# shichaoy/pop_up_slam

Measured on AMD Instinct MI355X. Metric: graph-solve iters/sec + final chi2, 1k-pose/5k-edge plane graph, higher is better.
Workload: dtype f64; 1 GPU; C2 synthetic corridor: 1000 SE3 poses, 200 planes, 5000 plane edges, 999 odometry edges (BASELINE.json configs[1], seed 42); jacobian_mode=numeric, total_lm_solves=773

## Files before the change

### include/pps.h

```cpp
#ifndef PPS_H
#define PPS_H

#include <stddef.h>
#include <stdint.h>

#ifdef __cplusplus
extern "C" {
#endif

#define PPS_VERSION 305

typedef struct pps_graph pps_graph;

enum pps_status {
  PPS_OK = 0,
  PPS_EINVAL = 1,
  PPS_ENOTPD = 2,
  PPS_EHIP = 3,
  PPS_ENOMEM = 4,
  PPS_ESTATE = 5
};

enum pps_jacobian_mode {
  PPS_JAC_NUMERIC = 0,
  PPS_JAC_ANALYTIC = 1
};

typedef struct pps_props {
  double epsilon2;
  double epsilon_abs;
  double epsilon_rel;
  int    max_iterations;
  double lm_lambda0;
  double lm_lambda_factor;
  int    jacobian_mode;
  int    device;
  int    verbose;
} pps_props;

void pps_default_props(pps_props* p);
int  pps_version(void);
const char* pps_last_error(const pps_graph* g);

int pps_graph_create(const pps_props* props, pps_graph** out);
int pps_graph_destroy(pps_graph* g);
int pps_get_props(const pps_graph* g, pps_props* out);
int pps_set_props(pps_graph* g, const pps_props* p);

int pps_add_pose(pps_graph* g, const double tq[7], int* id);
int pps_add_plane(pps_graph* g, const double abcd[4], int* id);

int pps_add_pose_prior(pps_graph* g, int pose, const double meas6[6], const double sqrtinf_ut[21], int* fid);
int pps_add_odometry(pps_graph* g, int pose1, int pose2, const double meas6[6], const double sqrtinf_ut[21], int* fid);
int pps_add_plane_obs(pps_graph* g, int pose, int plane, const double meas4[4], const double sqrtinf_ut[6], int* fid);
int pps_add_plane_obs2(pps_graph* g, int pose_id, int plane_id, const double meas4[4], const double ray6[6],
                       const double sqrtinf_ut[6], int* fid);
int pps_edge_ray(const float invK[9], const float seg2d[4], double ray6[6]);
int pps_add_plane_prior(pps_graph* g, int plane, const double meas4[4], const double sqrtinf_ut[6], int* fid);

int pps_set_measurement(pps_graph* g, int fid, const double meas4[4]);
int pps_set_measurements(pps_graph* g, int n, const int* fids, const double* meas4 );

int pps_remove_factor(pps_graph* g, int fid);
int pps_remove_node(pps_graph* g, int nid);

int pps_update(pps_graph* g);
int pps_batch_optimize(pps_graph* g, int* iterations);
int pps_chi2(pps_graph* g, double* chi2);

int pps_cov_recover(pps_graph* g);
int pps_cov_marginals(pps_graph* g, int n, const int* ids, double* out, int64_t* offsets);
int pps_cov_access(pps_graph* g, int n, const int* rows, const int* cols, double* out, int64_t* offsets, int* in_pattern);
int pps_cov_joint(pps_graph* g, int n, const int* ids, double* out);
int pps_cov_last_times(const pps_graph* g, double sec[2]);
int pps_cov_factor(pps_graph* g);
int pps_debug_cov_path_form(pps_graph* g, int form);
int pps_cov_select(pps_graph* g);
int pps_debug_cov_select_form(pps_graph* g, int form);
int pps_cov_block(pps_graph* g, int nr, const int* rows, int nc, const int* cols, double* out);
int pps_cov_block_last(const pps_graph* g, double* kernel_sec, int* launches);

int pps_assoc_gate(pps_graph* g, int pose_id, int n_meas, const double* meas4, const double* sqrtinf_ut, int n_planes, const int* plane_ids,
                   double* d2, int* best);
int pps_assoc_gate_last(const pps_graph* g, double* kernel_sec, int* launches);
int pps_debug_assoc_gate_records(pps_graph* g, int64_t cap, double* rec, int64_t* needed);

int pps_merge_gate(pps_graph* g, int n_planes, const int* plane_ids, double floor_var, double threshold, double* d2, int* best, int cap_pairs,
                   int* pairs, int* n_pairs);
int pps_merge_gate_last(const pps_graph* g, double* kernel_sec, int* launches, int* n_not_pd);
int pps_debug_merge_gate_records(pps_graph* g, int64_t cap, double* rec, int64_t* needed);

int pps_loop_gate(pps_graph* g, int n, const int* pose_a, const int* pose_b, const double* meas6 ,
                  const double* sqrtinf_ut , double threshold, double* d2 , double* S ,
                  int cap_accepted, int* accepted, int* n_accepted);
int pps_loop_gate_last(const pps_graph* g, double* kernel_sec, int* launches, int* n_not_pd);
int pps_debug_loop_gate_records(pps_graph* g, int64_t cap, double* rec, int64_t* needed);

int pps_factor_gate(pps_graph* g, int n, const int* fids, double thr3, double thr6, double* d2, double* leverage, int cap_flagged, int* flagged,
                    int* n_flagged);
int pps_factor_gate_last(const pps_graph* g, double* kernel_sec, int* launches, int* n_untestable);
int pps_debug_factor_gate_records(pps_graph* g, int64_t cap, double* rec, int64_t* needed);

enum pps_cost_kind { PPS_COST_NONE = 0, PPS_COST_HUBER = 1, PPS_COST_PSEUDO_HUBER = 2, PPS_COST_CAUCHY = 3 };
int pps_set_cost_function(pps_graph* g, int kind, double b);
int pps_get_cost_function(const pps_graph* g, int* kind, double* b);

typedef struct pps_multi pps_multi;
int pps_multi_create(int n, pps_graph* const* graphs, pps_multi** out);
int pps_multi_destroy(pps_multi* m);
const char* pps_multi_last_error(const pps_multi* m);
int pps_multi_optimize(pps_multi* m, int* iterations, int* status);
int pps_multi_rounds(const pps_multi* m, int* rounds);
int pps_multi_save_state(pps_multi* m);
int pps_multi_restore_state(pps_multi* m);
int pps_multi_set_profiling(pps_multi* m, int level);
int pps_multi_phase_times(const pps_multi* m, double sec[5], long long counts[4]);

int pps_num_nodes(const pps_graph* g, int* n);
int pps_num_factors(const pps_graph* g, int* n);
int pps_get_pose(pps_graph* g, int id, double tq[7]);
int pps_get_plane(pps_graph* g, int id, double abcd[4]);
int pps_set_pose(pps_graph* g, int id, const double tq[7]);
int pps_set_plane(pps_graph* g, int id, const double abcd[4]);
int pps_get_poses(pps_graph* g, int n, const int* ids, double* out);
int pps_get_planes(pps_graph* g, int n, const int* ids, double* out);
int pps_save_state(pps_graph* g);
int pps_restore_state(pps_graph* g);

typedef struct pps_stats {
  int    n_poses, n_planes, n_factors;
  int    dim_nodes, dim_measure;
  int    n_fronts, n_levels, max_front;
  int64_t nnz_L;
  int    lm_iterations;
  int    lm_trials_accepted, lm_trials_rejected;
  double chi2_initial, chi2_final, lambda_final;
  double last_delta_norm;
  double t_total, t_analysis, t_upload;
  double t_linearize, t_assemble, t_factor, t_backsolve, t_retract_chi2;
  int    n_linearize, n_factorize;
  int    lm_trials_notpd;
  int    n_launches;
} pps_stats;
int pps_get_stats(const pps_graph* g, pps_stats* out);
int pps_get_trace(const pps_graph* g, int cap, double* lambda, double* chi2, int* accepted, int* n);
int pps_set_profiling(pps_graph* g, int level);

int pps_factor_shape(const pps_graph* g, int fid, int* dim, int* cols);
int pps_eval_factor(pps_graph* g, int fid, int mode , double* J, double* r);

int pps_analyze(pps_graph* g);
int pps_analysis_reuse(const pps_graph* g, int* fronts_kept, int* fronts_total);
int pps_analysis_kept(const pps_graph* g, int kept[6]);
int pps_analysis_dump(pps_graph* g, int64_t cap, int32_t* out, int64_t* needed);

int pps_time_linearize(pps_graph* g, int mode, int iters, double* sec_per_launch);
int pps_bench_sweep(pps_graph* g, int mode, int replicas, int iters, double sec_per_sweep[3],
                    int64_t* n_plane_edges, int64_t* n_odo_edges);

int pps_debug_front_factor(int tiles, int strip, int p, int b, const double* A, double* L, double* U, double* not_pd);
int pps_debug_front_factor_w(int tiles, int strip, int p, int b, const double* A, double* L, double* U, double* not_pd, int width);

int pps_debug_exmap(int kind, int n, const double* x, const double* delta, double* out);

int pps_debug_solve(pps_graph* g, double lambda, double lambda2, double* delta, double* delta2, int* form, double* not_pd);

int pps_popup_planes(int device, const float* seg2d, int n, const float invK[9], const float T_wc[16],
                     float* planes_out);

typedef struct pps_point { float x, y, z; uint32_t rgba; } pps_point;

typedef struct pps_popup pps_popup;
int pps_popup_create(int device, int width, int height, const float invK[9], pps_popup** out);
int pps_popup_destroy(pps_popup* p);
const char* pps_popup_last_error(const pps_popup* p);
int pps_popup_set_image(pps_popup* p, const unsigned char* bgr);
int pps_popup_run(pps_popup* p, const float* seg2d, int n, const float T_wc[16], const float* polys,
                  const int* poly_off, int nplanes, int step, float depth_thre, float ceiling_thre, int* n_valid);
int pps_popup_run_async(pps_popup* p, const float* seg2d, int n, const float T_wc[16], const float* polys,
                        const int* poly_off, int nplanes, int step, float depth_thre, float ceiling_thre);
int pps_popup_planes_wait(pps_popup* p, float* planes);
int pps_popup_wait(pps_popup* p, int* n_valid);
int pps_popup_download(pps_popup* p, float* planes, pps_point* cloud, float* depth, int32_t* plane_id);
int pps_popup_set_outputs(pps_popup* p, int want_depth, int want_plane_id);
int pps_popup_plane_info(pps_popup* p, float plane_cam_dist_thre, const int* actual_plane_indices, int n_actual,
                         float* dist_to_cam, int32_t* good);
int pps_popup_fill_depth(pps_popup* p);
int pps_popup_download_segments3d(pps_popup* p, float* seg3d_world);
int pps_popup_last_kernel_time(const pps_popup* p, double* sec);
int pps_popup_polygons_simple(const float K[9], const float invK[9], const float T_wc[16], int width, int height, const float* seg2d, int n,
                              float* verts, int cap_verts, int* poly_off, int* n_verts);
int pps_popup_mask_host(const float* polys, const int* poly_off, int nplanes, int width, int height, int step, int32_t* plane_id);

int pps_frames_set_calibration(pps_graph* g, const float invK[9]);
int pps_frames_add(pps_graph* g, int pose_id, int n_seg, const float* seg2d, const int* fids, int* frame_id);
int pps_refresh_measurements(pps_graph* g);
int pps_get_measurement(pps_graph* g, int fid, double meas4[4]);

typedef struct pps_assoc_params {
  double edge_asso_2ddist;
  double edge_asso_planedist;
  double edge_asso_proj;
  double edge_asso_angle;
  int assoc_near_frames;
} pps_assoc_params;
void pps_assoc_default_params(pps_assoc_params* p);
int pps_landmark_update(pps_graph* g, int plane_id, int frame_plane_indice, int frame_seq_id, const float seg2d[4],
                        const float seg3d_xy[4]);
int pps_landmark_set_merged(pps_graph* g, int plane_id);
int pps_find_closest_planes(pps_graph* g, const double est_pose[7], int frame_seq_id, int n, const double* planes_local,
                            const int* frame_plane_indice, const float* seg2d, const float* seg3d_xy,
                            const pps_assoc_params* prm, int* best_plane_id, double* best_err);

int pps_graph_save(pps_graph* g, const char* path, int precision);
int pps_graph_load(const char* path, const pps_props* props, pps_graph** out);

int pps_reproject_points(pps_graph* g, int n, const int* plane_ids, const float* pts_xyz, float* out_xyz);

typedef struct pps_edge_params {
  int downsample_contour;
  int dilation_distance, erosion_distance;
  double pre_vertical_thre, pre_minium_len, pre_contour_close_thre, interval_overlap_thre, post_short_thre,
         post_bind_dist_thre, post_merge_dist_thre, post_merge_angle_thre, post_extend_thre;
  double pre_boundary_thre, pre_merge_angle_thre, pre_merge_dist_thre, pre_proj_angle_thre, pre_proj_cover_thre,
         pre_proj_cover_large_thre, pre_proj_dist_thre;
} pps_edge_params;
void pps_edge_default_params(pps_edge_params* p);

typedef struct pps_edges pps_edges;
int pps_edges_create(int device, int width, int height, pps_edges** out);
int pps_edges_destroy(pps_edges* e);
const char* pps_edges_last_error(const pps_edges* e);
int pps_edges_select(pps_edges* e, const unsigned char* label_map, int label_on_device, const float* lsd_lines,
                     int n_lines, const pps_edge_params* prm, float* open_segs, int* n_open, float* closed_segs,
                     int* n_closed, float* open_in_closed);
int pps_edges_download_label(pps_edges* e, unsigned char* out, int* w, int* h);
int pps_edges_contour(pps_edges* e, float* xy, int cap, int* n, int* n_contours, int* n_points);
int pps_edges_last_kernel_time(const pps_edges* e, double* sec);
int pps_edges_host_contour(const int16_t* cell_segs, int n, float scale, float* xy, int cap, int* n_xy, int* n_contours,
                           int* n_points);
int pps_edges_host_select(const float* contour_xy, int n_contour, int width, int height, const float* lsd_lines, int n_lines,
                          const pps_edge_params* prm, float* open_segs, int* n_open, float* closed_segs, int* n_closed,
                          float* open_in_closed);

typedef struct pps_map pps_map;
typedef struct pps_map_chunk {
  int32_t frame;
  int32_t frame_seq_id;
  int32_t frame_plane;
  int32_t plane_id;
  int64_t offset, count;
} pps_map_chunk;
typedef struct pps_map_totals {
  int64_t capacity, n_points;
  int64_t built_points;
  int32_t n_frames, n_chunks, built_chunks, reserved;
} pps_map_totals;
typedef struct pps_map_select {
  int32_t counter;
  int32_t every_frame;
  int32_t old_age, old_every, new_every;
  int32_t age[3], min_tracked[3];
} pps_map_select;
void pps_map_default_select(pps_map_select* s, int counter);
int pps_map_create(pps_graph* g, int64_t capacity_points, pps_map** out);
int pps_map_destroy(pps_map* m);
const char* pps_map_last_error(const pps_map* m);
int pps_map_add_frame(pps_map* m, pps_popup* p, int frame_seq_id, int nplanes, const int* plane_node_ids, int* counts);
int pps_map_redirect(pps_map* m, int from_plane, int to_plane);
int pps_map_info(const pps_map* m, pps_map_totals* out);
int pps_map_chunks(const pps_map* m, int cap, pps_map_chunk* out, int* n);
int pps_map_built_chunks(const pps_map* m, int cap, pps_map_chunk* out, int* n);
int pps_map_select_host(const pps_map_chunk* chunks, int n, const pps_map_select* sel, int32_t* keep, int* n_keep);
int pps_map_build(pps_map* m, const pps_map_select* sel, int64_t* n_points, int* n_chunks);
int pps_map_download(pps_map* m, int which, int64_t first, int64_t n, pps_point* out);
int pps_map_last_times(const pps_map* m, double sec[2]);

#ifdef __cplusplus
}
#endif
#endif
```

### pop_up_slam_amd/__init__.py

```python
from __future__ import annotations

import ctypes as C
import os

import numpy as np

_HERE = os.path.dirname(os.path.abspath(__file__))
LIB_PATH = os.environ.get("PPS_LIB") or os.path.join(_HERE, "libpps.so")

PPS_OK, PPS_EINVAL, PPS_ENOTPD, PPS_EHIP, PPS_ENOMEM, PPS_ESTATE = range(6)
JAC_NUMERIC, JAC_ANALYTIC = 0, 1
COST_NONE, COST_HUBER, COST_PSEUDO_HUBER, COST_CAUCHY = range(4)

_dp = C.POINTER(C.c_double)
_fp = C.POINTER(C.c_float)
_ip = C.POINTER(C.c_int)


PPS_VERSION = 305


class PpsProps(C.Structure):
    _fields_ = [
        ("epsilon2", C.c_double), ("epsilon_abs", C.c_double), ("epsilon_rel", C.c_double),
        ("max_iterations", C.c_int), ("lm_lambda0", C.c_double), ("lm_lambda_factor", C.c_double),
        ("jacobian_mode", C.c_int), ("device", C.c_int), ("verbose", C.c_int),
    ]


class PpsStats(C.Structure):
    _fields_ = [
        ("n_poses", C.c_int), ("n_planes", C.c_int), ("n_factors", C.c_int),
        ("dim_nodes", C.c_int), ("dim_measure", C.c_int),
        ("n_fronts", C.c_int), ("n_levels", C.c_int), ("max_front", C.c_int),
        ("nnz_L", C.c_int64),
        ("lm_iterations", C.c_int), ("lm_trials_accepted", C.c_int), ("lm_trials_rejected", C.c_int),
        ("chi2_initial", C.c_double), ("chi2_final", C.c_double), ("lambda_final", C.c_double),
        ("last_delta_norm", C.c_double),
        ("t_total", C.c_double), ("t_analysis", C.c_double), ("t_upload", C.c_double),
        ("t_linearize", C.c_double), ("t_assemble", C.c_double), ("t_factor", C.c_double),
        ("t_backsolve", C.c_double), ("t_retract_chi2", C.c_double),
        ("n_linearize", C.c_int), ("n_factorize", C.c_int), ("lm_trials_notpd", C.c_int), ("n_launches", C.c_int),
    ]

    def asdict(self):
        return {k: getattr(self, k) for k, _ in self._fields_}


class PpsError(RuntimeError):
    def __init__(self, code, msg):
        super().__init__(f"pps error {code}: {msg}")
        self.code = code


_LIB = None

def edge_ray(invK, seg2d):
    k = np.ascontiguousarray(invK, dtype=np.float32).reshape(9); sg = np.ascontiguousarray(seg2d, dtype=np.float32).reshape(4)
    out = np.zeros(6)
    rc = lib().pps_edge_ray(k.ctypes.data_as(_fp), sg.ctypes.data_as(_fp), out.ctypes.data_as(_dp))
    if rc != PPS_OK:
        raise PpsError(rc, "pps_edge_ray")
    return out


class PpsEdgeParams(C.Structure):
    _fields_ = [("downsample_contour", C.c_int), ("dilation_distance", C.c_int), ("erosion_distance", C.c_int)] + [
        (k, C.c_double) for k in ("pre_vertical_thre", "pre_minium_len", "pre_contour_close_thre", "interval_overlap_thre",
                                  "post_short_thre", "post_bind_dist_thre", "post_merge_dist_thre", "post_merge_angle_thre",
                                  "post_extend_thre", "pre_boundary_thre", "pre_merge_angle_thre", "pre_merge_dist_thre",
                                  "pre_proj_angle_thre", "pre_proj_cover_thre", "pre_proj_cover_large_thre",
                                  "pre_proj_dist_thre")]


class PpsAssocParams(C.Structure):
    _fields_ = [("edge_asso_2ddist", C.c_double), ("edge_asso_planedist", C.c_double), ("edge_asso_proj", C.c_double),
                ("edge_asso_angle", C.c_double), ("assoc_near_frames", C.c_int)]


class PpsMapChunk(C.Structure):
    _fields_ = [("frame", C.c_int32), ("frame_seq_id", C.c_int32), ("frame_plane", C.c_int32), ("plane_id", C.c_int32),
                ("offset", C.c_int64), ("count", C.c_int64)]


class PpsMapTotals(C.Structure):
    _fields_ = [("capacity", C.c_int64), ("n_points", C.c_int64), ("built_points", C.c_int64),
                ("n_frames", C.c_int32), ("n_chunks", C.c_int32), ("built_chunks", C.c_int32), ("reserved", C.c_int32)]


class PpsMapSelect(C.Structure):
    _fields_ = [("counter", C.c_int32), ("every_frame", C.c_int32), ("old_age", C.c_int32), ("old_every", C.c_int32),
                ("new_every", C.c_int32), ("age", C.c_int32 * 3), ("min_tracked", C.c_int32 * 3)]


CHUNK_DTYPE = np.dtype([("frame", "<i4"), ("frame_seq_id", "<i4"), ("frame_plane", "<i4"), ("plane_id", "<i4"),
                        ("offset", "<i8"), ("count", "<i8")])


SYMBOLS = [
    "pps_default_props", "pps_version", "pps_last_error", "pps_graph_create", "pps_graph_destroy",
    "pps_get_props", "pps_set_props", "pps_add_pose", "pps_add_plane", "pps_add_pose_prior",
    "pps_add_odometry", "pps_add_plane_obs", "pps_add_plane_prior", "pps_set_measurement",
    "pps_set_measurements", "pps_remove_factor", "pps_remove_node", "pps_update", "pps_batch_optimize",
    "pps_chi2", "pps_num_nodes", "pps_num_factors", "pps_get_pose", "pps_get_plane", "pps_set_pose",
    "pps_set_plane", "pps_get_poses", "pps_get_planes", "pps_get_stats", "pps_get_trace",
    "pps_set_profiling", "pps_factor_shape", "pps_eval_factor", "pps_analyze", "pps_analysis_dump",
    "pps_bench_sweep", "pps_save_state", "pps_restore_state",
    "pps_popup_planes", "pps_popup_create", "pps_popup_destroy", "pps_popup_last_error", "pps_popup_set_image",
    "pps_popup_run", "pps_popup_run_async", "pps_popup_planes_wait", "pps_popup_wait", "pps_popup_download", "pps_popup_last_kernel_time",
    "pps_frames_set_calibration", "pps_frames_add", "pps_refresh_measurements", "pps_get_measurement",
    "pps_popup_download_segments3d", "pps_assoc_default_params", "pps_landmark_update", "pps_landmark_set_merged",
    "pps_find_closest_planes", "pps_graph_save", "pps_graph_load", "pps_add_plane_obs2", "pps_edge_ray",
    "pps_time_linearize", "pps_debug_front_factor", "pps_debug_front_factor_w", "pps_debug_exmap", "pps_debug_solve", "pps_reproject_points", "pps_popup_set_outputs",
    "pps_edge_default_params", "pps_edges_create", "pps_edges_destroy", "pps_edges_last_error", "pps_edges_select",
    "pps_edges_download_label", "pps_edges_contour", "pps_edges_last_kernel_time", "pps_edges_host_contour",
    "pps_edges_host_select", "pps_popup_fill_depth", "pps_popup_plane_info", "pps_popup_mask_host",
    "pps_multi_create", "pps_multi_destroy", "pps_multi_last_error", "pps_multi_optimize", "pps_multi_rounds", "pps_multi_save_state", "pps_multi_restore_state", "pps_multi_set_profiling", "pps_multi_phase_times", "pps_popup_polygons_simple", "pps_analysis_reuse", "pps_analysis_kept",
    "pps_cov_recover", "pps_cov_marginals", "pps_cov_access", "pps_cov_joint", "pps_cov_last_times",
    "pps_cov_factor", "pps_debug_cov_path_form", "pps_cov_select", "pps_debug_cov_select_form",
    "pps_cov_block", "pps_cov_block_last", "pps_assoc_gate", "pps_assoc_gate_last", "pps_debug_assoc_gate_records",
    "pps_merge_gate", "pps_merge_gate_last", "pps_debug_merge_gate_records",
    "pps_factor_gate", "pps_factor_gate_last", "pps_debug_factor_gate_records",
    "pps_loop_gate", "pps_loop_gate_last", "pps_debug_loop_gate_records",
    "pps_map_default_select", "pps_map_create", "pps_map_destroy", "pps_map_last_error", "pps_map_add_frame", "pps_map_redirect",
    "pps_map_info", "pps_map_chunks", "pps_map_built_chunks", "pps_map_select_host", "pps_map_build", "pps_map_download",
    "pps_map_last_times",
    "pps_set_cost_function", "pps_get_cost_function",
]


def lib():
    global _LIB
    if _LIB is None:
        if not os.path.exists(LIB_PATH):
            raise ImportError(
                f"{LIB_PATH} not found: build it with `python -c 'import __graft_entry__ as g; g.build()'` "
                "(or make -C pop_up_slam_amd/csrc).  There is no CPU fallback.")
        L = C.CDLL(LIB_PATH)
        L.pps_version.restype = C.c_int
        if L.pps_version() != PPS_VERSION:
            raise ImportError(f"{LIB_PATH} reports PPS_VERSION {L.pps_version()}, this binding mirrors {PPS_VERSION}: rebuild the library")
        L.pps_last_error.restype = C.c_char_p
        L.pps_last_error.argtypes = [C.c_void_p]
        L.pps_default_props.argtypes = [C.POINTER(PpsProps)]
        L.pps_default_props.restype = None
        L.pps_graph_create.argtypes = [C.POINTER(PpsProps), C.POINTER(C.c_void_p)]
        L.pps_graph_destroy.argtypes = [C.c_void_p]
        L.pps_get_props.argtypes = [C.c_void_p, C.POINTER(PpsProps)]
        L.pps_set_props.argtypes = [C.c_void_p, C.POINTER(PpsProps)]
        L.pps_add_pose.argtypes = [C.c_void_p, _dp, _ip]
        L.pps_add_plane.argtypes = [C.c_void_p, _dp, _ip]
        L.pps_add_pose_prior.argtypes = [C.c_void_p, C.c_int, _dp, _dp, _ip]
        L.pps_add_odometry.argtypes = [C.c_void_p, C.c_int, C.c_int, _dp, _dp, _ip]
        L.pps_add_plane_obs.argtypes = [C.c_void_p, C.c_int, C.c_int, _dp, _dp, _ip]
        L.pps_add_plane_prior.argtypes = [C.c_void_p, C.c_int, _dp, _dp, _ip]
        L.pps_set_measurement.argtypes = [C.c_void_p, C.c_int, _dp]
        L.pps_set_measurements.argtypes = [C.c_void_p, C.c_int, _ip, _dp]
        L.pps_remove_factor.argtypes = [C.c_void_p, C.c_int]
        L.pps_remove_node.argtypes = [C.c_void_p, C.c_int]
        L.pps_update.argtypes = [C.c_void_p]
        L.pps_batch_optimize.argtypes = [C.c_void_p, _ip]
        L.pps_chi2.argtypes = [C.c_void_p, _dp]
        L.pps_num_nodes.argtypes = [C.c_void_p, _ip]
        L.pps_num_factors.argtypes = [C.c_void_p, _ip]
        L.pps_get_pose.argtypes = [C.c_void_p, C.c_int, _dp]
        L.pps_get_plane.argtypes = [C.c_void_p, C.c_int, _dp]
        L.pps_set_pose.argtypes = [C.c_void_p, C.c_int, _dp]
        L.pps_set_plane.argtypes = [C.c_void_p, C.c_int, _dp]
        L.pps_get_poses.argtypes = [C.c_void_p, C.c_int, _ip, _dp]
        L.pps_get_planes.argtypes = [C.c_void_p, C.c_int, _ip, _dp]
        L.pps_save_state.argtypes = [C.c_void_p]
        L.pps_restore_state.argtypes = [C.c_void_p]
        L.pps_get_stats.argtypes = [C.c_void_p, C.POINTER(PpsStats)]
        L.pps_get_trace.argtypes = [C.c_void_p, C.c_int, _dp, _dp, _ip, _ip]
        L.pps_set_profiling.argtypes = [C.c_void_p, C.c_int]
        L.pps_factor_shape.argtypes = [C.c_void_p, C.c_int, _ip, _ip]
        L.pps_eval_factor.argtypes = [C.c_void_p, C.c_int, C.c_int, _dp, _dp]
        L.pps_analyze.argtypes = [C.c_void_p]
        L.pps_analysis_dump.argtypes = [C.c_void_p, C.c_int64, C.POINTER(C.c_int32), C.POINTER(C.c_int64)]
        L.pps_bench_sweep.argtypes = [C.c_void_p, C.c_int, C.c_int, C.c_int, _dp, C.POINTER(C.c_int64),
                                      C.POINTER(C.c_int64)]
        _u8 = C.POINTER(C.c_ubyte)
        L.pps_popup_planes.argtypes = [C.c_int, _fp, C.c_int, _fp, _fp, _fp]
        L.pps_popup_create.argtypes = [C.c_int, C.c_int, C.c_int, _fp, C.POINTER(C.c_void_p)]
        L.pps_popup_destroy.argtypes = [C.c_void_p]
        L.pps_popup_last_error.argtypes = [C.c_void_p]
        L.pps_popup_last_error.restype = C.c_char_p
        L.pps_popup_set_image.argtypes = [C.c_void_p, _u8]
        L.pps_popup_run.argtypes = [C.c_void_p, _fp, C.c_int, _fp, _fp, _ip, C.c_int, C.c_int, C.c_float, C.c_float, _ip]
        L.pps_popup_run_async.argtypes = L.pps_popup_run.argtypes[:-1]
        L.pps_popup_planes_wait.argtypes = [C.c_void_p, _fp]
        L.pps_popup_wait.argtypes = [C.c_void_p, C.POINTER(C.c_int)]
        L.pps_popup_download.argtypes = [C.c_void_p, _fp, C.c_void_p, _fp, C.POINTER(C.c_int32)]
        L.pps_popup_last_kernel_time.argtypes = [C.c_void_p, _dp]
        L.pps_popup_mask_host.argtypes = [_fp, _ip, C.c_int, C.c_int, C.c_int, C.c_int, C.POINTER(C.c_int32)]
        L.pps_popup_polygons_simple.argtypes = [_fp, _fp, _fp, C.c_int, C.c_int, _fp, C.c_int, _fp, C.c_int, _ip, _ip]
        L.pps_multi_create.argtypes = [C.c_int, C.POINTER(C.c_void_p), C.POINTER(C.c_void_p)]
        L.pps_multi_destroy.argtypes = [C.c_void_p]
        L.pps_multi_last_error.argtypes = [C.c_void_p]
        L.pps_multi_last_error.restype = C.c_char_p
        L.pps_multi_optimize.argtypes = [C.c_void_p, _ip, _ip]
        L.pps_multi_rounds.argtypes = [C.c_void_p, _ip]
        L.pps_multi_save_state.argtypes = [C.c_void_p]; L.pps_multi_restore_state.argtypes = [C.c_void_p]
        L.pps_multi_set_profiling.argtypes = [C.c_void_p, C.c_int]
        L.pps_multi_phase_times.argtypes = [C.c_void_p, _dp, C.POINTER(C.c_longlong)]
        L.pps_popup_fill_depth.argtypes = [C.c_void_p]
        L.pps_popup_plane_info.argtypes = [C.c_void_p, C.c_float, _ip, C.c_int, _fp, _ip]
        L.pps_frames_set_calibration.argtypes = [C.c_void_p, _fp]
        L.pps_frames_add.argtypes = [C.c_void_p, C.c_int, C.c_int, _fp, _ip, _ip]
        L.pps_refresh_measurements.argtypes = [C.c_void_p]
        L.pps_get_measurement.argtypes = [C.c_void_p, C.c_int, _dp]
        L.pps_popup_download_segments3d.argtypes = [C.c_void_p, _fp]
        L.pps_popup_set_outputs.argtypes = [C.c_void_p, C.c_int, C.c_int]
        L.pps_assoc_default_params.argtypes = [C.POINTER(PpsAssocParams)]
        L.pps_edge_default_params.argtypes = [C.POINTER(PpsEdgeParams)]; L.pps_edge_default_params.restype = None
        L.pps_edges_create.argtypes = [C.c_int, C.c_int, C.c_int, C.POINTER(C.c_void_p)]
        L.pps_edges_destroy.argtypes = [C.c_void_p]
        L.pps_edges_last_error.argtypes = [C.c_void_p]; L.pps_edges_last_error.restype = C.c_char_p
        L.pps_edges_select.argtypes = [C.c_void_p, C.c_void_p, C.c_int, _fp, C.c_int, C.POINTER(PpsEdgeParams), _fp, _ip, _fp, _ip, _fp]
        L.pps_edges_download_label.argtypes = [C.c_void_p, C.POINTER(C.c_ubyte), _ip, _ip]
        L.pps_edges_contour.argtypes = [C.c_void_p, _fp, C.c_int, _ip, _ip, _ip]
        L.pps_edges_last_kernel_time.argtypes = [C.c_void_p, _dp]
        L.pps_edges_host_contour.argtypes = [C.POINTER(C.c_int16), C.c_int, C.c_float, _fp, C.c_int, _ip, _ip, _ip]
        L.pps_edges_host_select.argtypes = [_fp, C.c_int, C.c_int, C.c_int, _fp, C.c_int, C.POINTER(PpsEdgeParams), _fp, _ip, _fp, _ip, _fp]
        L.pps_assoc_default_params.restype = None
        L.pps_landmark_update.argtypes = [C.c_void_p, C.c_int, C.c_int, C.c_int, _fp, _fp]
        L.pps_landmark_set_merged.argtypes = [C.c_void_p, C.c_int]
        L.pps_add_plane_obs2.argtypes = [C.c_void_p, C.c_int, C.c_int, _dp, _dp, _dp, _ip]
        L.pps_edge_ray.argtypes = [_fp, _fp, _dp]
        L.pps_time_linearize.argtypes = [C.c_void_p, C.c_int, C.c_int, C.POINTER(C.c_double)]
        L.pps_debug_front_factor.argtypes = [C.c_int, C.c_int, C.c_int, C.c_int, _dp, _dp, _dp, C.POINTER(C.c_double)]
        if hasattr(L, "pps_debug_front_factor_w"):
            L.pps_debug_front_factor_w.argtypes = L.pps_debug_front_factor.argtypes + [C.c_int]
        L.pps_debug_exmap.argtypes = [C.c_int, C.c_int, _dp, _dp, _dp]
        L.pps_debug_solve.argtypes = [C.c_void_p, C.c_double, C.c_double, _dp, _dp, C.POINTER(C.c_int), C.POINTER(C.c_double)]
        L.pps_reproject_points.argtypes = [C.c_void_p, C.c_int, _ip, _fp, _fp]
        L.pps_graph_save.argtypes = [C.c_void_p, C.c_char_p, C.c_int]
        L.pps_graph_load.argtypes = [C.c_char_p, C.POINTER(PpsProps), C.POINTER(C.c_void_p)]
        L.pps_find_closest_planes.argtypes = [C.c_void_p, _dp, C.c_int, C.c_int, _dp, _ip, _fp, _fp, C.POINTER(PpsAssocParams), _ip, _dp]
        _i64p = C.POINTER(C.c_int64)
        L.pps_cov_recover.argtypes = [C.c_void_p]
        L.pps_cov_marginals.argtypes = [C.c_void_p, C.c_int, _ip, _dp, _i64p]
        L.pps_cov_access.argtypes = [C.c_void_p, C.c_int, _ip, _ip, _dp, _i64p, _ip]
        L.pps_cov_joint.argtypes = [C.c_void_p, C.c_int, _ip, _dp]
        L.pps_cov_last_times.argtypes = [C.c_void_p, _dp]
        L.pps_cov_factor.argtypes = [C.c_void_p]
        L.pps_debug_cov_path_form.argtypes = [C.c_void_p, C.c_int]
        L.pps_cov_select.argtypes = [C.c_void_p]
        L.pps_debug_cov_select_form.argtypes = [C.c_void_p, C.c_int]
        L.pps_cov_block.argtypes = [C.c_void_p, C.c_int, _ip, C.c_int, _ip, _dp]
        L.pps_cov_block_last.argtypes = [C.c_void_p, _dp, _ip]
        L.pps_assoc_gate.argtypes = [C.c_void_p, C.c_int, C.c_int, _dp, _dp, C.c_int, _ip, _dp, _ip]
        L.pps_assoc_gate_last.argtypes = [C.c_void_p, _dp, _ip]
        L.pps_debug_assoc_gate_records.argtypes = [C.c_void_p, C.c_int64, _dp, C.POINTER(C.c_int64)]
        L.pps_merge_gate.argtypes = [C.c_void_p, C.c_int, _ip, C.c_double, C.c_double, _dp, _ip, C.c_int, _ip, _ip]
        L.pps_merge_gate_last.argtypes = [C.c_void_p, _dp, _ip, _ip]
        L.pps_debug_merge_gate_records.argtypes = [C.c_void_p, C.c_int64, _dp, C.POINTER(C.c_int64)]
        L.pps_loop_gate.argtypes = [C.c_void_p, C.c_int, _ip, _ip, _dp, _dp, C.c_double, _dp, _dp, C.c_int, _ip, _ip]
        L.pps_loop_gate_last.argtypes = [C.c_void_p, _dp, _ip, _ip]
        L.pps_debug_loop_gate_records.argtypes = [C.c_void_p, C.c_int64, _dp, C.POINTER(C.c_int64)]
        L.pps_factor_gate.argtypes = [C.c_void_p, C.c_int, _ip, C.c_double, C.c_double, _dp, _dp, C.c_int, _ip, _ip]
        L.pps_factor_gate_last.argtypes = [C.c_void_p, _dp, _ip, _ip]
        L.pps_debug_factor_gate_records.argtypes = [C.c_void_p, C.c_int64, _dp, C.POINTER(C.c_int64)]
        L.pps_set_cost_function.argtypes = [C.c_void_p, C.c_int, C.c_double]
        L.pps_get_cost_function.argtypes = [C.c_void_p, _ip, _dp]
        _i32p = C.POINTER(C.c_int32)
        L.pps_map_default_select.argtypes = [C.POINTER(PpsMapSelect), C.c_int]; L.pps_map_default_select.restype = None
        L.pps_map_create.argtypes = [C.c_void_p, C.c_int64, C.POINTER(C.c_void_p)]
        L.pps_map_destroy.argtypes = [C.c_void_p]
        L.pps_map_last_error.argtypes = [C.c_void_p]; L.pps_map_last_error.restype = C.c_char_p
        L.pps_map_add_frame.argtypes = [C.c_void_p, C.c_void_p, C.c_int, C.c_int, _ip, _ip]
        L.pps_map_redirect.argtypes = [C.c_void_p, C.c_int, C.c_int]
        L.pps_map_info.argtypes = [C.c_void_p, C.POINTER(PpsMapTotals)]
        L.pps_map_chunks.argtypes = [C.c_void_p, C.c_int, C.c_void_p, _ip]
        L.pps_map_built_chunks.argtypes = [C.c_void_p, C.c_int, C.c_void_p, _ip]
        L.pps_map_select_host.argtypes = [C.c_void_p, C.c_int, C.POINTER(PpsMapSelect), _i32p, _ip]
        L.pps_map_build.argtypes = [C.c_void_p, C.POINTER(PpsMapSelect), _i64p, _ip]
        L.pps_map_download.argtypes = [C.c_void_p, C.c_int, C.c_int64, C.c_int64, C.c_void_p]
        L.pps_map_last_times.argtypes = [C.c_void_p, _dp]
        _LIB = L
    return _LIB


def _d(a, n=None):
    a = np.ascontiguousarray(a, dtype=np.float64)
    if n is not None and a.size != n:
        raise ValueError(f"expected {n} doubles, got {a.size}")
    return a, a.ctypes.data_as(_dp)


def default_props(**kw):
    p = PpsProps()
    lib().pps_default_props(C.byref(p))
    for k, v in kw.items():
        setattr(p, k, v)
    return p


class Graph:

    def __init__(self, **props):
        self.L = lib()
        self.props = default_props(**props)
        h = C.c_void_p()
        rc = self.L.pps_graph_create(C.byref(self.props), C.byref(h))
        if rc != PPS_OK:
            raise PpsError(rc, "pps_graph_create failed")
        self.h = h

    @classmethod
    def load(cls, path, **props):
        self = cls.__new__(cls)
        self.L = lib()
        self.props = default_props(**props)
        h = C.c_void_p()
        rc = self.L.pps_graph_load(os.fsencode(path), C.byref(self.props), C.byref(h))
        if rc != PPS_OK:
            raise PpsError(rc, f"pps_graph_load({path}) failed")
        self.h = h
        return self

    def save(self, path, precision=0):
        self._ck(self.L.pps_graph_save(self.h, os.fsencode(path), int(precision)))

    def close(self):
        if getattr(self, "h", None):
            self.L.pps_graph_destroy(self.h)
            self.h = None

    def __del__(self):
        try:
            self.close()
        except Exception:
            pass

    def _ck(self, rc):
        if rc != PPS_OK:
            raise PpsError(rc, self.L.pps_last_error(self.h).decode())

    def set_props(self, **kw):
        for k, v in kw.items():
            setattr(self.props, k, v)
        self._ck(self.L.pps_set_props(self.h, C.byref(self.props)))

    def get_props(self):
        p = PpsProps(); self._ck(self.L.pps_get_props(self.h, C.byref(p))); return p

    def add_pose(self, tq):
        a, p = _d(tq, 7); i = C.c_int(); self._ck(self.L.pps_add_pose(self.h, p, C.byref(i))); return i.value

    def add_plane(self, abcd):
        a, p = _d(abcd, 4); i = C.c_int(); self._ck(self.L.pps_add_plane(self.h, p, C.byref(i))); return i.value

    def add_pose_prior(self, pose, meas6, ut21):
        a, p = _d(meas6, 6); b, q = _d(ut21, 21); i = C.c_int()
        self._ck(self.L.pps_add_pose_prior(self.h, pose, p, q, C.byref(i))); return i.value

    def add_odometry(self, p1, p2, meas6, ut21):
        a, p = _d(meas6, 6); b, q = _d(ut21, 21); i = C.c_int()
        self._ck(self.L.pps_add_odometry(self.h, p1, p2, p, q, C.byref(i))); return i.value

    def add_plane_obs(self, pose, plane, meas4, ut6):
        a, p = _d(meas4, 4); b, q = _d(ut6, 6); i = C.c_int()
        self._ck(self.L.pps_add_plane_obs(self.h, pose, plane, p, q, C.byref(i))); return i.value

    def add_plane_obs2(self, pose, plane, meas4, ray6, ut6):
        a, p = _d(meas4, 4); r, pr = _d(ray6, 6); b, q = _d(ut6, 6); i = C.c_int()
        self._ck(self.L.pps_add_plane_obs2(self.h, pose, plane, p, pr, q, C.byref(i))); return i.value

    def add_plane_prior(self, plane, meas4, ut6):
        a, p = _d(meas4, 4); b, q = _d(ut6, 6); i = C.c_int()
        self._ck(self.L.pps_add_plane_prior(self.h, plane, p, q, C.byref(i))); return i.value

    def set_measurement(self, fid, meas4):
        a, p = _d(meas4, 4); self._ck(self.L.pps_set_measurement(self.h, fid, p))

    def set_measurements(self, fids, meas):
        f = np.ascontiguousarray(fids, dtype=np.int32); a, p = _d(meas, 4 * len(f))
        self._ck(self.L.pps_set_measurements(self.h, len(f), f.ctypes.data_as(_ip), p))

    def remove_factor(self, fid):
        self._ck(self.L.pps_remove_factor(self.h, fid))

    def remove_node(self, nid):
        self._ck(self.L.pps_remove_node(self.h, nid))

    def update(self):
        self._ck(self.L.pps_update(self.h))

    def batch_optimize(self):
        it = C.c_int(); self._ck(self.L.pps_batch_optimize(self.h, C.byref(it))); return it.value

    def chi2(self):
        v = C.c_double(); self._ck(self.L.pps_chi2(self.h, C.byref(v))); return v.value

    def set_cost_function(self, kind, b=1.0):
        self._ck(self.L.pps_set_cost_function(self.h, int(kind), float(b)))

    def cost_function(self):
        k = C.c_int(); b = C.c_double()
        self._ck(self.L.pps_get_cost_function(self.h, C.byref(k), C.byref(b)))
        return k.value, b.value

    def _node_dims(self, ids):
        dims = []
        for i in ids:
            try:
                self.get_pose(int(i)); dims.append(6)
            except PpsError:
                self.get_plane(int(i)); dims.append(3)
        return dims

    def cov_recover(self):
        self._ck(self.L.pps_cov_recover(self.h))

    def cov_factor(self):
        self._ck(self.L.pps_cov_factor(self.h))

    def cov_select(self):
        self._ck(self.L.pps_cov_select(self.h))

    def debug_cov_select_form(self, form):
        self._ck(self.L.pps_debug_cov_select_form(self.h, int(form)))

    def debug_cov_path_form(self, form):
        self._ck(self.L.pps_debug_cov_path_form(self.h, int(form)))

    def cov_marginals(self, ids=None):
        if ids is None:
            n = self.num_nodes(); ptr = None
        else:
            i = np.ascontiguousarray(ids, dtype=np.int32); n = len(i); ptr = i.ctypes.data_as(_ip)
        out = np.zeros(36 * max(n, 1)); off = np.zeros(n + 1, dtype=np.int64)
        self._ck(self.L.pps_cov_marginals(self.h, n, ptr, out.ctypes.data_as(_dp), off.ctypes.data_as(C.POINTER(C.c_int64))))
        blocks = []
        for k in range(n):
            d = int(round(np.sqrt(off[k + 1] - off[k])))
            blocks.append(out[off[k]:off[k + 1]].reshape(d, d).copy())
        return blocks

    def cov_access(self, pairs):
        pr = np.ascontiguousarray(pairs, dtype=np.int32).reshape(-1, 2); n = len(pr)
        rows = np.ascontiguousarray(pr[:, 0]); cols = np.ascontiguousarray(pr[:, 1])
        out = np.full(36 * max(n, 1), np.nan); off = np.zeros(n + 1, dtype=np.int64); inp = np.zeros(max(n, 1), dtype=np.int32)
        self._ck(self.L.pps_cov_access(self.h, n, rows.ctypes.data_as(_ip), cols.ctypes.data_as(_ip), out.ctypes.data_as(_dp),
                                       off.ctypes.data_as(C.POINTER(C.c_int64)), inp.ctypes.data_as(_ip)))
        res = []
        for k in range(n):
            if not inp[k]:
                res.append(None); continue
            size = int(off[k + 1] - off[k])
            dr = 6 if size == 36 else 3 if size == 9 else self._node_dims([pr[k, 0]])[0]
            res.append(out[off[k]:off[k + 1]].reshape(dr, size // dr).copy())
        return res

    def cov_joint(self, ids):
        i = np.ascontiguousarray(ids, dtype=np.int32); n = len(i)
        N = sum(self._node_dims(i))
        out = np.zeros((N, N))
        self._ck(self.L.pps_cov_joint(self.h, n, i.ctypes.data_as(_ip), out.ctypes.data_as(_dp)))
        return out

    def _records(self, fn):
        n = C.c_int64(0)
        self._ck(fn(self.h, 0, None, C.byref(n)))
        rec = np.zeros(n.value)
        self._ck(fn(self.h, n.value, rec.ctypes.data_as(_dp), C.byref(n)))
        return rec

    def _last(self, fn, n_ints):
        s = C.c_double(); k = [C.c_int() for _ in range(n_ints)]
        self._ck(fn(self.h, C.byref(s), *[C.byref(i) for i in k]))
        return (s.value,) + tuple(i.value for i in k)

    def cov_block(self, rows, cols=None):
        r = np.ascontiguousarray(rows, dtype=np.int32).reshape(-1)
        c = r if cols is None else np.ascontiguousarray(cols, dtype=np.int32).reshape(-1)
        out = np.full(36 * max(len(r), 1) * max(len(c), 1), np.nan)
        self._ck(self.L.pps_cov_block(self.h, len(r), r.ctypes.data_as(_ip), len(c), None if cols is None else c.ctypes.data_as(_ip),
                                      out.ctypes.data_as(_dp)))
        nr, nc = sum(self._node_dims(r)), sum(self._node_dims(c))
        return out[:nr * nc].reshape(nr, nc).copy()

    def cov_block_last(self):
        return self._last(self.L.pps_cov_block_last, 1)

    def assoc_gate(self, pose_id, meas4, sqrtinf_ut, plane_ids=None):
        m = np.ascontiguousarray(meas4, dtype=np.float64).reshape(-1, 4)
        w = np.ascontiguousarray(sqrtinf_ut, dtype=np.float64).reshape(-1, 6)
        if len(m) != len(w):
            raise ValueError("assoc_gate: one sqrtinf row per measurement")
        ids = None if plane_ids is None else np.ascontiguousarray(plane_ids, dtype=np.int32).reshape(-1)
        n_pl = self.stats()["n_planes"] if ids is None else len(ids)
        d2 = np.full((len(m), n_pl), np.nan); best = np.full(len(m), -1, dtype=np.int32)
        self._ck(self.L.pps_assoc_gate(self.h, int(pose_id), len(m), m.ctypes.data_as(_dp), w.ctypes.data_as(_dp), n_pl,
                                       None if ids is None else ids.ctypes.data_as(_ip), d2.ctypes.data_as(_dp), best.ctypes.data_as(_ip)))
        return d2, best

    def assoc_gate_records(self):
        rec = self._records(self.L.pps_debug_assoc_gate_records).reshape(-1, 30)
        return np.concatenate([rec[:, :18].reshape(-1, 3, 6), rec[:, 18:27].reshape(-1, 3, 3)], axis=2), rec[:, 27:].copy()

    def assoc_gate_last(self):
        return self._last(self.L.pps_assoc_gate_last, 1)

    def merge_gate(self, plane_ids=None, floor_var=0.0, threshold=7.815, want_d2=True):
        ids = None if plane_ids is None else np.ascontiguousarray(plane_ids, dtype=np.int32).reshape(-1)
        n = self.stats()["n_planes"] if ids is None else len(ids)
        d2 = np.zeros((n, n)) if want_d2 else None
        best = np.full(max(n, 1), -1, dtype=np.int32)
        cap = min(max(n * (n - 1) // 2, 1), 4096)
        while True:
            pairs = np.zeros((cap, 2), dtype=np.int32); cnt = C.c_int(0)
            self._ck(self.L.pps_merge_gate(self.h, n, None if ids is None else ids.ctypes.data_as(_ip), float(floor_var), float(threshold),
                                           None if d2 is None else d2.ctypes.data_as(_dp), best.ctypes.data_as(_ip), cap, pairs.ctypes.data_as(_ip),
                                           C.byref(cnt)))
            if cnt.value <= cap:
                return d2, best[:n].copy(), pairs[:cnt.value].copy()
            cap = cnt.value

    def merge_gate_records(self):
        rec = self._records(self.L.pps_debug_merge_gate_records).reshape(-1, 21)
        return rec[:, :9].reshape(-1, 3, 3).copy(), rec[:, 9:18].reshape(-1, 3, 3).copy(), rec[:, 18:].copy()

    def merge_gate_last(self):
        return self._last(self.L.pps_merge_gate_last, 2)

    def loop_gate(self, pose_a, pose_b, meas6, sqrtinf_ut, threshold=12.592, want_S=False):
        ia = np.ascontiguousarray(pose_a, dtype=np.int32).reshape(-1); ib = np.ascontiguousarray(pose_b, dtype=np.int32).reshape(-1)
        n = len(ia)
        m = np.ascontiguousarray(meas6, dtype=np.float64).reshape(-1, 6); w = np.ascontiguousarray(sqrtinf_ut, dtype=np.float64).reshape(-1, 21)
        if len(ib) != n or len(m) != n or len(w) != n:
            raise ValueError("loop_gate: pose_a, pose_b, meas6 and sqrtinf_ut must have one entry per candidate")
        d2 = np.full(n, np.nan); S = np.zeros((n, 6, 6)) if want_S else None
        acc = np.zeros(max(n, 1), dtype=np.int32); cnt = C.c_int(0)
        self._ck(self.L.pps_loop_gate(self.h, n, ia.ctypes.data_as(_ip), ib.ctypes.data_as(_ip), m.ctypes.data_as(_dp), w.ctypes.data_as(_dp), float(threshold),
                                      d2.ctypes.data_as(_dp), None if S is None else S.ctypes.data_as(_dp), n, acc.ctypes.data_as(_ip), C.byref(cnt)))
        return d2, S, acc[:cnt.value].copy()

    def loop_gate_records(self):
        rec = self._records(self.L.pps_debug_loop_gate_records).reshape(-1, 78)
        return rec[:, :72].reshape(-1, 6, 12).copy(), rec[:, 72:].copy()

    def loop_gate_last(self):
        return self._last(self.L.pps_loop_gate_last, 2)

    def factor_gate(self, fids=None, thr3=7.815, thr6=12.592):
        ids = None if fids is None else np.ascontiguousarray(fids, dtype=np.int32).reshape(-1)
        n = self.num_factors() if ids is None else len(ids)
        d2 = np.full(n, np.nan); lev = np.full(n, np.nan)
        flagged = np.zeros(max(n, 1), dtype=np.int32); cnt = C.c_int(0)
        self._ck(self.L.pps_factor_gate(self.h, n, None if ids is None else ids.ctypes.data_as(_ip), float(thr3), float(thr6), d2.ctypes.data_as(_dp),
                                        lev.ctypes.data_as(_dp), n, flagged.ctypes.data_as(_ip), C.byref(cnt)))
        return d2, lev, flagged[:cnt.value].copy()

    def factor_gate_records(self):
        return self._records(self.L.pps_debug_factor_gate_records).reshape(-1, 78)

    def factor_gate_last(self):
        return self._last(self.L.pps_factor_gate_last, 2)

    def cov_last_times(self):
        s = (C.c_double * 2)(); self._ck(self.L.pps_cov_last_times(self.h, s)); return float(s[0]), float(s[1])

    def num_nodes(self):
        n = C.c_int(); self._ck(self.L.pps_num_nodes(self.h, C.byref(n))); return n.value

    def num_factors(self):
        n = C.c_int(); self._ck(self.L.pps_num_factors(self.h, C.byref(n))); return n.value

    def get_pose(self, nid):
        out = np.zeros(7); self._ck(self.L.pps_get_pose(self.h, nid, out.ctypes.data_as(_dp))); return out

    def get_plane(self, nid):
        out = np.zeros(4); self._ck(self.L.pps_get_plane(self.h, nid, out.ctypes.data_as(_dp))); return out

    def set_pose(self, nid, tq):
# ... 583 lines not shown
```

### pop_up_slam_amd/csrc/pps_api.cpp

```cpp
#include "pps_graph.h"

using namespace pps;
using namespace pps_impl;

namespace pps {
Switches read_switches() {
  auto on = [](const char* k) { return getenv(k) != nullptr; };
  auto num = [](const char* k, long long dflt) { const char* e = getenv(k); return e && *e ? atoll(e) : dflt; };
  Switches s;
  s.k1_thread_form = on("PPS_K1_THREAD_FORM");
  {
    long long plain = num("PPS_PLAIN_SCHEDULE", 0);
    if (on("PPS_PLAIN_SCHEDULE") && plain <= 0) plain = 15;
    s.no_preassemble = (plain & 1) != 0; s.no_solve_flow = (plain & 2) != 0; s.no_root_fuse = (plain & 4) != 0; s.split_expand = (plain & 8) != 0;
  }
  s.no_spec_lin = on("PPS_NO_SPEC_LIN");
  s.no_dual = on("PPS_NO_DUAL");
  s.lm_plain_host = on("PPS_LM_PLAIN_HOST");
  s.no_early_record = on("PPS_NO_EARLY_RECORD");
  s.no_strip = on("PPS_NO_STRIP");
  s.no_incremental = on("PPS_NO_INCREMENTAL");
  s.no_incr_compact = on("PPS_NO_INCR_COMPACT");
  s.verify_upload = on("PPS_DEBUG_VERIFY_UPLOAD");
  s.multi_levels = on("PPS_MULTI_LEVELS");
  s.multi_thread_form = on("PPS_MULTI_THREAD_FORM");
  s.debug_drop_flag = (int)num("PPS_DEBUG_DROP_FLAG", 0);
  if (on("PPS_DEBUG_DROP_FLAG") && s.debug_drop_flag < 1) s.debug_drop_flag = 1;
  s.trace = (int)num("PPS_TRACE", 0);
  if (on("PPS_TRACE") && s.trace < 1) s.trace = 1;
  {
    long long tm = num("PPS_TIMING", 0);
    if (on("PPS_TIMING") && tm <= 0) tm = 7;
    s.analysis_timing = (tm & 1) != 0; s.upload_timing = (tm & 2) != 0; s.multi_timing = (tm & 8) ? 2 : ((tm & 4) ? 1 : 0);
    s.lm_timing = (tm & 16) != 0;
  }
  s.multi_split = (int)num("PPS_MULTI_SPLIT", 0);
  s.multi_thread_factors = num("PPS_MULTI_THREAD_FACTORS", 120000);
  return s;
}
}

namespace pps_impl {
void report_front_trace(pps_graph* g) {
  const Analysis& A = g->an;
  std::vector<long long> tr((size_t)A.n_fronts * 8);
  (void)hipMemcpy(tr.data(), g->dev.trace, tr.size() * 8, hipMemcpyDeviceToHost);
  if (g->dev.trace_solve) {
    for (int l = A.n_levels - 1; l >= 0; l--) {
      double ph[5] = {0, 0, 0, 0, 0}, gap = 0; int n = 0, ng = 0;
      for (int s2 = 0; s2 < A.n_fronts; s2++) {
        if (A.f_level[s2] != l) continue;
        n++;
        for (int k = 0; k < 5; k++) ph[k] += (double)(tr[(size_t)s2 * 8 + k + 1] - tr[(size_t)s2 * 8 + k]);
        const int par = A.f_parent[s2];
        if (par >= 0) { gap += (double)(tr[(size_t)s2 * 8] - tr[(size_t)par * 8 + 5]); ng++; }
      }
      if (!n) continue;
      fprintf(stderr, "  solve level %d (%d fronts): panel load %.0f boundary values %.0f y - L_B^T x_b %.0f back-substitution %.0f store %.0f | start after parent's end %.0f\n",
              l, n, ph[0] / n, ph[1] / n, ph[2] / n, ph[3] / n, ph[4] / n, ng ? gap / ng : 0.0);
    }
  } else {
    double acc[5] = {0, 0, 0, 0, 0};
    std::vector<double> lvl_tot(A.n_levels, 0.0); std::vector<int> lvl_n(A.n_levels, 0);
    for (int s2 = 0; s2 < A.n_fronts; s2++) {
      for (int k = 0; k < 5; k++) acc[k] += (double)(tr[(size_t)s2 * 8 + k + 1] - tr[(size_t)s2 * 8 + k]);
      lvl_tot[A.f_level[s2]] += (double)(tr[(size_t)s2 * 8 + 5] - tr[(size_t)s2 * 8]); lvl_n[A.f_level[s2]]++;
    }
    { double pn = 0, tr2 = 0; for (int s2 = 0; s2 < A.n_fronts; s2++) { pn += (double)tr[(size_t)s2 * 8 + 6]; tr2 += (double)tr[(size_t)s2 * 8 + 7]; }
      fprintf(stderr, "PPS_TRACE elimination split: panel %.0f trailing %.0f cycles per front\n", pn / A.n_fronts, tr2 / A.n_fronts); }
    fprintf(stderr, "PPS_TRACE mean cycles per front: zero %.0f gather %.0f extend-add %.0f eliminate %.0f store %.0f\n",
            acc[0] / A.n_fronts, acc[1] / A.n_fronts, acc[2] / A.n_fronts, acc[3] / A.n_fronts, acc[4] / A.n_fronts);
    for (int l = 0; l < A.n_levels; l++) fprintf(stderr, "  level %d: %d fronts, mean total %.0f cycles\n", l, lvl_n[l], lvl_tot[l] / std::max(1, lvl_n[l]));
    {
      std::vector<long long> last_child_end(A.n_fronts, 0);
      for (int s2 = 0; s2 < A.n_fronts; s2++) if (A.f_parent[s2] >= 0) last_child_end[A.f_parent[s2]] = std::max(last_child_end[A.f_parent[s2]], tr[(size_t)s2 * 8 + 5]);
      for (int l = 0; l < A.n_levels; l++) {
        double ph[7] = {0, 0, 0, 0, 0, 0, 0}, gap = 0; int n = 0, ng = 0;
        for (int s2 = 0; s2 < A.n_fronts; s2++) {
          if (A.f_level[s2] != l) continue;
          n++;
          for (int k = 0; k < 5; k++) ph[k] += (double)(tr[(size_t)s2 * 8 + k + 1] - tr[(size_t)s2 * 8 + k]);
          ph[5] += (double)tr[(size_t)s2 * 8 + 6]; ph[6] += (double)tr[(size_t)s2 * 8 + 7];
          if (last_child_end[s2] > 0) { gap += (double)(tr[(size_t)s2 * 8] - last_child_end[s2]); ng++; }
        }
        if (!n) continue;
        fprintf(stderr, "  level %d: zero %.0f gather %.0f extend-add %.0f eliminate %.0f (panel %.0f trailing %.0f) store %.0f | start after last child's end %.0f\n", l,
                ph[0] / n, ph[1] / n, ph[2] / n, ph[3] / n, ph[5] / n, ph[6] / n, ph[4] / n, ng ? gap / ng : 0.0);
      }
    }
    {
      double w[8] = {0, 0, 0, 0, 0, 0, 0, 0}; int nw2 = 0;
      for (int s2 = 0; s2 < A.n_fronts; s2++) {
        if (A.f_p[s2] + A.f_b[s2] + 1 <= 64) continue;
        nw2++;
        for (int k = 0; k < 5; k++) w[k] += (double)(tr[(size_t)s2 * 8 + k + 1] - tr[(size_t)s2 * 8 + k]);
        w[5] += (double)tr[(size_t)s2 * 8 + 6]; w[6] += (double)tr[(size_t)s2 * 8 + 7];
      }
      if (nw2) fprintf(stderr, "  fronts beyond 64 rows (%d): zero %.0f gather %.0f extend-add %.0f eliminate %.0f (panel %.0f trailing %.0f) store %.0f cycles\n", nw2,
                       w[0] / nw2, w[1] / nw2, w[2] / nw2, w[3] / nw2, w[5] / nw2, w[6] / nw2, w[4] / nw2);
    }
    long long tmin = tr[0], tmax = tr[5];
    for (int s2 = 0; s2 < A.n_fronts; s2++) { tmin = std::min(tmin, tr[(size_t)s2 * 8]); tmax = std::max(tmax, tr[(size_t)s2 * 8 + 5]); }
    fprintf(stderr, "  first start -> last end: %lld cycles\n", tmax - tmin);
  }
}
}

extern "C" {

void pps_default_props(pps_props* p) {
  if (!p) return;
  p->epsilon2 = 1e-2 * 0.1;
  p->epsilon_abs = 1e-3 * 0.1;
  p->epsilon_rel = 1e-5 * 0.1;
  p->max_iterations = 500;
  p->lm_lambda0 = 1e-6;
  p->lm_lambda_factor = 10.;
  p->jacobian_mode = PPS_JAC_NUMERIC;
  p->device = 0;
  p->verbose = 0;
}

int pps_version(void) { return PPS_VERSION; }

const char* pps_last_error(const pps_graph* g) { return g ? g->err.c_str() : "null handle"; }

int pps_graph_create(const pps_props* props, pps_graph** out) {
  if (!out) return PPS_EINVAL;
  pps_graph* g = new (std::nothrow) pps_graph();
  if (!g) return PPS_ENOMEM;
  if (props) g->props = *props; else pps_default_props(&g->props);
  g->sw = read_switches();
  g->aprm.timing = g->sw.analysis_timing ? 1 : 0;
  *out = g;
  return PPS_OK;
}

int pps_graph_destroy(pps_graph* g) {
  if (!g) return PPS_EINVAL;
  if (!g->up_laps.empty()) {
    std::vector<std::pair<std::string, double>> v(g->up_laps.begin(), g->up_laps.end());
    std::sort(v.begin(), v.end());
    for (auto& kv : v) fprintf(stderr, "[upload] %-34s %9.3f ms total\n", kv.first.c_str(), 1e3 * kv.second);
  }
  if (g->acache) analysis_cache_free(g->acache);
  if (g->dev_ready) {
    (void)hipSetDevice(g->props.device);
    (void)hipStreamSynchronize(g->stream);
    free_device(g);
    release_arenas(g);
    if (g->host_result) (void)hipHostFree(g->host_result);
    if (g->ev[0]) (void)hipEventDestroy(g->ev[0]);
    if (g->ev[1]) (void)hipEventDestroy(g->ev[1]);
    for (hipEvent_t e : g->k1_events) (void)hipEventDestroy(e);
    for (hipEvent_t e : g->fk_events) (void)hipEventDestroy(e);
    if (g->d_lms) (void)hipFree(g->d_lms);
    if (g->h_lms) (void)hipHostFree(g->h_lms);
    if (g->d_queries) (void)hipHostFree(g->d_queries);
    if (g->d_results) (void)hipHostFree(g->d_results);
    if (g->d_lm_planes) (void)hipFree(g->d_lm_planes);
    if (g->rp_pin) (void)hipHostFree(g->rp_pin);
    cov_release(g);
    (void)hipStreamDestroy(g->stream);
  }
  delete g;
  return PPS_OK;
}

int pps_get_props(const pps_graph* g, pps_props* out) {
  if (!g || !out) return PPS_EINVAL;
  *out = g->props;
  return PPS_OK;
}
int pps_set_props(pps_graph* g, const pps_props* p) {
  if (!g || !p) return PPS_EINVAL;
  if (g->dev_ready && p->device != g->props.device) return fail(g, PPS_ESTATE, "device cannot change after the first solve");
  if (p->jacobian_mode != g->props.jacobian_mode) cov_invalidate(g);
  g->props = *p;
  return PPS_OK;
}

int pps_set_cost_function(pps_graph* g, int kind, double b) {
  if (!g) return PPS_EINVAL;
  if (kind != PPS_COST_NONE && kind != PPS_COST_HUBER && kind != PPS_COST_PSEUDO_HUBER && kind != PPS_COST_CAUCHY)
    return fail(g, PPS_EINVAL, "set_cost_function: unknown kind " + std::to_string(kind));
  if (kind != PPS_COST_NONE) {
    if (!std::isfinite(b) || !(b > 0.0)) return fail(g, PPS_EINVAL, "set_cost_function: b must be a finite number > 0");
    if (kind == PPS_COST_CAUCHY && b >= kPi) return fail(g, PPS_EINVAL, "set_cost_function: the Cauchy cost log(pi / b) log(1 + d^2 / b^2) is positive only for b < pi");
  }
  cov_invalidate(g);
  g->cost = kind == PPS_COST_NONE ? CostFn{} : make_cost(kind, b);
  return PPS_OK;
}
int pps_get_cost_function(const pps_graph* g, int* kind, double* b) {
  if (!g || !kind || !b) return PPS_EINVAL;
  *kind = g->cost.kind; *b = g->cost.b;
  return PPS_OK;
}

static int add_node(pps_graph* g, int type, const double* v, int nv, int* id) {
  if (!g || !v) return PPS_EINVAL;
  for (int k = 0; k < nv; k++) if (!std::isfinite(v[k])) return fail(g, PPS_EINVAL, "non-finite node value");
  if (g->dev_values_newer) { int rc = download_state(g); if (rc != PPS_OK) return rc; }
  cov_invalidate(g);
  HostNode n{};
  n.type = type;
  for (int k = 0; k < nv; k++) n.v[k] = v[k];
  if (type == NODE_PLANE) normalize4(n.v);
  n.deleted = false; n.compact = n.slot = -1;
  g->nodes.push_back(n);
  g->n_live_nodes++;
  g->dim_nodes += type == NODE_POSE ? 6 : 3;
  g->topo_dirty = true; g->analysis_stale = true; g->host_values_newer = true;
  if (id) *id = (int)g->nodes.size() - 1;
  return PPS_OK;
}

int pps_add_pose(pps_graph* g, const double tq[7], int* id) { return add_node(g, NODE_POSE, tq, 7, id); }
int pps_add_plane(pps_graph* g, const double abcd[4], int* id) { return add_node(g, NODE_PLANE, abcd, 4, id); }

static int add_factor(pps_graph* g, int type, int a, int b, const double* meas, int nm, const double* ut, int nw, int* fid) {
  if (!g || !meas || !ut) return PPS_EINVAL;
  for (int k = 0; k < nm; k++) if (!std::isfinite(meas[k])) return fail(g, PPS_EINVAL, "non-finite measurement");
  for (int k = 0; k < nw; k++) if (!std::isfinite(ut[k])) return fail(g, PPS_EINVAL, "non-finite sqrtinf");
  cov_invalidate(g);
  HostFactor f{};
  f.type = type; f.a = a; f.b = b; f.deleted = false; f.slot = -1;
  for (int k = 0; k < nm; k++) f.meas[k] = meas[k];
  if (nm == 4) normalize4(f.meas);
  for (int k = 0; k < nw; k++) f.w[k] = ut[k];
  g->factors.push_back(f);
  g->n_live_factors++;
  g->n_live_type[type]++;
  g->dim_measure += kFDim[type];
  g->topo_dirty = true; g->analysis_stale = true;
  if (fid) *fid = (int)g->factors.size() - 1;
  return PPS_OK;
}

int pps_add_pose_prior(pps_graph* g, int pose, const double meas6[6], const double ut[21], int* fid) {
  if (!g) return PPS_EINVAL;
  if (!live_node(g, pose, NODE_POSE)) return fail(g, PPS_EINVAL, "pose prior: unknown pose id");
  return add_factor(g, F_POSE_PRIOR, pose, -1, meas6, 6, ut, 21, fid);
}
int pps_add_odometry(pps_graph* g, int p1, int p2, const double meas6[6], const double ut[21], int* fid) {
  if (!g) return PPS_EINVAL;
  if (!live_node(g, p1, NODE_POSE) || !live_node(g, p2, NODE_POSE) || p1 == p2) return fail(g, PPS_EINVAL, "odometry: bad pose ids");
  return add_factor(g, F_ODOMETRY, p1, p2, meas6, 6, ut, 21, fid);
}
int pps_add_plane_obs(pps_graph* g, int pose, int plane, const double meas4[4], const double ut[6], int* fid) {
  if (!g) return PPS_EINVAL;
  if (!live_node(g, pose, NODE_POSE) || !live_node(g, plane, NODE_PLANE)) return fail(g, PPS_EINVAL, "plane obs: bad node ids");
  return add_factor(g, F_PLANE_OBS, pose, plane, meas4, 4, ut, 6, fid);
}
int pps_add_plane_obs2(pps_graph* g, int pose, int plane, const double meas4[4], const double ray6[6], const double ut[6],
                       int* fid) {
  if (!g || !ray6) return PPS_EINVAL;
  for (int k = 0; k < 6; k++) if (!std::isfinite(ray6[k])) return fail(g, PPS_EINVAL, "non-finite edge ray");
  int id = -1;
  int rc = pps_add_plane_obs(g, pose, plane, meas4, ut, &id);
  if (rc != PPS_OK) return rc;
  g->factors[id].repop = 1;
  g->n_live_repop++;
  memcpy(g->factors[id].ray, ray6, sizeof g->factors[id].ray);
  if (fid) *fid = id;
  return PPS_OK;
}

int pps_edge_ray(const float invK[9], const float seg2d[4], double ray6[6]) {
  if (!invK || !seg2d || !ray6) return PPS_EINVAL;
  for (int e = 0; e < 2; e++) {
    const float u = seg2d[2 * e], v = seg2d[2 * e + 1];
    for (int i = 0; i < 3; i++) ray6[3 * e + i] = (double)(invK[i * 3 + 0] * u + invK[i * 3 + 1] * v + invK[i * 3 + 2] * 1.f);
  }
  return PPS_OK;
}

int pps_add_plane_prior(pps_graph* g, int plane, const double meas4[4], const double ut[6], int* fid) {
  if (!g) return PPS_EINVAL;
  if (!live_node(g, plane, NODE_PLANE)) return fail(g, PPS_EINVAL, "plane prior: unknown plane id");
  return add_factor(g, F_PLANE_PRIOR, plane, -1, meas4, 4, ut, 6, fid);
}

int pps_set_measurement(pps_graph* g, int fid, const double meas4[4]) { return pps_set_measurements(g, 1, &fid, meas4); }

int pps_set_measurements(pps_graph* g, int n, const int* fids, const double* meas4) {
  if (!g || !fids || !meas4 || n < 0) return PPS_EINVAL;
  cov_invalidate(g);
  if (g->dev_meas_newer) { int rc = download_measurements(g); if (rc != PPS_OK) return rc; }
  for (int i = 0; i < n; i++) {
    const int fid = fids[i];
    if (fid < 0 || fid >= (int)g->factors.size() || g->factors[fid].deleted) return fail(g, PPS_EINVAL, "set_measurement: unknown factor id");
    HostFactor& f = g->factors[fid];
    if (f.type != F_PLANE_OBS && f.type != F_PLANE_PRIOR) return fail(g, PPS_EINVAL, "set_measurement: not a plane factor");
    for (int k = 0; k < 4; k++) {
      if (!std::isfinite(meas4[4 * i + k])) return fail(g, PPS_EINVAL, "non-finite measurement");
      f.meas[k] = meas4[4 * i + k];
    }
    normalize4(f.meas);
  }
  g->meas_dirty = true; g->pk_meas_ok = false;
  return PPS_OK;
}

// ... 314 lines not shown
```

### pop_up_slam_amd/csrc/pps_device.h

```cpp
#pragma once

#include <hip/hip_runtime.h>

#include <cstdint>

#include "pps_cost.h"
#include "pps_k3_plan.h"

namespace pps {

struct DevGraph {
  int n_pose = 0, n_plane = 0, pose_ld = 0, plane_ld = 0;
  double *pose_est = nullptr, *pose_lin = nullptr;
  double *plane_est = nullptr, *plane_lin = nullptr;
  int *pose_voff = nullptr, *plane_voff = nullptr;
  int n_obs = 0, n_odo = 0, n_pp = 0, n_lp = 0;
  int obs_ld = 0, odo_ld = 0, pp_ld = 0, lp_ld = 0;
  int *obs_pose = nullptr, *obs_plane = nullptr; double *obs_meas = nullptr, *obs_w = nullptr;
  int n_obs_fixed = 0; double* obs_ray = nullptr;
  int *odo_a = nullptr, *odo_b = nullptr;         double *odo_meas = nullptr, *odo_w = nullptr;
  int *pp_pose = nullptr;                          double *pp_meas = nullptr, *pp_w = nullptr;
  int *lp_plane = nullptr;                         double *lp_meas = nullptr, *lp_w = nullptr;
  double* J = nullptr;
  int64_t joff_obs = 0, joff_odo = 0, joff_pp = 0, joff_lp = 0;
  double* P = nullptr;
  int64_t poff_obs = 0;
  double* H = nullptr;
  double* L = nullptr;
  double* U = nullptr;
  double* delta = nullptr;
  int n_scalars = 0;
  int n_fronts = 0, n_levels = 0, max_front = 0, n_segs = 0, n_blocks = 0;
  int *f_p = nullptr, *f_b = nullptr, *f_poff = nullptr;
  int* pidx = nullptr;
  int64_t *f_Loff = nullptr, *f_Uoff = nullptr;
  int *f_bidx_off = nullptr, *bidx = nullptr;
  int *f_child_off = nullptr, *child = nullptr;
  int *f_cmap_off = nullptr, *cmap = nullptr;
  int *level_fronts = nullptr;
  int *f_asm_off = nullptr, *asm_blk = nullptr, *asm_lrow = nullptr, *asm_lcol = nullptr;
  int *asm_el0 = nullptr, *asm_fsz = nullptr;
  int *blk_rows = nullptr, *blk_cols = nullptr, *blk_size = nullptr, *blk_nseg = nullptr;
  int64_t* blk_hoff = nullptr;
  int *seg_blk = nullptr, *seg_c0 = nullptr, *seg_cnt = nullptr;
  int64_t* seg_hoff = nullptr;
  int* contrib = nullptr;
  int n_mseg = 0; int* mseg_blk = nullptr;
  int *f_el_off = nullptr, *el_src = nullptr, *el_tgt = nullptr;
  int *blk_doff = nullptr, *blk_dst = nullptr;
  double* Hf = nullptr;
  int64_t* f_ea_off = nullptr; int* ea_tgt = nullptr;
  int *grp_lvl_off = nullptr, *glvl_front_off = nullptr, *glvl_fronts = nullptr;
  int* grp_span = nullptr;
  int *frec = nullptr, *crec = nullptr, *srec = nullptr;
  int* obs_dir = nullptr;
  int* k3_flag = nullptr;
  double* k3_xhand = nullptr;
  int* nd_segs = nullptr; int n_nd_segs = 0;
  int* k2_single = nullptr; int n_k2_single = 0;
  int* k2_multi = nullptr; int n_k2_multi = 0;
  int* k2_finish = nullptr; int n_k2_finish = 0;
  int* k2t = nullptr; int n_k2t_big = 0, n_k2t_small = 0, n_k2t_spec = 0;
  int *cls_off = nullptr, *cls_fronts = nullptr;
  double* chi2_partials = nullptr;
  int chi2_blocks = 0;
  double* dn_partials = nullptr;
  unsigned int* ticket = nullptr;
  double* result_dev = nullptr;
  long long* trace = nullptr;
  int trace_solve = 0;
  int no_strip = 0;
  unsigned sw = 0;
  double step_ac[4] = {0, 0, 0, 0};
  double* gwork = nullptr;
  int64_t gwork_stride = 0;
};

constexpr double kStatusInternal = 64.0;
enum : unsigned { SW_K1_THREAD_FORM = 1u, SW_NO_SOLVE_FLOW = 2u, SW_NO_ROOT_FUSE = 4u, SW_DEBUG_DROP_FLAG = 8u, SW_DEBUG_DROP_XFLAG = 16u, SW_NO_EARLY_RECORD = 32u };
struct Switches {
  bool k1_thread_form = false;
  bool no_preassemble = false;
  bool no_solve_flow = false;
  bool no_root_fuse = false;
  bool split_expand = false;
  bool no_spec_lin = false;
  bool no_dual = false;
  bool no_early_record = false;
  bool lm_plain_host = false;
  bool no_strip = false;
  bool no_incremental = false;
  bool no_incr_compact = false;
  bool verify_upload = false;
  bool multi_levels = false, multi_thread_form = false;
  int debug_drop_flag = 0;
  int trace = 0;
  bool analysis_timing = false, upload_timing = false, lm_timing = false;
  int multi_timing = 0;
  int multi_split = 0;
  long long multi_thread_factors = 120000;
  unsigned dev_bits() const {
    return (k1_thread_form ? SW_K1_THREAD_FORM : 0u) | (no_solve_flow ? SW_NO_SOLVE_FLOW : 0u) | (no_root_fuse ? SW_NO_ROOT_FUSE : 0u) |
           (debug_drop_flag == 1 ? SW_DEBUG_DROP_FLAG : 0u) | (debug_drop_flag == 2 ? SW_DEBUG_DROP_XFLAG : 0u) |
           (no_early_record ? SW_NO_EARLY_RECORD : 0u);
  }
};
Switches read_switches();

struct LinGuard {
  const double* chi[2];
  const double* pose[2];
  const double* plane[2];
  double error;
  int on, single;
  int want = -1;
};

struct SpecLin {
  double *J, *P, *H, *Hf;
  int which;
};

unsigned long long launch_count();
void count_launch();
#define PPS_LAUNCH(...) do { ::pps::count_launch(); hipLaunchKernelGGL(__VA_ARGS__); } while (0)
#define PPS_LAUNCH_EV(ev0, ev1, kernel, grid, block, lds, st, ...)                                                     \
  do {                                                                                                                 \
    ::pps::count_launch();                                                                                             \
    if (ev0) hipExtLaunchKernelGGL(kernel, grid, block, lds, st, ev0, ev1, 0, __VA_ARGS__);                            \
    else hipLaunchKernelGGL(kernel, grid, block, lds, st, __VA_ARGS__);                                                \
  } while (0)

hipError_t step_constants(double ac[4]);
hipError_t launch_linearize(const DevGraph& d, int mode, bool at_estimate, hipStream_t st, const LinGuard* guard = nullptr, hipEvent_t ev0 = nullptr,
                            hipEvent_t ev1 = nullptr);
hipError_t launch_hblocks(const DevGraph& d, hipStream_t st, const LinGuard* guard = nullptr, bool products = true);
bool k1_lane_form(const DevGraph& d, int mode);
bool k1_products(const DevGraph& d, int mode);
hipError_t launch_factor_level(const DevGraph& d, int level_begin, int level_count, int level_max_front, double lambda,
                               hipStream_t st);
hipError_t launch_backsolve_level(const DevGraph& d, int level_begin, int level_count, hipStream_t st);
struct DualAlt {
  double *L, *U, *delta, *result_dev, *chi2_partials, *dn_partials;
  unsigned int* ticket;
  double lambda;
};
hipError_t ensure_k3_attrs();
hipError_t launch_band_factor(const DevGraph& d, const DualAlt* alt, const K3StagePlan& sp, double lambda, hipStream_t st, hipEvent_t ev0 = nullptr,
                              hipEvent_t ev1 = nullptr, bool pre_ok = true);
hipError_t launch_band_solve(const DevGraph& d, const DualAlt* alt, const K3StagePlan& sp, hipStream_t st);
hipError_t launch_band_root(const DevGraph& d, const DualAlt* alt, const K3Plan& p, double lambda, hipStream_t st, hipEvent_t ev0 = nullptr,
                            hipEvent_t ev1 = nullptr);
hipError_t launch_band_all_factor(const DevGraph& d, const DualAlt* alt, const K3Plan& p, double lambda, int epoch, hipStream_t st,
                                  hipEvent_t ev0 = nullptr, hipEvent_t ev1 = nullptr);
hipError_t launch_band_all_solve(const DevGraph& d, const DualAlt* alt, const K3Plan& p, int epoch, hipStream_t st);
hipError_t launch_trial_dual(const DevGraph& d, const DualAlt& alt, const double* base_pose, const double* base_plane, double* out_pose0,
                             double* out_plane0, double* out_pose1, double* out_plane1, double* host_result0, double seq0, double* host_result1,
                             double seq1, hipStream_t st, int n_trials = 2);
hipError_t launch_trial_lin(const DevGraph& d, const DualAlt& alt, const SpecLin& sl, const double* base_pose, const double* base_plane, double* out_pose0,
                            double* out_plane0, double* out_pose1, double* out_plane1, double* host_result0, double seq0, double* host_result1,
                            double seq1, hipStream_t st, hipEvent_t ev0 = nullptr, hipEvent_t ev1 = nullptr);
int trial_lin_waves(const DevGraph& d);
bool trial_lin_ok(const DevGraph& d, int mode);
hipError_t launch_hblocks_spec(const DevGraph& d, const SpecLin& sl, hipStream_t st, const LinGuard* guard = nullptr);
hipError_t launch_expand_ea(const DevGraph& d, int n_fronts, double* zero, size_t n_zero, int* ones, size_t n_ones, hipStream_t st);
hipError_t launch_expand_el(const DevGraph& d, int n_asm, hipStream_t st);
hipError_t launch_expand_lists(const DevGraph& d, int n_fronts, int n_asm, double* zero, size_t n_zero, hipStream_t st);
bool band_level_solve_direct_ok(int p, int b);
int debug_front_factor(int tiles, int strip, int p, int b, const double* A_host, double* L_host, double* U_host, double* not_pd);
int debug_front_factor_w(int tiles, int strip, int p, int b, const double* A_host, double* L_host, double* U_host, double* not_pd, int width);
int debug_exmap(int kind, int n, const double* x_host, const double* delta_host, double* out_host);
hipError_t launch_retract_trial(const DevGraph& d, hipStream_t st);
hipError_t launch_retract_apply(const DevGraph& d, hipStream_t st);
hipError_t launch_chi2(const DevGraph& d, bool at_estimate, double* host_result, double seq, hipStream_t st);
hipError_t launch_clear_status(const DevGraph& d, hipStream_t st);
hipError_t launch_chi2_trial(const DevGraph& d, double* host_result, double seq, hipStream_t st);
hipError_t launch_linearize_robust(const DevGraph& d, const CostFn& cost, int mode, bool at_estimate, hipStream_t st, hipEvent_t ev0 = nullptr,
                                   hipEvent_t ev1 = nullptr);
hipError_t launch_chi2_robust(const DevGraph& d, const CostFn& cost, bool at_estimate, double* host_result, double seq, hipStream_t st);
hipError_t launch_chi2_trial_robust(const DevGraph& d, const CostFn& cost, double* host_result, double seq, hipStream_t st);

int dense_front_max_pivots();
hipError_t launch_dense_hpush(const DevGraph& d, int max_el_per_front, double lambda, hipStream_t st);
hipError_t launch_dense_factor_level(const DevGraph& d, int level_begin, int level_count, const int* off_asm, int n_asm,
                                     const int* off_pan, int n_pan, const int* off_trl, int n_trl, hipStream_t st);
hipError_t launch_dense_solve_level(const DevGraph& d, int level_begin, int level_count, int level_max_b, hipStream_t st);

constexpr int kBatchMax = 128;
enum { BF_ACTIVE = 1,
       BF_RELIN = 2 };
struct BatchStage { int grp_begin, grp_count; };
struct BatchAlt {
  double *L, *U, *delta, *result_dev, *chi2_partials, *dn_partials;
  unsigned int* ticket;
  double* pose[3];
  double* plane[3];
};
struct BatchArgs {
  const DevGraph* gs;
  const BatchStage* stage_tab;
  double* results;
  int n_total, b0, n;
  int no_products;
  double seq;
  double lambda[kBatchMax];
  unsigned char flags[kBatchMax];
  const BatchAlt* alt;
  int rstride, lin_apply;
  double lambda2[kBatchMax];
  unsigned char xsel[kBatchMax];
};
struct BatchGeom {
  int lin_blocks = 0, lin_obs_blocks = 0, lin_rest_blocks = 0, repop_blocks = 0;
  int hblocks = 0, k2t_blocks = 0, k2tg_blocks = 0, hreduce = 0, retract = 0, chi2 = 0;
  int k2_blocks = 0, k2_finish = 0;
  long long n_factors_total = 0;
  bool lin_thread_form = false;
  int n_stages = 0;
  int stage_groups[32] = {0}, stage_nw_factor[32] = {0}, stage_nw_solve[32] = {0};
  int stage_per_wave_factor[32] = {0}, stage_per_wave_solve[32] = {0}, stage_grp_fronts[32] = {0};
  bool stage_reg_only[32] = {false};
  bool stage_pre[32] = {false};
  int stage_nw_flow[32] = {0};
  bool level_form = false;
  int n_levels = 0;
  int lvl_cls_blocks[64][3] = {{0}};
  int lvl_blocks[64] = {0};
  int lvl_direct_pp[64] = {0};
  int lvl_max_panel[64] = {0};
  int solve_per_wave_all = 0;
  int stage_max_front[32] = {0};
};
hipError_t launch_batch_linearize(const BatchArgs& a, const BatchGeom& g, int mode, hipStream_t st);
hipError_t launch_batch_hblocks(const BatchArgs& a, const BatchGeom& g, hipStream_t st, bool products);
hipError_t launch_batch_chi2(const BatchArgs& a, const BatchGeom& g, int slot, hipStream_t st);
hipError_t launch_batch_solve(const BatchArgs& a, const BatchGeom& g, hipStream_t st, hipEvent_t after_factor = nullptr);
struct RestoreRec { double* dst; const double* src; long long n; };
hipError_t launch_batch_restore(const RestoreRec* tab, int n, hipStream_t st);
hipError_t launch_batch_begin_dual(const BatchArgs& a, const BatchGeom& g, hipStream_t st);
hipError_t launch_batch_trial_dual(const BatchArgs& a, const BatchGeom& g, hipStream_t st);

hipError_t launch_scatter_patches(const char* table, const char* src_base, int n_patches, char* arena, hipStream_t st);

int lds_front_limit();

hipError_t launch_sweep_bench(const DevGraph& d, int mode, int replicas, double* Jbig, int part, hipStream_t st);

}
```

### pop_up_slam_amd/csrc/pps_graph.h

```cpp
#pragma once
#include <hip/hip_runtime.h>

#include <algorithm>
#include <charconv>
#include <chrono>
#include <cmath>
#include <cstdio>
#include <cstdlib>
#include <cstring>
#include <mutex>
#include <new>
#include <string>
#include <unordered_map>
#include <vector>

#include "../../include/pps.h"
#include "pps_cov.h"
#include "pps_device.h"
#include "pps_geom.h"
#include "pps_lm.h"
#include "pps_popup_dev.h"
#include "pps_symbolic.h"

namespace pps_impl {

struct HostNode {
  int type;
  double v[7];
  bool deleted;
  int compact;
  int slot;
};
struct HostFactor {
  int type;
  int a, b;
  double meas[6];
  double w[21];
  bool deleted;
  int slot;
  int repop;
  double ray[6];
};

inline pps::BandTreeView k3_tree_view(const pps::Analysis& A) {
  pps::BandTreeView v;
  v.n_stages = A.n_stages; v.n_groups = A.n_groups; v.n_levels = A.n_levels; v.n_fronts = A.n_fronts; v.band_levels = A.band_levels;
  v.stage_grp_off = A.stage_grp_off.data(); v.grp_lvl_off = A.grp_lvl_off.data(); v.glvl_front_off = A.glvl_front_off.data(); v.glvl_fronts = A.glvl_fronts.data();
  v.stage_max_front = A.stage_max_front.data(); v.stage_max_width = A.stage_max_width.data(); v.f_p = A.f_p.data(); v.f_b = A.f_b.data(); v.f_level = A.f_level.data();
  v.level_off = A.level_off.data(); v.level_fronts = A.level_fronts.data(); v.f_el_off = A.f_el_off.data();
  return v;
}

inline double now_s() {
  using namespace std::chrono;
  return duration_cast<duration<double>>(steady_clock::now().time_since_epoch()).count();
}

template <class T>
struct DevBuf {
  T* p = nullptr; size_t cap = 0;
  int reserve(pps_graph* g, size_t count, const char* who = nullptr, const std::string& what = std::string(), const char* advice = "");
  void release() { if (p) (void)hipFree(p); p = nullptr; cap = 0; }
};

struct QueryState {
  DevBuf<char> out;
  DevBuf<unsigned int> ticket;
  DevBuf<double> rec;
  size_t rec_n = 0;
  bool clean = false;
  bool done = false;
  double sec = 0; int launches = 0;
  int count = 0;
  void release() { out.release(); ticket.release(); rec.release(); rec_n = 0; clean = done = false; }
};

}

struct pps_graph {
  pps_props props;
  std::string err;
  std::vector<pps_impl::HostNode> nodes;
  std::vector<pps_impl::HostFactor> factors;
  int n_live_nodes = 0, n_live_factors = 0, dim_nodes = 0, dim_measure = 0;
  int n_live_type[4] = {0, 0, 0, 0}, n_live_repop = 0;
  bool topo_dirty = true;
  bool analysis_stale = true;
  bool host_values_newer = true;
  bool dev_values_newer = false;
  bool meas_dirty = false;
  bool analyzed = false;
  int n_analyses = 0;
  std::vector<pps::SymNode> sym_nodes; std::vector<pps::SymFactor> sym_factors;
  size_t cmp_nodes = 0, cmp_factors = 0; int64_t cmp_base[4] = {0, 0, 0, 0}; bool cmp_valid = false, cmp_has_repop = false;
  bool grown_only = true;
  bool grown_only_upload = false;
  pps::Analysis an;
  pps::AnalysisParams aprm;
  pps::Switches sw;
  pps::CostFn cost;
  pps::AnalysisCache* acache = nullptr;
  std::vector<int> pose_ids, plane_ids;
  std::vector<int> fslot_ids[4];
  pps::K3Plan plan;
  bool use_band() const { return plan.band(); }
  bool use_dense() const { return plan.form == pps::K3Form::Dense; }
  int *d_dw_asm = nullptr, *d_dw_pan = nullptr, *d_dw_trl = nullptr;
  bool dev_ready = false;
  hipStream_t stream = nullptr;
  pps::DevGraph dev;
  std::vector<void*> allocs;
  struct Arena { char* base = nullptr; size_t cap = 0, off = 0, spill = 0; };
  Arena up, scr;
  char* stage = nullptr;
  size_t stage_cap = 0;
  size_t stage_lo = 0, stage_hi = 0;
  struct UpSlot { size_t off, cap; };
  std::vector<UpSlot> up_slots;
  size_t up_cursor = 0, up_high = 0;
  bool up_unknown = true;
  long an_seq = 0, an_base_seq = -1, up_an_seq = -1;
  bool hint_violation = false;
  bool verify_hints = false;
  bool up_unknown_meas = false;
  size_t slot_obs_meas = (size_t)-1;
  size_t slot_lp_meas = (size_t)-1;
  std::vector<int> pk_obs_a, pk_obs_b, pk_odo_a, pk_odo_b, pk_obs_ids, pk_odo_ids;
  std::vector<double> pk_obs_m, pk_obs_w, pk_odo_m, pk_odo_w;
  size_t pk_n_obs = 0, pk_n_odo = 0, pk_ld_obs = 0, pk_ld_odo = 0;
  bool pk_meas_ok = false;
  bool status_clean = false;
  bool up_inflight = false;
  double* state_pin = nullptr; size_t state_pin_cap = 0;
  bool pin_holds_est = false;
  std::unordered_map<std::string, double> up_laps;
  struct UpPatch { size_t off, len; bool exact8 = false; };
  std::vector<UpPatch> up_patches;
  char* patch_host = nullptr; size_t patch_cap = 0;
  size_t up_bytes_sent = 0, up_bytes_total = 0;
  double* host_result = nullptr;
  double seq = 0.0;
  double *spec_pose = nullptr, *spec_plane = nullptr, *spec_chi2_partials = nullptr, *spec_dn_partials = nullptr;
  unsigned int* spec_ticket = nullptr;
  double seq2 = 0.0;
  double *spec_L = nullptr, *spec_U = nullptr, *spec_delta = nullptr;
  double* spec_result = nullptr;
  double *spec_J = nullptr, *spec_P = nullptr, *spec_H = nullptr, *spec_Hf = nullptr;
  int k3_epoch = 0;
  double *snap_pose = nullptr, *snap_plane = nullptr;
  int snap_version = -1, upload_version = 0;
  int k2t_version = -1;
  int profiling = 0;
  hipEvent_t ev[2] = {nullptr, nullptr};
  unsigned long long launches0 = 0;
  std::vector<char> k1_skip;
  std::vector<hipEvent_t> k1_events;
  std::vector<hipEvent_t> fk_events;
  int fk_used = 0;
  int k1_used = 0;
  float frames_invK[9] = {1, 0, 0, 0, 1, 0, 0, 0, 1};
  std::vector<int> fr_pose;
  std::vector<int> fr_seg_off{0};
  std::vector<float> fr_seg;
  std::vector<int> fr_item_frame, fr_item_plane, fr_item_fid;
  bool frames_dirty = true;
  std::vector<int> fr_slot, fr_pslot;
  long n_removals = 0, fr_cache_removals = -1;
  int fr_hint_version = -2; size_t fr_hint_cursor = 0, fr_hint_items = 0, fr_hint_frames = 0;
  int frames_version = -1;
  int *d_item_frame = nullptr, *d_item_plane = nullptr, *d_item_slot = nullptr, *d_frame_pose_slot = nullptr, *d_frame_seg_off = nullptr;
  float* d_fr_seg = nullptr;
  bool dev_meas_newer = false;
  int n_obs_fixed = 0;
  struct Landmark { int plane_id, fpi, seq, deleted; float seg2d[4], seg3d[4]; };
  std::vector<Landmark> lms;
  std::unordered_map<int, int> lm_of_plane;
  bool lms_dirty = true;
  int lms_upload_version = -1;
  pps::AssocLandmark* d_lms = nullptr; size_t d_lms_cap = 0;
  pps::AssocLandmark* h_lms = nullptr;
  pps::AssocQuery* d_queries = nullptr; pps::AssocResult* d_results = nullptr; size_t d_q_cap = 0;
  double* d_lm_planes = nullptr; size_t d_lm_planes_cap = 0;
  char* rp_pin = nullptr; size_t rp_cap = 0;
  bool cov_valid = false;
  bool cov_factor_valid = false;
  int cov_version = -1;
  enum : unsigned { kCovTables = 1,
                    kCovLevelShapes = 2,
                    kCovParent = 4,
                    kCovDense = 8 };
  struct CovCache { int version = -1; unsigned have = 0; } cov_cache;
  pps_impl::DevBuf<double> cov_S;
  pps_impl::DevBuf<int> cov_parent;
  pps_impl::DevBuf<char> cov_req;
  pps_impl::DevBuf<double> cov_out;
  std::vector<int> cov_epos, cov_front_of;
  hipEvent_t cov_ev[3] = {nullptr, nullptr, nullptr};
  double cov_sec[2] = {0, 0};
  std::vector<int> cov_rootlen; int cov_max_p = 0, cov_max_rows = 0;
  pps_impl::DevBuf<char> cov_breq;
  pps_impl::DevBuf<double> cov_strip;
  hipEvent_t cov_qev[2] = {nullptr, nullptr};
  pps_impl::DevBuf<double> cov_zscr;
  int cov_path_form = 0;
  pps_impl::DevBuf<double> cov_G;
  pps_impl::DevBuf<int> cov_dtab;
  int cov_dpre_items = 0;
  std::vector<int> cov_dlevel;
  int cov_select_form = 0;
  pps_impl::QueryState q_block, q_assoc, q_merge, q_loop, q_factor;
  pps_impl::DevBuf<char> fgate_tab; int fgate_tab_version = -1, fgate_tab_n = 0;
  pps_impl::DevBuf<int> fgate_list;
  pps_stats stats{};
  std::vector<double> tr_lambda, tr_chi2;
  std::vector<int> tr_acc;
};

namespace pps_impl {
using namespace pps;

inline int fail(pps_graph* g, int code, const std::string& msg) {
  if (g) g->err = msg;
  return code;
}
inline int hip_fail(pps_graph* g, hipError_t e, const char* what) {
  return fail(g, PPS_EHIP, std::string(what) + ": " + hipGetErrorString(e));
}
#define HIP_TRY(g, expr)                                   \
  do {                                                     \
    hipError_t _e = (expr);                                \
    if (_e != hipSuccess) return hip_fail(g, _e, #expr);   \
  } while (0)

inline bool live_node(const pps_graph* g, int id, int type) {
  return id >= 0 && id < (int)g->nodes.size() && !g->nodes[id].deleted && g->nodes[id].type == type;
}

void free_device(pps_graph* g);
void release_arenas(pps_graph* g);
void up_diff(pps_graph* g, size_t o, const char* src, size_t n, bool force, size_t same_prefix = 0);
int flush_uploads(pps_graph* g);
int verify_uploads(pps_graph* g, const char* where);
int ensure_device(pps_graph* g);
int64_t j_capacity(int64_t n);
void j_bases(const pps_graph* g, int64_t base[4], int64_t* total);
void p_bases(const pps_graph* g, int64_t base[4], int64_t* total);
int run_analysis(pps_graph* g);
int state_pin_reserve(pps_graph* g, size_t doubles);
int linpoint_from_estimate(pps_graph* g);
int download_state(pps_graph* g);
int enqueue_state_download(pps_graph* g);
void state_download_arrived(pps_graph* g);
int upload_state(pps_graph* g, bool sync = true);
int download_measurements(pps_graph* g);
int upload_measurements(pps_graph* g);
int upload_all(pps_graph* g);
int prepare_solve(pps_graph* g);
int read_result(pps_graph* g, bool at_estimate, double* chi2, double* dnorm, bool* notpd);
void begin_solve(pps_graph* g);
void abandon_device_copy(pps_graph* g);
int clear_stale_status(pps_graph* g);
int enqueue_plain_factor(pps_graph* g, double lambda);
struct NoSolveScope {
  pps_graph* g; pps_stats saved; int profiling; unsigned long long launches0;
  explicit NoSolveScope(pps_graph* g_) : g(g_), saved(g_->stats), profiling(g_->profiling), launches0(g_->launches0) { g->profiling = 0; }
  ~NoSolveScope() {
    g->profiling = profiling;
    g->launches0 = launches0;
    pps_stats s = saved;
    s.n_fronts = g->stats.n_fronts; s.n_levels = g->stats.n_levels; s.max_front = g->stats.max_front; s.nnz_L = g->stats.nnz_L;
    g->stats = s;
  }
};
inline LmSink lm_sink(pps_graph* g, bool verbose) { return LmSink{&g->props, &g->tr_lambda, &g->tr_chi2, &g->tr_acc, &g->stats, verbose}; }
inline void place_state_copies(pps_graph* g, double* const pose[3], double* const plane[3], int fin) {
  g->dev.pose_est = pose[fin]; g->dev.plane_est = plane[fin];
  g->dev.pose_lin = pose[(fin + 1) % 3]; g->dev.plane_lin = plane[(fin + 1) % 3];
  g->spec_pose = pose[(fin + 2) % 3]; g->spec_plane = plane[(fin + 2) % 3];
}
constexpr const char* kHandoverMessage = "internal error: a hand-over flag between the waves or workgroups of a K3 launch never arrived (the step was discarded)";
inline bool handover_timed_out(const double* rec) { return rec[2] >= pps::kStatusInternal; }
inline bool robust(const pps_graph* g) { return g->cost.kind != COST_NONE; }
inline hipError_t lin_launch(pps_graph* g, int mode, bool at_estimate, const LinGuard* guard = nullptr, hipEvent_t ev0 = nullptr, hipEvent_t ev1 = nullptr) {
  if (robust(g)) return launch_linearize_robust(g->dev, g->cost, mode, at_estimate, g->stream, ev0, ev1);
  return launch_linearize(g->dev, mode, at_estimate, g->stream, guard, ev0, ev1);
}
inline hipError_t chi2_launch(pps_graph* g, bool at_estimate, double* host_result, double seq) {
  if (robust(g)) return launch_chi2_robust(g->dev, g->cost, at_estimate, host_result, seq, g->stream);
  return launch_chi2(g->dev, at_estimate, host_result, seq, g->stream);
}
inline hipError_t chi2_trial_launch(pps_graph* g, double* host_result, double seq) {
  if (robust(g)) return launch_chi2_trial_robust(g->dev, g->cost, host_result, seq, g->stream);
  return launch_chi2_trial(g->dev, host_result, seq, g->stream);
}
// ... 120 lines not shown
```

### pop_up_slam_amd/csrc/pps_k4.hip

```cpp
#include <algorithm>
#include <cstdlib>

#include <hip/hip_ext.h>

#include "pps_geom.h"
#include "pps_kcommon.h"
#include "pps_k1_body.h"
#include "pps_k4_body.h"

namespace pps {

template <bool TRIAL>
__device__ __forceinline__ void body_retract(const DevGraph& d, double* __restrict__ pose_lin, double* __restrict__ pose_est,
                                             double* __restrict__ plane_lin, double* __restrict__ plane_est, int bx, double* red) {
  const int i = bx * blockDim.x + threadIdx.x;
  double dn = 0.0;
  if (i < d.n_pose) {
    double p[7], o[7], dl[6];
    load_pose(pose_lin, d.pose_ld, i, p);
    const int off = d.pose_voff[i];
#pragma unroll
    for (int k = 0; k < 6; k++) { dl[k] = d.delta[off + k]; dn += dl[k] * dl[k]; }
    pose_exmap(p, dl, o);
    if (TRIAL) {
#pragma unroll
      for (int k = 0; k < 7; k++) { pose_est[(size_t)k * d.pose_ld + i] = p[k]; pose_lin[(size_t)k * d.pose_ld + i] = o[k]; }
    } else {
#pragma unroll
      for (int k = 0; k < 7; k++) pose_est[(size_t)k * d.pose_ld + i] = o[k];
    }
  } else if (i < d.n_pose + d.n_plane) {
    const int l = i - d.n_pose;
    double p[4], o[4], dl[3];
    load_plane(plane_lin, d.plane_ld, l, p);
    const int off = d.plane_voff[l];
#pragma unroll
    for (int k = 0; k < 3; k++) { dl[k] = d.delta[off + k]; dn += dl[k] * dl[k]; }
    plane_exmap(p, dl, o);
    if (TRIAL) {
#pragma unroll
      for (int k = 0; k < 4; k++) { plane_est[(size_t)k * d.plane_ld + l] = p[k]; plane_lin[(size_t)k * d.plane_ld + l] = o[k]; }
    } else {
#pragma unroll
      for (int k = 0; k < 4; k++) plane_est[(size_t)k * d.plane_ld + l] = o[k];
    }
  }
#pragma unroll
  for (int o2 = 32; o2 > 0; o2 >>= 1) dn += __shfl_down(dn, o2, 64);
  if ((threadIdx.x & 63) == 0) red[threadIdx.x >> 6] = dn;
  __syncthreads();
  if (threadIdx.x == 0) d.dn_partials[bx] = red[0] + red[1] + red[2] + red[3];
}

template <bool TRIAL>
__global__ __launch_bounds__(256) void k_retract(DevGraph d) {
  __shared__ double red[4];
  body_retract<TRIAL>(d, d.pose_lin, d.pose_est, d.plane_lin, d.plane_est, blockIdx.x, red);
}

hipError_t launch_retract_trial(const DevGraph& d, hipStream_t st) {
  const int n = d.n_pose + d.n_plane;
  if (n == 0) return hipSuccess;
  PPS_LAUNCH(k_retract<true>, dim3(cdiv(n, 256)), dim3(256), 0, st, d);
  return hipGetLastError();
}
hipError_t launch_retract_apply(const DevGraph& d, hipStream_t st) {
  const int n = d.n_pose + d.n_plane;
  if (n == 0) return hipSuccess;
  PPS_LAUNCH(k_retract<false>, dim3(cdiv(n, 256)), dim3(256), 0, st, d);
  return hipGetLastError();
}

__global__ __launch_bounds__(kChiBlock) void k_chi2(DevGraph d, const double* __restrict__ pose,
                                                    const double* __restrict__ plane, int nb_obs, int nb_odo, int nb_pp,
                                                    int n_dn, double* __restrict__ out, double seq) {
  body_chi2(d, pose, plane, nb_obs, nb_odo, nb_pp, n_dn, out, seq, blockIdx.x, gridDim.x);
}

__device__ __forceinline__ void body_retract_to(const DevGraph& d, const double* __restrict__ base_pose, const double* __restrict__ base_plane,
                                                double* __restrict__ out_pose, double* __restrict__ out_plane, int bx, double* red, bool light = false) {
  const int i = bx * blockDim.x + threadIdx.x;
  double dn = 0.0;
  if (i < d.n_pose) {
    double p[7], o[7], dl[6];
    load_pose(base_pose, d.pose_ld, i, p);
    const int off = d.pose_voff[i];
#pragma unroll
    for (int k = 0; k < 6; k++) { dl[k] = d.delta[off + k]; dn += dl[k] * dl[k]; }
    pose_exmap(p, dl, o);
#pragma unroll
    for (int k = 0; k < 7; k++) out_pose[(size_t)k * d.pose_ld + i] = o[k];
  } else if (i < d.n_pose + d.n_plane) {
    const int l = i - d.n_pose;
    double p[4], o[4], dl[3];
    load_plane(base_plane, d.plane_ld, l, p);
    const int off = d.plane_voff[l];
#pragma unroll
    for (int k = 0; k < 3; k++) { dl[k] = d.delta[off + k]; dn += dl[k] * dl[k]; }
    plane_exmap(p, dl, o);
#pragma unroll
    for (int k = 0; k < 4; k++) out_plane[(size_t)k * d.plane_ld + l] = o[k];
  }
#pragma unroll
  for (int o2 = 32; o2 > 0; o2 >>= 1) dn += __shfl_down(dn, o2, 64);
  if ((threadIdx.x & 63) == 0) red[threadIdx.x >> 6] = dn;
  __syncthreads();
  if (threadIdx.x == 0) {
    const double t = red[0] + red[1] + red[2] + red[3];
    if (light) publish_partial(&d.dn_partials[bx], t); else d.dn_partials[bx] = t;
  }
}

__global__ __launch_bounds__(kChiBlock) void k_trial_dual(DevGraph d, DualAlt alt, const double* __restrict__ base_pose, const double* __restrict__ base_plane,
                                                          double* __restrict__ out_pose, double* __restrict__ out_plane, double* __restrict__ out_pose1,
                                                          double* __restrict__ out_plane1, int nb_ret, int nb_obs, int nb_odo, int nb_pp, int nb_chi,
                                                          double* __restrict__ out, double seq, double* __restrict__ out1, double seq1) {
  if (blockIdx.y) {
    d.delta = alt.delta; d.chi2_partials = alt.chi2_partials; d.dn_partials = alt.dn_partials; d.ticket = alt.ticket; d.result_dev = alt.result_dev;
    out_pose = out_pose1; out_plane = out_plane1; out = out1; seq = seq1;
  }
  const int total = nb_ret + nb_chi;
  if ((int)blockIdx.x >= nb_ret) {
    body_chi2<true, true>(d, base_pose, base_plane, nb_obs, nb_odo, nb_pp, nb_ret, out, seq, (int)blockIdx.x - nb_ret, nb_chi, total);
    return;
  }
  __shared__ double red[4];
  body_retract_to(d, base_pose, base_plane, out_pose, out_plane, blockIdx.x, red);
  __shared__ bool last;
  if (threadIdx.x == 0) {
    __builtin_amdgcn_fence(__ATOMIC_RELEASE, "agent");
    asm volatile("s_waitcnt vmcnt(0)" ::: "memory");
    last = atomicAdd(d.ticket, 1u) == (unsigned int)(total - 1);
  }
  __syncthreads();
  if (!last) return;
  if (threadIdx.x == 0) __builtin_amdgcn_fence(__ATOMIC_ACQUIRE, "agent");
  __syncthreads();
  chi2_finish(d, nb_chi, nb_ret, out, seq);
  if (threadIdx.x == 0) *d.ticket = 0u;
}

hipError_t launch_trial_dual(const DevGraph& d, const DualAlt& alt, const double* base_pose, const double* base_plane, double* out_pose0,
                             double* out_plane0, double* out_pose1, double* out_plane1, double* host_result0, double seq0, double* host_result1,
                             double seq1, hipStream_t st, int n_trials) {
  const int n = d.n_pose + d.n_plane;
  const int nb_obs = cdiv(d.n_obs, kChiBlock), nb_odo = cdiv(d.n_odo, kChiBlock), nb_pp = cdiv(d.n_pp, kChiBlock), nb_lp = cdiv(d.n_lp, kChiBlock);
  const int nb = nb_obs + nb_odo + nb_pp + nb_lp;
  if (nb == 0 || n == 0) return hipErrorInvalidValue;
  const int nb_ret = cdiv(n, 256);
  PPS_LAUNCH(k_trial_dual, dim3(nb_ret + nb, n_trials), dim3(kChiBlock), 0, st, d, alt, base_pose, base_plane, out_pose0, out_plane0, out_pose1, out_plane1, nb_ret,
             nb_obs, nb_odo, nb_pp, nb, host_result0, seq0, host_result1, seq1);
  return hipGetLastError();
}

__global__ __launch_bounds__(kChiBlock) void k_trial_lin(DevGraph d, DualAlt alt, SpecLin sl, const double* __restrict__ base_pose, const double* __restrict__ base_plane,
                                                         double* __restrict__ out_pose, double* __restrict__ out_plane, double* __restrict__ out_pose1,
                                                         double* __restrict__ out_plane1, int nb_ret, int nb_obs, int nb_odo, int nb_pp, int nb_chi,
                                                         double* __restrict__ out, double seq, double* __restrict__ out1, double seq1, int lb_obs, int lb_odo, int lb_pp, int apply) {
  static_assert(kChiBlock == kLanesPerBlock, "one block size for the trial blocks and the lane-form sweep");
  const int total = nb_ret + nb_chi;
  const bool sweep = (int)blockIdx.x >= 2 * total;
  const int y = sweep ? sl.which : ((int)blockIdx.x >= total ? 1 : 0);
  const int bx0 = sweep ? (int)blockIdx.x - 2 * total : (int)blockIdx.x - y * total;
  if (y) {
    d.delta = alt.delta; d.chi2_partials = alt.chi2_partials; d.dn_partials = alt.dn_partials; d.ticket = alt.ticket; d.result_dev = alt.result_dev;
    out_pose = out_pose1; out_plane = out_plane1; out = out1; seq = seq1;
  }
  if (sweep) {
    d.J = sl.J; d.P = sl.P; d.H = sl.H; d.Hf = sl.Hf;
    body_linearize_lanes(d, base_pose, base_plane, lb_obs, lb_odo, lb_pp, bx0, apply != 0);
    return;
  }
  const bool light = (d.sw & SW_NO_EARLY_RECORD) == 0;
  if (light) __builtin_amdgcn_s_setprio(3);
  if (bx0 >= nb_ret) {
    body_chi2<true, true>(d, base_pose, base_plane, nb_obs, nb_odo, nb_pp, nb_ret, out, seq, bx0 - nb_ret, nb_chi, total, CostFn{}, light);
    return;
  }
  __shared__ double red[4];
  body_retract_to(d, base_pose, base_plane, out_pose, out_plane, bx0, red, light);
  __shared__ bool last;
  if (threadIdx.x == 0) {
    if (!light) __builtin_amdgcn_fence(__ATOMIC_RELEASE, "agent");
    asm volatile("s_waitcnt vmcnt(0)" ::: "memory");
    last = atomicAdd(d.ticket, 1u) == (unsigned int)(total - 1);
  }
  __syncthreads();
  if (!last) return;
  if (threadIdx.x == 0) __builtin_amdgcn_fence(__ATOMIC_ACQUIRE, "agent");
  __syncthreads();
  chi2_finish(d, nb_chi, nb_ret, out, seq, light);
  if (threadIdx.x == 0) *d.ticket = 0u;
}

int trial_lin_waves(const DevGraph& d) {
  const int nb = cdiv(d.n_obs, kChiBlock) + cdiv(d.n_odo, kChiBlock) + cdiv(d.n_pp, kChiBlock) + cdiv(d.n_lp, kChiBlock) + cdiv(d.n_pose + d.n_plane, 256);
  const int lb = cdiv(d.n_obs_fixed, kObsPerBlock) + cdiv(d.n_odo, kFactorsPerBlock) + cdiv(d.n_pp, kFactorsPerBlock) + cdiv(d.n_lp, kFactorsPerBlock);
  return (2 * nb + lb) * (kChiBlock / 64);
}
bool trial_lin_ok(const DevGraph& d, int mode) { return k1_lane_form(d, mode) && d.n_obs == d.n_obs_fixed && d.P != nullptr; }

hipError_t launch_trial_lin(const DevGraph& d, const DualAlt& alt, const SpecLin& sl, const double* base_pose, const double* base_plane, double* out_pose0,
                            double* out_plane0, double* out_pose1, double* out_plane1, double* host_result0, double seq0, double* host_result1,
                            double seq1, hipStream_t st, hipEvent_t ev0, hipEvent_t ev1) {
  const int n = d.n_pose + d.n_plane;
  const int nb_obs = cdiv(d.n_obs, kChiBlock), nb_odo = cdiv(d.n_odo, kChiBlock), nb_pp = cdiv(d.n_pp, kChiBlock), nb_lp = cdiv(d.n_lp, kChiBlock);
  const int nb = nb_obs + nb_odo + nb_pp + nb_lp;
  if (nb == 0 || n == 0) return hipErrorInvalidValue;
  const int nb_ret = cdiv(n, 256);
  const int lb_obs = cdiv(d.n_obs_fixed, kObsPerBlock), lb_odo = cdiv(d.n_odo, kFactorsPerBlock), lb_pp = cdiv(d.n_pp, kFactorsPerBlock),
            lb_lp = cdiv(d.n_lp, kFactorsPerBlock);
  const int lb_all = lb_obs + lb_odo + lb_pp + lb_lp;
  PPS_LAUNCH_EV(ev0, ev1, k_trial_lin, dim3(2 * (nb_ret + nb) + lb_all), dim3(kChiBlock), 0, st, d, alt, sl, base_pose, base_plane, out_pose0,
                out_plane0, out_pose1, out_plane1, nb_ret, nb_obs, nb_odo, nb_pp, nb, host_result0, seq0, host_result1, seq1, lb_obs, lb_odo, lb_pp, 1);
  return hipGetLastError();
}

hipError_t launch_chi2(const DevGraph& d, bool at_estimate, double* host_result, double seq, hipStream_t st) {
  const int nb_obs = cdiv(d.n_obs, kChiBlock), nb_odo = cdiv(d.n_odo, kChiBlock), nb_pp = cdiv(d.n_pp, kChiBlock),
            nb_lp = cdiv(d.n_lp, kChiBlock);
  const int nb = nb_obs + nb_odo + nb_pp + nb_lp;
  const double* pose = at_estimate ? d.pose_est : d.pose_lin;
  const double* plane = at_estimate ? d.plane_est : d.plane_lin;
  if (nb == 0) return hipErrorInvalidValue;
  const int n_dn = cdiv(d.n_pose + d.n_plane, 256);
  PPS_LAUNCH(k_chi2, dim3(nb), dim3(kChiBlock), 0, st, d, pose, plane, nb_obs, nb_odo, nb_pp, n_dn, host_result, seq);
  return hipGetLastError();
}

__global__ __launch_bounds__(kChiBlock) void k_chi2_trial(DevGraph d, int nb_obs, int nb_odo, int nb_pp, int n_dn, double* __restrict__ out, double seq) {
  body_chi2<true, true>(d, d.pose_est, d.plane_est, nb_obs, nb_odo, nb_pp, n_dn, out, seq, blockIdx.x, gridDim.x);
}

hipError_t launch_chi2_trial(const DevGraph& d, double* host_result, double seq, hipStream_t st) {
  const int nb_obs = cdiv(d.n_obs, kChiBlock), nb_odo = cdiv(d.n_odo, kChiBlock), nb_pp = cdiv(d.n_pp, kChiBlock),
            nb_lp = cdiv(d.n_lp, kChiBlock);
  const int nb = nb_obs + nb_odo + nb_pp + nb_lp;
  if (nb == 0) return hipErrorInvalidValue;
  PPS_LAUNCH(k_chi2_trial, dim3(nb), dim3(kChiBlock), 0, st, d, nb_obs, nb_odo, nb_pp, cdiv(d.n_pose + d.n_plane, 256), host_result, seq);
  return hipGetLastError();
}

__global__ __launch_bounds__(kChiBlock) void kb_chi2(BatchArgs a, int slot) {
  PPS_BATCH_PROLOGUE(BF_ACTIVE)
  const int nb_obs = dcdiv(d.n_obs, kChiBlock), nb_odo = dcdiv(d.n_odo, kChiBlock), nb_pp = dcdiv(d.n_pp, kChiBlock),
            nb_lp = dcdiv(d.n_lp, kChiBlock);
  const int nb = nb_obs + nb_odo + nb_pp + nb_lp;
  if ((int)blockIdx.x >= nb) return;
  body_chi2<false>(d, pose_lin, plane_lin, nb_obs, nb_odo, nb_pp, dcdiv(d.n_pose + d.n_plane, 256),
                   a.results + (size_t)(a.alt ? 12 : 8) * (size_t)(a.b0 + b) + 4 * slot, a.seq, blockIdx.x, nb);
}

__global__ __launch_bounds__(kChiBlock) void kb_chi2_finish(BatchArgs a, int slot, int dual) {
  PPS_BATCH_PROLOGUE(BF_ACTIVE)
  const int nb = dcdiv(d.n_obs, kChiBlock) + dcdiv(d.n_odo, kChiBlock) + dcdiv(d.n_pp, kChiBlock) + dcdiv(d.n_lp, kChiBlock);
  const int n_dn = dcdiv(d.n_pose + d.n_plane, 256);
  if (!dual) { chi2_finish(d, nb, n_dn, a.results + (size_t)(a.alt ? 12 : 8) * (size_t)(a.b0 + b) + 4 * slot, a.seq); return; }
  DevGraph d2 = d;
  if (blockIdx.z) {
    const BatchAlt al = load_alt(a.alt + a.b0 + b);
    d2.chi2_partials = al.chi2_partials; d2.dn_partials = al.dn_partials; d2.result_dev = al.result_dev;
  }
  chi2_finish(d2, nb, n_dn, a.results + 12 * (size_t)(a.b0 + b) + 4 * (1 + blockIdx.z), a.seq);
}

hipError_t launch_batch_chi2(const BatchArgs& a, const BatchGeom& g, int slot, hipStream_t st) {
  if (g.chi2 <= 0) return hipErrorInvalidValue;
  PPS_LAUNCH(kb_chi2, dim3(g.chi2, a.n), dim3(kChiBlock), 0, st, a, slot);
  PPS_LAUNCH(kb_chi2_finish, dim3(1, a.n), dim3(kChiBlock), 0, st, a, slot, 0);
  return hipGetLastError();
}

__global__ __launch_bounds__(64) void kb_begin_dual(BatchArgs a) {
  PPS_BATCH_PROLOGUE(BF_ACTIVE)
  const BatchAlt al = load_alt(a.alt + a.b0 + b);
  if (threadIdx.x < 4) { d.result_dev[threadIdx.x] = 0.0; al.result_dev[threadIdx.x] = 0.0; }
}

__global__ __launch_bounds__(kChiBlock) void kb_trial_dual(BatchArgs a, int nb_ret) {
  __shared__ double red[4];
  PPS_BATCH_PROLOGUE(BF_ACTIVE)
  const BatchAlt al = load_alt(a.alt + a.b0 + b);
  const int xs = a.xsel[b], z = blockIdx.z;
  const int ts = (xs + 1 + z) % 3;
  DevGraph d2 = d;
  if (z) { d2.delta = al.delta; d2.chi2_partials = al.chi2_partials; d2.dn_partials = al.dn_partials; d2.ticket = al.ticket; d2.result_dev = al.result_dev; }
  if ((int)blockIdx.x < nb_ret) {
    if ((int)blockIdx.x * 256 >= d.n_pose + d.n_plane) return;
    body_retract_to(d2, pose_lin, plane_lin, sel3(al.pose, ts), sel3(al.plane, ts), blockIdx.x, red);
    return;
  }
  const int nb_obs = dcdiv(d.n_obs, kChiBlock), nb_odo = dcdiv(d.n_odo, kChiBlock), nb_pp = dcdiv(d.n_pp, kChiBlock),
            nb_lp = dcdiv(d.n_lp, kChiBlock);
  const int nb = nb_obs + nb_odo + nb_pp + nb_lp;
  const int bx = (int)blockIdx.x - nb_ret;
  if (bx >= nb) return;
  body_chi2<false, true>(d2, pose_lin, plane_lin, nb_obs, nb_odo, nb_pp, dcdiv(d.n_pose + d.n_plane, 256),
                         a.results + 12 * (size_t)(a.b0 + b) + 4 * (1 + z), a.seq, bx, nb);
}

__global__ __launch_bounds__(256) void kb_restore(const RestoreRec* __restrict__ tab) {
  const RestoreRec r = tab[blockIdx.y];
  for (long long i = (long long)blockIdx.x * 256 + threadIdx.x; i < r.n; i += 256LL * gridDim.x) r.dst[i] = r.src[i];
}

hipError_t launch_batch_restore(const RestoreRec* tab, int n, hipStream_t st) {
  PPS_LAUNCH(kb_restore, dim3(8, n), dim3(256), 0, st, tab);
  return hipGetLastError();
}

hipError_t launch_batch_begin_dual(const BatchArgs& a, const BatchGeom& g, hipStream_t st) {
  (void)g;
  PPS_LAUNCH(kb_begin_dual, dim3(1, a.n), dim3(64), 0, st, a);
  return hipGetLastError();
}

hipError_t launch_batch_trial_dual(const BatchArgs& a, const BatchGeom& g, hipStream_t st) {
  if (g.chi2 <= 0) return hipErrorInvalidValue;
  static_assert(kChiBlock == 256, "the retraction blocks of kb_trial_dual are 256 nodes wide");
  PPS_LAUNCH(kb_trial_dual, dim3(g.retract + g.chi2, a.n, 2), dim3(kChiBlock), 0, st, a, g.retract);
  PPS_LAUNCH(kb_chi2_finish, dim3(1, a.n, 2), dim3(kChiBlock), 0, st, a, 0, 1);
  return hipGetLastError();
}

__global__ __launch_bounds__(256) void k_scatter_patches(const char* __restrict__ table, const char* __restrict__ src_base, char* __restrict__ arena) {
  const long long* tab = reinterpret_cast<const long long*>(table) + 4 * (size_t)blockIdx.x;
  const long long dst = tab[0], src = tab[1], len = tab[2];
  if (tab[3]) {
    const long long* s8 = reinterpret_cast<const long long*>(src_base + src);
    long long* d8 = reinterpret_cast<long long*>(arena + dst);
    for (long long i = (long long)blockIdx.y * 256 + threadIdx.x; i < len / 8; i += (long long)gridDim.y * 256) d8[i] = s8[i];
    return;
  }
  const int4* s4 = reinterpret_cast<const int4*>(src_base + src);
  int4* d4 = reinterpret_cast<int4*>(arena + dst);
  for (long long i = (long long)blockIdx.y * 256 + threadIdx.x; i < len / 16; i += (long long)gridDim.y * 256) d4[i] = s4[i];
}

hipError_t launch_scatter_patches(const char* table, const char* src_base, int n_patches, char* arena, hipStream_t st) {
  if (n_patches <= 0) return hipSuccess;
  PPS_LAUNCH(k_scatter_patches, dim3(n_patches, 8), dim3(256), 0, st, table, src_base, arena);
  return hipGetLastError();
}

hipError_t launch_clear_status(const DevGraph& d, hipStream_t st) {
  return hipMemsetAsync(d.result_dev, 0, 4 * sizeof(double), st);
}

__global__ void k_debug_exmap(int kind, int n, const double* __restrict__ x, const double* __restrict__ dl, double* __restrict__ out) {
  const int i = blockIdx.x * blockDim.x + threadIdx.x;
  if (i >= n) return;
  if (kind == 0) {
    double p[7], d[6], o[7];
    for (int k = 0; k < 7; k++) p[k] = x[i * 7 + k];
    for (int k = 0; k < 6; k++) d[k] = dl[i * 6 + k];
    pose_exmap(p, d, o);
    for (int k = 0; k < 7; k++) out[i * 7 + k] = o[k];
  } else {
    double p[4], d[3], o[4];
    for (int k = 0; k < 4; k++) p[k] = x[i * 4 + k];
    for (int k = 0; k < 3; k++) d[k] = dl[i * 3 + k];
    plane_exmap(p, d, o);
    for (int k = 0; k < 4; k++) out[i * 4 + k] = o[k];
  }
}

int debug_exmap(int kind, int n, const double* x_host, const double* delta_host, double* out_host) {
// ... 19 lines not shown
```

### pop_up_slam_amd/csrc/pps_k4_body.h

```cpp
#pragma once
#include "pps_cost.h"
#include "pps_geom.h"
#include "pps_kcommon.h"

namespace pps {

constexpr int kChiBlock = 256;

__device__ __forceinline__ void publish_partial(double* p, double v) {
  const unsigned long long old = __hip_atomic_exchange(reinterpret_cast<unsigned long long*>(p), (unsigned long long)__double_as_longlong(v),
                                                       __ATOMIC_RELAXED, __HIP_MEMORY_SCOPE_AGENT);
  asm volatile("" ::"v"(old));
}

__device__ __forceinline__ void chi2_finish(const DevGraph& d, int nb, int n_dn, double* __restrict__ out, double seq, bool light = false) {
  const double npd = threadIdx.x == 0 ? __hip_atomic_load(&d.result_dev[2], __ATOMIC_RELAXED, __HIP_MEMORY_SCOPE_AGENT) : 0.0;
  double cs = 0.0, dn = 0.0;
  for (int i = threadIdx.x; i < nb; i += kChiBlock) cs += __hip_atomic_load(&d.chi2_partials[i], __ATOMIC_RELAXED, __HIP_MEMORY_SCOPE_AGENT);
  for (int i = threadIdx.x; i < n_dn; i += kChiBlock) dn += __hip_atomic_load(&d.dn_partials[i], __ATOMIC_RELAXED, __HIP_MEMORY_SCOPE_AGENT);
#pragma unroll
  for (int o = 32; o > 0; o >>= 1) { cs += __shfl_down(cs, o, 64); dn += __shfl_down(dn, o, 64); }
  __shared__ double red2[2][kChiBlock / 64];
  if ((threadIdx.x & 63) == 0) { red2[0][threadIdx.x >> 6] = cs; red2[1][threadIdx.x >> 6] = dn; }
  __syncthreads();
  if (threadIdx.x == 0) {
    double a = 0.0, b2 = 0.0;
    for (int k = 0; k < kChiBlock / 64; k++) { a += red2[0][k]; b2 += red2[1][k]; }
    d.result_dev[0] = a; d.result_dev[1] = b2; d.result_dev[2] = 0.0;
    if (light) {
      __hip_atomic_store(&out[0], a, __ATOMIC_RELAXED, __HIP_MEMORY_SCOPE_SYSTEM);
      __hip_atomic_store(&out[1], b2, __ATOMIC_RELAXED, __HIP_MEMORY_SCOPE_SYSTEM);
      __hip_atomic_store(&out[2], npd, __ATOMIC_RELAXED, __HIP_MEMORY_SCOPE_SYSTEM);
      asm volatile("s_waitcnt vmcnt(0)" ::: "memory");
      __hip_atomic_store(&out[3], seq, __ATOMIC_RELAXED, __HIP_MEMORY_SCOPE_SYSTEM);
      return;
    }
    out[0] = a; out[1] = b2; out[2] = npd;
    __hip_atomic_store(&out[3], seq, __ATOMIC_RELEASE, __HIP_MEMORY_SCOPE_SYSTEM);
  }
}

template <bool TICKET = true, bool APPLY = false, bool ROBUST = false>
__device__ __forceinline__ void body_chi2(const DevGraph& d, const double* __restrict__ pose,
                                          const double* __restrict__ plane, int nb_obs, int nb_odo, int nb_pp,
                                          int n_dn, double* __restrict__ out, double seq, int bx, int nb, int total_blocks = 0, const CostFn& cost = CostFn{}, bool light = false) {
  __shared__ double red[kChiBlock / 64];
  int b = bx;
  double s = 0.0;
  if (b < nb_obs) {
    const int i = b * kChiBlock + threadIdx.x;
    if (i < d.n_obs) {
      double pz[7], pl[4], ms[4], w[6], e[3], r[3];
      fetch_pose<APPLY>(d, pose, d.obs_pose[i], pz);
      fetch_plane<APPLY>(d, plane, d.obs_plane[i], pl);
      if (i < d.n_obs_fixed) load_soa<4>(d.obs_meas, d.obs_ld, i, ms);
      else {
        double ray[6];
        load_soa<6>(d.obs_ray, d.n_obs - d.n_obs_fixed, i - d.n_obs_fixed, ray);
        repop_wall_plane(pz, ray, ms);
      }
      load_soa<6>(d.obs_w, d.obs_ld, i, w);
      res_plane_obs(pz, pl, ms, e);
      whiten<3>(w, e, r);
      if (ROBUST) robustify<3>(cost, r);
      s = r[0] * r[0] + r[1] * r[1] + r[2] * r[2];
    }
  } else if ((b -= nb_obs) < nb_odo) {
    const int i = b * kChiBlock + threadIdx.x;
    if (i < d.n_odo) {
      double p1[7], p2[7], ms[6], w[21], e[6], r[6];
      fetch_pose<APPLY>(d, pose, d.odo_a[i], p1);
      fetch_pose<APPLY>(d, pose, d.odo_b[i], p2);
      load_soa<6>(d.odo_meas, d.odo_ld, i, ms);
      load_soa<21>(d.odo_w, d.odo_ld, i, w);
      res_odometry(p1, p2, ms, e);
      whiten<6>(w, e, r);
      if (ROBUST) robustify<6>(cost, r);
#pragma unroll
      for (int k = 0; k < 6; k++) s += r[k] * r[k];
    }
  } else if ((b -= nb_odo) < nb_pp) {
    const int i = b * kChiBlock + threadIdx.x;
    if (i < d.n_pp) {
      double pz[7], ms[6], w[21], e[6], r[6];
      fetch_pose<APPLY>(d, pose, d.pp_pose[i], pz);
      load_soa<6>(d.pp_meas, d.pp_ld, i, ms);
      load_soa<21>(d.pp_w, d.pp_ld, i, w);
      res_pose_prior(pz, ms, e);
      whiten<6>(w, e, r);
      if (ROBUST) robustify<6>(cost, r);
#pragma unroll
      for (int k = 0; k < 6; k++) s += r[k] * r[k];
    }
  } else {
    b -= nb_pp;
    const int i = b * kChiBlock + threadIdx.x;
    if (i < d.n_lp) {
      double pl[4], ms[4], w[6], e[3], r[3];
      fetch_plane<APPLY>(d, plane, d.lp_plane[i], pl);
      load_soa<4>(d.lp_meas, d.lp_ld, i, ms);
      load_soa<6>(d.lp_w, d.lp_ld, i, w);
      res_plane_prior(pl, ms, e);
      whiten<3>(w, e, r);
      if (ROBUST) robustify<3>(cost, r);
      s = r[0] * r[0] + r[1] * r[1] + r[2] * r[2];
    }
  }
#pragma unroll
  for (int o = 32; o > 0; o >>= 1) s += __shfl_down(s, o, 64);
  if ((threadIdx.x & 63) == 0) red[threadIdx.x >> 6] = s;
  __syncthreads();
  if (!TICKET) {
    if (threadIdx.x == 0) { double t = 0.0; for (int k = 0; k < kChiBlock / 64; k++) t += red[k]; d.chi2_partials[bx] = t; }
    return;
  }
  __shared__ bool last;
  if (threadIdx.x == 0) {
    double t = 0.0;
    for (int k = 0; k < kChiBlock / 64; k++) t += red[k];
    if (light) publish_partial(&d.chi2_partials[bx], t);
    else { d.chi2_partials[bx] = t; __builtin_amdgcn_fence(__ATOMIC_RELEASE, "agent"); }
    asm volatile("s_waitcnt vmcnt(0)" ::: "memory");
    last = atomicAdd(d.ticket, 1u) == (unsigned int)((total_blocks > 0 ? total_blocks : nb) - 1);
  }
  __syncthreads();
  if (!last) return;
  if (threadIdx.x == 0) __builtin_amdgcn_fence(__ATOMIC_ACQUIRE, "agent");
  __syncthreads();
  chi2_finish(d, nb, n_dn, out, seq, light);
  if (threadIdx.x == 0) *d.ticket = 0u;
}

}
```

### pop_up_slam_amd/csrc/pps_lm.h

```cpp
#pragma once
#include <cmath>
#include <cstdio>
#include <vector>

#include "../../include/pps.h"

namespace pps_impl {

struct LmSink {
  const pps_props* prop;
  std::vector<double>*tr_lambda, *tr_chi2;
  std::vector<int>* tr_acc;
  pps_stats* stats;
  bool verbose;
};

enum class LmVerdict { Rejected, Accepted, Converged };

constexpr const char* kLmNotPdMessage = "normal equations not positive definite at the last LM trial";

struct LmControl {
  double lambda, error = 0.0, dnorm = 0.0;
  int num_iter = 0;
  bool last_notpd = false;
  int n_notpd = 0;

  explicit LmControl(const pps_props& p) : lambda(p.lm_lambda0) {}

  bool running(const pps_props& p) const { return (p.max_iterations <= 0 || num_iter < p.max_iterations) && dnorm > p.epsilon2 && error > p.epsilon_abs; }

  void take_step(const double* rec) {
    dnorm = std::sqrt(rec[1]);
    last_notpd = rec[2] != 0.0;
    n_notpd += last_notpd ? 1 : 0;
  }

  struct Trial { double lambda, chi2; int iter; bool accepted; };
  __attribute__((always_inline)) LmVerdict decide(const pps_props& p, double error_new, Trial* t) {
    num_iter++;
    const double error_diff = error - error_new;
    const bool accepted = error_diff > 0.;
    *t = Trial{lambda, error_new, num_iter, accepted};
    if (!accepted) {
      lambda *= p.lm_lambda_factor;
      return LmVerdict::Rejected;
    }
    const bool converged = error_diff < p.epsilon_rel * error;
    error = error_new;
    if (converged) return LmVerdict::Converged;
    lambda /= p.lm_lambda_factor;
    return LmVerdict::Accepted;
  }
  static void note(const LmSink& s, const Trial& t) {
    s.tr_lambda->push_back(t.lambda); s.tr_chi2->push_back(t.chi2); s.tr_acc->push_back(t.accepted ? 1 : 0);
    if (s.verbose) fprintf(stderr, "LM Iteration %d: (lambda=%g) %s %.12g\n", t.iter, t.lambda, t.accepted ? "residual:" : "rejected", t.chi2);
    if (t.accepted) s.stats->lm_trials_accepted++; else s.stats->lm_trials_rejected++;
  }
  __attribute__((always_inline)) LmVerdict judge(const LmSink& s, double error_new) {
    Trial t;
    const LmVerdict v = decide(*s.prop, error_new, &t);
    note(s, t);
    return v;
  }

  int finish(const LmSink& s, int* iterations) const {
    pps_stats& st = *s.stats;
    st.lm_iterations = num_iter;
    st.chi2_final = error; st.lambda_final = lambda; st.last_delta_norm = dnorm;
    st.lm_trials_notpd = n_notpd;
    if (iterations) *iterations = num_iter;
    return last_notpd ? PPS_ENOTPD : PPS_OK;
  }
};

enum class LmNext {
  Done,
  Second,
  Relaunch,
  Relinearise
};

struct LmDualWalk {
  LmControl lm;
  int cur = 0, x = 0;
  bool have_next = false;
  bool trial_taken = false;

  explicit LmDualWalk(const pps_props& p) : lm(p) {}

  int trial(int k) const { const int c = x + 1 + k; return c < 3 ? c : c - 3; }
  int final_copy() const { return trial_taken ? trial(cur) : x; }
  void begin_set(bool two_trials) { cur = 0; have_next = two_trials; }
  __attribute__((always_inline)) LmNext judge(const pps_props& p, double error_new, LmControl::Trial* t) {
    const LmVerdict v = lm.decide(p, error_new, t);
    if (v == LmVerdict::Converged) { trial_taken = true; return LmNext::Done; }
    if (v == LmVerdict::Accepted) { x = trial(cur); return LmNext::Relinearise; }
    if (!have_next) return LmNext::Relaunch;
    cur = 1; have_next = false;
    return LmNext::Second;
  }
};

}
```

### pop_up_slam_amd/csrc/pps_solve.cpp

```cpp
#include "pps_graph.h"

using namespace pps;
using namespace pps_impl;

namespace pps_impl {

struct PhaseTimer {
  pps_graph* g; double* acc; bool on;
  PhaseTimer(pps_graph* g_, double* a) : g(g_), acc(a), on(g_->profiling >= 2) { if (on) (void)hipEventRecord(g->ev[0], g->stream); }
  ~PhaseTimer() {
    if (!on) return;
    (void)hipEventRecord(g->ev[1], g->stream);
    (void)hipEventSynchronize(g->ev[1]);
    float ms = 0;
    (void)hipEventElapsedTime(&ms, g->ev[0], g->ev[1]);
    *acc += 1e-3 * ms;
  }
};

static int take_event_pair(pps_graph* g, bool events, std::vector<hipEvent_t>& evs, int& used, hipEvent_t* e0, hipEvent_t* e1) {
  *e0 = *e1 = nullptr;
  if (!events) return PPS_OK;
  if (used + 2 > (int)evs.size()) for (int k = 0; k < 2; k++) { hipEvent_t e; HIP_TRY(g, hipEventCreate(&e)); evs.push_back(e); }
  *e0 = evs[used]; *e1 = evs[used + 1]; used += 2;
  return PPS_OK;
}
static int take_k1_events(pps_graph* g, char skip, hipEvent_t* e0, hipEvent_t* e1, int* pair = nullptr) {
  const bool events = g->profiling == 1;
  const int rc = take_event_pair(g, events, g->k1_events, g->k1_used, e0, e1); if (rc != PPS_OK) return rc;
  if (pair) *pair = events ? g->k1_used / 2 - 1 : -1;
  if (!events) return PPS_OK;
  g->k1_skip.resize(g->k1_events.size() / 2, 0);
  g->k1_skip[g->k1_used / 2 - 1] = skip;
  return PPS_OK;
}

int do_linearize(pps_graph* g, const LinGuard* guard = nullptr) {
  if (g->profiling == 1) {
    hipEvent_t e0, e1;
    { const int rc = take_k1_events(g, 0, &e0, &e1); if (rc != PPS_OK) return rc; }
    HIP_TRY(g, lin_launch(g, g->props.jacobian_mode, false, guard, e0, e1));
  } else
  { PhaseTimer t(g, &g->stats.t_linearize); HIP_TRY(g, lin_launch(g, g->props.jacobian_mode, false, guard)); }
  { PhaseTimer t(g, &g->stats.t_assemble); HIP_TRY(g, launch_hblocks(g->dev, g->stream, guard, k1_products(g->dev, g->props.jacobian_mode))); }
  if (!guard) g->stats.n_linearize++;
  return PPS_OK;
}

struct NoHook { void operator()() const {} };
template <class Hook = NoHook>
static int enqueue_factor_solve(pps_graph* g, const DevGraph& dv, const DualAlt* alt, double lambda, hipStream_t st_, bool events, Hook first_launched = Hook()) {
  const K3Plan& P = g->plan;
  hipEvent_t e0, e1;
  if (P.form == K3Form::BandAll) {
    { const int rc = take_event_pair(g, events, g->fk_events, g->fk_used, &e0, &e1); if (rc != PPS_OK) return rc; }
    g->k3_epoch = g->k3_epoch >= (1 << 30) ? 1 : g->k3_epoch + 1;
    HIP_TRY(g, launch_band_all_factor(dv, alt, P, lambda, g->k3_epoch, st_, e0, e1));
    first_launched();
    HIP_TRY(g, launch_band_all_solve(dv, alt, P, g->k3_epoch, st_));
    return PPS_OK;
  }
  const int top = (int)P.stages.size() - 1;
  const bool fuse = P.root.fusable;
  for (int st = 0; st <= top; st++) {
    { const int rc = take_event_pair(g, events, g->fk_events, g->fk_used, &e0, &e1); if (rc != PPS_OK) return rc; }
    if (fuse && st == top) HIP_TRY(g, launch_band_root(dv, alt, P, lambda, st_, e0, e1));
    else HIP_TRY(g, launch_band_factor(dv, alt, P.stages[st], lambda, st_, e0, e1));
    if (st == 0) first_launched();
  }
  for (int st = fuse ? top - 1 : top; st >= 0; st--) HIP_TRY(g, launch_band_solve(dv, alt, P.stages[st], st_));
  return PPS_OK;
}

static DualAlt dual_alt(const pps_graph* g, double lambda2) {
  return DualAlt{g->spec_L, g->spec_U, g->spec_delta, g->spec_result, g->spec_chi2_partials, g->spec_dn_partials, g->spec_ticket, lambda2};
}

int do_solve_on(pps_graph* g, const DevGraph& dv, double lambda, hipStream_t st_) { return enqueue_factor_solve(g, dv, nullptr, lambda, st_, false); }

int enqueue_plain_factor(pps_graph* g, double lambda) {
  const Analysis& A = g->an;
  const DevGraph& d = g->dev;
  if (g->use_band()) {
    for (const K3StagePlan& sp : g->plan.stages) HIP_TRY(g, launch_band_factor(d, nullptr, sp, lambda, g->stream, nullptr, nullptr, false));
    return PPS_OK;
  }
  if (g->use_dense()) {
    HIP_TRY(g, hipMemsetAsync(d.L, 0, (size_t)A.L_size * 8, g->stream));
    HIP_TRY(g, launch_dense_hpush(d, g->plan.max_el_per_front, lambda, g->stream));
  }
  for (int l = 0; l < A.n_levels; l++) {
    const int base = A.level_off[l] + l, cnt = A.level_off[l + 1] - A.level_off[l];
    if (g->use_dense()) HIP_TRY(g, launch_dense_factor_level(d, A.level_off[l], cnt, g->d_dw_asm + base, g->plan.dw_asm[base + cnt], g->d_dw_pan + base, g->plan.dw_pan[base + cnt],
                                                             g->d_dw_trl + base, g->plan.dw_trl[base + cnt], g->stream));
    else HIP_TRY(g, launch_factor_level(d, A.level_off[l], cnt, g->plan.level_max_front[l], lambda, g->stream));
  }
  return PPS_OK;
}

static int enqueue_plain_backsolve(pps_graph* g) {
  const Analysis& A = g->an;
  const DevGraph& d = g->dev;
  if (g->use_band()) {
    for (int st = A.n_stages - 1; st >= 0; st--) HIP_TRY(g, launch_band_solve(d, nullptr, g->plan.stages[st], g->stream));
    return PPS_OK;
  }
  for (int l = A.n_levels - 1; l >= 0; l--) {
    const int cnt = A.level_off[l + 1] - A.level_off[l];
    if (g->use_dense()) HIP_TRY(g, launch_dense_solve_level(d, A.level_off[l], cnt, g->plan.level_max_b[l], g->stream));
    else HIP_TRY(g, launch_backsolve_level(d, A.level_off[l], cnt, g->stream));
  }
  return PPS_OK;
}

int do_solve(pps_graph* g, double lambda) {
  if (g->use_band() && g->profiling < 2) {
    const int rc = do_solve_on(g, g->dev, lambda, g->stream); if (rc != PPS_OK) return rc;
  } else {
    { PhaseTimer t(g, &g->stats.t_factor); const int rc = enqueue_plain_factor(g, lambda); if (rc != PPS_OK) return rc; }
    { PhaseTimer t(g, &g->stats.t_backsolve); const int rc = enqueue_plain_backsolve(g); if (rc != PPS_OK) return rc; }
  }
  g->stats.n_factorize++;
  return PPS_OK;
}

static int check_handover(pps_graph* g, const double* rec) { return handover_timed_out(rec) ? fail(g, PPS_EHIP, kHandoverMessage) : PPS_OK; }

int wait_result(pps_graph* g, volatile double* slot, double seq, hipStream_t producer = nullptr) {
  const double t0 = now_s();
  unsigned spins = 0;
  while (slot[3] != seq) {
    if ((++spins & 0x3ff) == 0 && now_s() - t0 > 0.5) {
      HIP_TRY(g, hipStreamSynchronize(producer ? producer : g->stream));
      if (slot[3] != seq) return fail(g, PPS_EHIP, "result record did not arrive");
      break;
    }
  }
  __atomic_thread_fence(__ATOMIC_ACQUIRE);
  return check_handover(g, const_cast<const double*>(slot));
}

void swap_state(pps_graph* g) {
  std::swap(g->dev.pose_est, g->dev.pose_lin);
  std::swap(g->dev.plane_est, g->dev.plane_lin);
}

int copy_state(pps_graph* g, bool est_to_lin) {
  const DevGraph& d = g->dev;
  if (est_to_lin) { swap_state(g); return PPS_OK; }
  HIP_TRY(g, hipMemcpyAsync(d.pose_est, d.pose_lin, ((size_t)7 * d.pose_ld + (size_t)4 * d.plane_ld) * 8, hipMemcpyDeviceToDevice, g->stream));
  return PPS_OK;
}

int linpoint_from_estimate(pps_graph* g) {
  const DevGraph& d = g->dev;
  HIP_TRY(g, hipMemcpyAsync(d.pose_lin, d.pose_est, ((size_t)7 * d.pose_ld + (size_t)4 * d.plane_ld) * 8, hipMemcpyDeviceToDevice, g->stream));
  return PPS_OK;
}

int read_result(pps_graph* g, bool at_estimate, double* chi2, double* dnorm, bool* notpd) {
  if (g->n_live_factors == 0) { *chi2 = 0.0; if (dnorm) *dnorm = 0.0; if (notpd) *notpd = false; return PPS_OK; }
  {
    PhaseTimer t(g, &g->stats.t_retract_chi2);
    HIP_TRY(g, chi2_launch(g, at_estimate, g->host_result, 0.0));
  }
  HIP_TRY(g, hipStreamSynchronize(g->stream));
  *chi2 = g->host_result[0];
  if (dnorm) *dnorm = std::sqrt(g->host_result[1]);
  if (notpd) *notpd = g->host_result[2] != 0.0;
  return check_handover(g, g->host_result);
}

void resolve_k1_events(pps_graph* g) {
  for (int k = 0; k + 1 < g->k1_used; k += 2) {
    float ms = 0;
    if ((size_t)(k / 2) < g->k1_skip.size() && g->k1_skip[k / 2]) continue;
    if (hipEventElapsedTime(&ms, g->k1_events[k], g->k1_events[k + 1]) == hipSuccess) g->stats.t_linearize += 1e-3 * ms;
  }
  g->k1_used = 0;
  for (int k = 0; k + 1 < g->fk_used; k += 2) {
    float ms = 0;
    if (hipEventElapsedTime(&ms, g->fk_events[k], g->fk_events[k + 1]) == hipSuccess) g->stats.t_factor += 1e-3 * ms;
  }
  g->fk_used = 0;
}

static void reset_solve_stats(pps_graph* g) {
  pps_stats& s = g->stats;
  s.t_linearize = s.t_assemble = s.t_factor = s.t_backsolve = s.t_retract_chi2 = 0;
  s.n_linearize = s.n_factorize = 0;
  s.lm_iterations = s.lm_trials_accepted = s.lm_trials_rejected = s.lm_trials_notpd = 0;
  s.t_analysis = s.t_upload = 0;
  s.n_launches = 0;
  g->launches0 = launch_count();
}

static void end_solve_stats(pps_graph* g, double t0) { g->stats.t_total = now_s() - t0; g->stats.n_launches = (int)(launch_count() - g->launches0); }

void begin_solve(pps_graph* g) {
  reset_solve_stats(g);
  g->tr_lambda.clear(); g->tr_chi2.clear(); g->tr_acc.clear();
}

int clear_stale_status(pps_graph* g) {
  if (!g->status_clean) {
    HIP_TRY(g, launch_clear_status(g->dev, g->stream));
    if (g->spec_result) HIP_TRY(g, hipMemsetAsync(g->spec_result, 0, 4 * sizeof(double), g->stream));
  }
  g->status_clean = false;
  return PPS_OK;
}

void abandon_device_copy(pps_graph* g) {
  if (!g->dev_ready) return;
  (void)hipStreamSynchronize(g->stream);
  g->topo_dirty = true; g->dev_values_newer = false; g->dev_meas_newer = false;
  g->up_unknown = true; g->up_unknown_meas = true; g->pk_meas_ok = false; g->status_clean = false;
}

}

extern "C" {

static int update_impl(pps_graph* g);
int pps_update(pps_graph* g) {
  if (!g) return PPS_EINVAL;
  cov_invalidate(g);
  const int rc = update_impl(g);
  if (rc != PPS_OK && rc != PPS_ENOTPD) abandon_device_copy(g);
  return rc;
}
static int update_impl(pps_graph* g) {
  const double t0 = now_s();
  reset_solve_stats(g);
  if (g->n_live_nodes > 0 && g->n_live_factors == 0) return PPS_OK;
  int rc = prepare_solve(g);
  if (rc != PPS_OK) return rc;
  rc = clear_stale_status(g); if (rc != PPS_OK) return rc;
  rc = copy_state(g, true); if (rc != PPS_OK) return rc;
  rc = do_linearize(g); if (rc != PPS_OK) return rc;
  rc = do_solve(g, 0.0); if (rc != PPS_OK) return rc;
  double chi2 = 0.0, dn = 0.0; bool notpd = false;
  if (g->n_live_factors > 0 && g->dev.n_pose + g->dev.n_plane > 0 && !robust(g)) {
    const DevGraph& d = g->dev;
    { PhaseTimer t(g, &g->stats.t_retract_chi2);
      HIP_TRY(g, launch_trial_dual(d, DualAlt{}, d.pose_lin, d.plane_lin, d.pose_est, d.plane_est, nullptr, nullptr, g->host_result, 0.0, nullptr, 0.0, g->stream, 1)); }
    rc = enqueue_state_download(g); if (rc != PPS_OK) return rc;
    HIP_TRY(g, hipStreamSynchronize(g->stream));
    chi2 = g->host_result[0]; dn = std::sqrt(g->host_result[1]); notpd = g->host_result[2] != 0.0;
    rc = check_handover(g, g->host_result); if (rc != PPS_OK) return rc;
  } else {
    { PhaseTimer t(g, &g->stats.t_retract_chi2); HIP_TRY(g, launch_retract_apply(g->dev, g->stream)); }
    rc = enqueue_state_download(g); if (rc != PPS_OK) return rc;
    rc = read_result(g, true, &chi2, &dn, &notpd); if (rc != PPS_OK) return rc;
  }
  resolve_k1_events(g);
  if (notpd) {
    rc = copy_state(g, false); if (rc != PPS_OK) return rc;
    HIP_TRY(g, hipStreamSynchronize(g->stream));
    end_solve_stats(g, t0);
    return fail(g, PPS_ENOTPD, "normal equations not positive definite");
  }
  g->dev_values_newer = true;
  state_download_arrived(g);
  g->status_clean = true;
  g->stats.chi2_final = chi2; g->stats.last_delta_norm = dn; g->stats.lambda_final = 0;
  end_solve_stats(g, t0);
  return PPS_OK;
}

static int lm_solve(pps_graph* g, int* iterations);

int pps_batch_optimize(pps_graph* g, int* iterations) {
  if (!g) return PPS_EINVAL;
  cov_invalidate(g);
  if (g->n_live_nodes > 0 && g->n_live_factors == 0) {
    begin_solve(g);
    if (iterations) *iterations = 0;
    return PPS_OK;
  }
  const int rc = lm_solve(g, iterations);
  if (rc != PPS_OK && rc != PPS_ENOTPD) abandon_device_copy(g);
  return rc;
}

static int end_lm_solve(pps_graph* g, const LmControl& lm, const LmSink& sink, int* iterations, double t0) {
  { const int rc2 = enqueue_state_download(g); if (rc2 != PPS_OK) return rc2; }
  HIP_TRY(g, hipStreamSynchronize(g->stream));
  g->dev_values_newer = true;
  state_download_arrived(g);
  g->status_clean = true;
  resolve_k1_events(g);
  end_solve_stats(g, t0);
  if (g->dev.trace) report_front_trace(g);
  if (lm.finish(sink, iterations) != PPS_OK) return fail(g, PPS_ENOTPD, kLmNotPdMessage);
  return PPS_OK;
}

static int lm_solve_dual(pps_graph* g, int* iterations, double t0) {
  const pps_props& prop = g->props;
  const Analysis& A = g->an;
  int rc = clear_stale_status(g); if (rc != PPS_OK) return rc;
  LmDualWalk walk(prop);
  LmControl& lm = walk.lm;
  const LmSink sink = lm_sink(g, prop.verbose != 0);
  double* slot0 = g->host_result;
  double* slot[2] = {g->host_result + 4, g->host_result + 8};
  DevGraph& d = g->dev;
  rc = copy_state(g, true); if (rc != PPS_OK) return rc;
  double* const c_pose[3] = {d.pose_lin, d.pose_est, g->spec_pose};
  double* const c_plane[3] = {d.plane_lin, d.plane_est, g->spec_plane};
  auto t_pose = [&](int k) { return c_pose[walk.trial(k)]; };
  auto t_plane = [&](int k) { return c_plane[walk.trial(k)]; };
  double seqs[2] = {0, 0};
  const bool adaptive = A.n_fronts >= 2048;
  bool use_alt = !adaptive;
  const bool fuse_lin = !g->sw.no_spec_lin && g->spec_J != nullptr && trial_lin_ok(d, prop.jacobian_mode) && trial_lin_waves(d) <= 3072;
  int fused_pair = -1;
  int pred = 0, pred_launched = 0;
  bool error_known = false;
  auto enqueue_trial_lin = [&](const DualAlt& alt, double s0, double s1) -> int {
    pred_launched = use_alt ? pred : 0;
    const SpecLin sl{g->spec_J, g->spec_P, g->spec_H, g->spec_Hf, pred_launched};
    hipEvent_t e0, e1;
    { const int rc2 = take_k1_events(g, 1, &e0, &e1, &fused_pair); if (rc2 != PPS_OK) return rc2; }
    HIP_TRY(g, launch_trial_lin(d, alt, sl, d.pose_lin, d.plane_lin, t_pose(0), t_plane(0), t_pose(1), t_plane(1), slot[0], s0, slot[1], s1, g->stream, e0, e1));
    const LinGuard gd{{d.result_dev, g->spec_result}, {nullptr, nullptr}, {nullptr, nullptr}, lm.error, error_known ? 1 : 0, use_alt ? 0 : 1, pred_launched};
    HIP_TRY(g, launch_hblocks_spec(d, sl, g->stream, &gd));
    return PPS_OK;
  };
  const bool plain_host = g->sw.lm_plain_host;
  struct PendingNote {
    const LmSink& s; LmControl::Trial t{}; bool owed = false;
    void flush() { if (owed) { LmControl::note(s, t); owed = false; } }
    ~PendingNote() { flush(); }
  } pending{sink};
  const bool lm_timing = g->sw.lm_timing;
  double t_rec = 0.0, rt_pre = 0.0, rt_call = 0.0, rt_relin = 0.0; int rt_n = 0, rt_n_relin = 0; bool relin = false;
  auto rt_note = [&](double t_pre) {
    if (!lm_timing || t_rec <= 0.0) return;
    const double t = now_s();
    if (relin) { rt_relin += t - t_rec; rt_n_relin++; } else { rt_pre += t_pre - t_rec; rt_call += t - t_pre; rt_n++; }
    t_rec = 0.0; relin = false;
  };
  auto enqueue_dual = [&](double lam) -> int {
    const DualAlt alt = dual_alt(g, lam * prop.lm_lambda_factor);
    walk.begin_set(use_alt);
    const int n_trials = use_alt ? 2 : 1;
    const double t_pre = lm_timing ? now_s() : 0.0;
    {
      const int rc2 = enqueue_factor_solve(g, d, use_alt ? &alt : nullptr, lam, g->stream, g->profiling == 1, [&] { rt_note(t_pre); pending.flush(); });
      if (rc2 != PPS_OK) return rc2;
    }
    g->stats.n_factorize += n_trials;
    g->seq += 1.0; seqs[0] = g->seq;
    g->seq2 += 1.0; seqs[1] = g->seq2;
    if (fuse_lin) return enqueue_trial_lin(alt, seqs[0], seqs[1]);
    HIP_TRY(g, launch_trial_dual(d, alt, d.pose_lin, d.plane_lin, t_pose(0), t_plane(0), t_pose(1), t_plane(1), slot[0], seqs[0], slot[1], seqs[1],
                                 g->stream, n_trials));
    return PPS_OK;
  };
  rc = do_linearize(g); if (rc != PPS_OK) return rc;
  g->seq += 1.0;
  const double seq0 = g->seq;
  HIP_TRY(g, launch_chi2(d, false, slot0, seq0, g->stream));
  const bool spec_lin = !g->sw.no_spec_lin && !fuse_lin && !adaptive;
  int spec_pair = -1;
  auto enqueue_spec_lin = [&](double err) -> int {
    if (!spec_lin) return PPS_OK;
    LinGuard gd{{d.result_dev, g->spec_result}, {t_pose(0), t_pose(1)}, {t_plane(0), t_plane(1)}, err, 1, walk.have_next ? 0 : 1};
    spec_pair = g->profiling == 1 ? g->k1_used / 2 : -1;
    return do_linearize(g, &gd);
  };
  auto drop_spec_lin = [&]() { if (spec_pair >= 0 && (size_t)spec_pair < g->k1_skip.size()) g->k1_skip[spec_pair] = 1; spec_pair = -1; };
  rc = enqueue_dual(lm.lambda); if (rc != PPS_OK) return rc;
  rc = wait_result(g, slot0, seq0); if (rc != PPS_OK) return rc;
  lm.error = slot0[0]; error_known = true;
  g->stats.chi2_initial = lm.error;
  rc = enqueue_spec_lin(lm.error); if (rc != PPS_OK) return rc;
  rc = wait_result(g, slot[0], seqs[0]); if (rc != PPS_OK) return rc;
  lm.take_step(slot[0]);
  while (lm.running(prop)) {
    if (lm_timing) t_rec = now_s();
    const LmNext next = walk.judge(prop, slot[walk.cur][0], &pending.t);
    if (plain_host) LmControl::note(sink, pending.t); else pending.owed = true;
    if (next == LmNext::Done) break;
    if (next == LmNext::Second) {
      t_rec = 0.0;
      pending.flush();
    } else {
      if (next == LmNext::Relinearise) {
        const int acc = walk.cur;
        if (adaptive) use_alt = acc != 0;
        pred = acc;
        d.pose_lin = c_pose[walk.x]; d.plane_lin = c_plane[walk.x];
        if (fuse_lin && acc == pred_launched) {
          std::swap(d.J, g->spec_J); std::swap(d.P, g->spec_P); std::swap(d.H, g->spec_H); std::swap(d.Hf, g->spec_Hf);
          g->stats.n_linearize++;
          if (fused_pair >= 0 && (size_t)fused_pair < g->k1_skip.size()) g->k1_skip[fused_pair] = 0;
        }
        else if (fuse_lin) { relin = true; rc = do_linearize(g); if (rc != PPS_OK) return rc; }
        else if (spec_lin) { g->stats.n_linearize++; spec_pair = -1; }
        else { rc = do_linearize(g); if (rc != PPS_OK) return rc; }
      } else {
        drop_spec_lin();
        if (adaptive) use_alt = true;
      }
      rc = enqueue_dual(lm.lambda); if (rc != PPS_OK) return rc;
      rc = enqueue_spec_lin(lm.error); if (rc != PPS_OK) return rc;
    }
    rc = wait_result(g, slot[walk.cur], seqs[walk.cur]); if (rc != PPS_OK) return rc;
    lm.take_step(slot[walk.cur]);
  }
  drop_spec_lin();
  pending.flush();
  if (lm_timing && rt_n > 0)
    fprintf(stderr, "[lm] record -> factor launch: %d launch sets, mean %.2f us before the launch call + %.2f us inside it; %d sets that relinearised first, mean %.2f us\n",
            rt_n, 1e6 * rt_pre / rt_n, 1e6 * rt_call / rt_n, rt_n_relin, rt_n_relin ? 1e6 * rt_relin / rt_n_relin : 0.0);
  place_state_copies(g, c_pose, c_plane, walk.final_copy());
  return end_lm_solve(g, lm, sink, iterations, t0);
}

static int lm_solve(pps_graph* g, int* iterations) {
  const double t0 = now_s();
  begin_solve(g);
  int rc = prepare_solve(g);
  if (rc != PPS_OK) return rc;
  if (g->use_band() && g->profiling < 2 && !g->dev.trace && !g->sw.no_dual && !robust(g)) return lm_solve_dual(g, iterations, t0);
  const pps_props& prop = g->props;
  rc = clear_stale_status(g); if (rc != PPS_OK) return rc;
  LmControl lm(prop);
  const LmSink sink = lm_sink(g, prop.verbose != 0);
  double* slot0 = g->host_result;
  double* slot1 = g->host_result + 4;
  auto enqueue_trial = [&](double lam) -> int {
    int r = do_solve(g, lam); if (r != PPS_OK) return r;
    PhaseTimer t(g, &g->stats.t_retract_chi2);
    HIP_TRY(g, launch_retract_trial(g->dev, g->stream));
    g->seq += 1.0;
    HIP_TRY(g, chi2_trial_launch(g, slot1, g->seq));
    return PPS_OK;
  };
  rc = copy_state(g, true); if (rc != PPS_OK) return rc;
  rc = do_linearize(g); if (rc != PPS_OK) return rc;
  g->seq += 1.0;
  const double seq0 = g->seq;
  HIP_TRY(g, chi2_launch(g, false, slot0, seq0));
  rc = enqueue_trial(lm.lambda); if (rc != PPS_OK) return rc;
  rc = wait_result(g, slot0, seq0); if (rc != PPS_OK) return rc;
  rc = wait_result(g, slot1, g->seq); if (rc != PPS_OK) return rc;
  lm.error = slot0[0];
  g->stats.chi2_initial = lm.error;
  lm.take_step(slot1);
  bool trial_pending = true;
  while (lm.running(prop)) {
    const LmVerdict v = lm.judge(sink, slot1[0]);
    if (v == LmVerdict::Converged) { trial_pending = false; break; }
    if (v == LmVerdict::Accepted) { rc = do_linearize(g); if (rc != PPS_OK) return rc; }
    else swap_state(g);
    rc = enqueue_trial(lm.lambda); if (rc != PPS_OK) return rc;
    rc = wait_result(g, slot1, g->seq); if (rc != PPS_OK) return rc;
    lm.take_step(slot1);
  }
  if (trial_pending) swap_state(g);
  swap_state(g);
  return end_lm_solve(g, lm, sink, iterations, t0);
}

int pps_chi2(pps_graph* g, double* chi2) {
  if (!g || !chi2) return PPS_EINVAL;
  int rc = prepare_solve(g);
  if (rc != PPS_OK) return rc;
  double dn; bool np;
  return read_result(g, true, chi2, &dn, &np);
}

static int debug_solve_impl(pps_graph* g, double lambda, double lambda2, double* delta, double* delta2, int* form, double* not_pd) {
  int rc = prepare_solve(g);
  if (rc != PPS_OK) return rc;
  const bool dual = lambda2 >= 0.0;
  if (dual && !(g->use_band() && g->spec_L && g->spec_U && g->spec_delta && g->spec_result))
    return fail(g, PPS_ESTATE, "debug_solve: two damping values in one launch need the band kernels and their second L / U / delta set (this graph runs in another K3 form)");
  if (form) *form = g->use_band() ? (g->plan.form == K3Form::BandAll ? 1 : 0) : (g->use_dense() ? 2 : 3);
  const DevGraph& d = g->dev;
  rc = clear_stale_status(g); if (rc != PPS_OK) return rc;
  rc = linpoint_from_estimate(g); if (rc != PPS_OK) return rc;
  rc = do_linearize(g); if (rc != PPS_OK) return rc;
  if (dual) {
    const DualAlt alt = dual_alt(g, lambda2);
    rc = enqueue_factor_solve(g, d, &alt, lambda, g->stream, false); if (rc != PPS_OK) return rc;
  } else {
    rc = do_solve(g, lambda); if (rc != PPS_OK) return rc;
  }
  double status[8] = {0, 0, 0, 0, 0, 0, 0, 0};
  const size_t n = (size_t)std::max(0, d.n_scalars);
  if (n) HIP_TRY(g, hipMemcpyAsync(delta, d.delta, n * 8, hipMemcpyDeviceToHost, g->stream));
  if (n && dual) HIP_TRY(g, hipMemcpyAsync(delta2, g->spec_delta, n * 8, hipMemcpyDeviceToHost, g->stream));
  HIP_TRY(g, hipMemcpyAsync(status, d.result_dev, 4 * sizeof(double), hipMemcpyDeviceToHost, g->stream));
  if (dual) HIP_TRY(g, hipMemcpyAsync(status + 4, g->spec_result, 4 * sizeof(double), hipMemcpyDeviceToHost, g->stream));
  HIP_TRY(g, hipStreamSynchronize(g->stream));
  if (status[2] != 0.0 || status[6] != 0.0) {
    rc = clear_stale_status(g); if (rc != PPS_OK) return rc;
    HIP_TRY(g, hipStreamSynchronize(g->stream));
  }
  g->status_clean = true;
  if (not_pd) *not_pd = std::max(status[2], status[6]);
  return PPS_OK;
}

int pps_debug_solve(pps_graph* g, double lambda, double lambda2, double* delta, double* delta2, int* form, double* not_pd) {
  if (!g) return PPS_EINVAL;
  if (!delta) return fail(g, PPS_EINVAL, "debug_solve: null delta");
  if (!(lambda >= 0.0) || !std::isfinite(lambda)) return fail(g, PPS_EINVAL, "debug_solve: lambda must be a finite number >= 0");
  if (std::isnan(lambda2) || std::isinf(lambda2)) return fail(g, PPS_EINVAL, "debug_solve: lambda2 must be a finite number (negative: one damping value)");
  if (lambda2 >= 0.0 && !delta2) return fail(g, PPS_EINVAL, "debug_solve: lambda2 >= 0 needs delta2");
  if (g->n_live_nodes == 0) return fail(g, PPS_ESTATE, "empty graph");
  if (g->n_live_factors == 0) return fail(g, PPS_ESTATE, "debug_solve: the graph has no factor");
  cov_invalidate(g);
  int rc;
  { NoSolveScope scope(g); rc = debug_solve_impl(g, lambda, lambda2, delta, delta2, form, not_pd); }
  if (rc != PPS_OK && rc != PPS_EINVAL && rc != PPS_ESTATE) abandon_device_copy(g);
  return rc;
}

}
```

### pop_up_slam_amd/csrc/pps_upload.cpp

```cpp
#include "pps_graph.h"

using namespace pps;
using namespace pps_impl;

namespace pps_impl {

void free_device(pps_graph* g) {
  for (void* p : g->allocs) (void)hipFree(p);
  g->allocs.clear();
  for (pps_graph::Arena* a : {&g->up, &g->scr}) {
    const size_t want = (a == &g->up ? std::max(a->off, g->up_high) : a->off) + a->spill;
    if (a->spill > 0 || a->base == nullptr) {
      if (a->base) (void)hipFree(a->base);
      a->cap = std::max<size_t>(size_t(1) << 20, 2 * want);
      if (hipMalloc(reinterpret_cast<void**>(&a->base), a->cap) != hipSuccess) { a->base = nullptr; a->cap = 0; }
      if (a == &g->up) { g->up_slots.clear(); g->up_high = 0; g->up_unknown = true; }
    }
    a->off = 0; a->spill = 0;
  }
  g->up_cursor = 0; g->up_patches.clear();
  if (g->stage_cap < g->up.cap) {
    if (g->stage) (void)hipHostFree(g->stage);
    g->stage = nullptr; g->stage_cap = 0;
    if (hipHostMalloc(reinterpret_cast<void**>(&g->stage), g->up.cap, hipHostMallocDefault) == hipSuccess) g->stage_cap = g->up.cap;
    g->up_unknown = true;
  }
  g->stage_lo = g->stage_hi = 0;
  g->dev = DevGraph();
}

void release_arenas(pps_graph* g) {
  for (pps_graph::Arena* a : {&g->up, &g->scr}) { if (a->base) (void)hipFree(a->base); a->base = nullptr; a->cap = a->off = a->spill = 0; }
  if (g->stage) (void)hipHostFree(g->stage);
  g->stage = nullptr; g->stage_cap = 0;
  if (g->patch_host) (void)hipHostFree(g->patch_host);
  if (g->state_pin) (void)hipHostFree(g->state_pin);
  g->state_pin = nullptr; g->state_pin_cap = 0; g->pin_holds_est = false;
  g->patch_host = nullptr; g->patch_cap = 0;
  g->up_slots.clear(); g->up_high = 0; g->up_unknown = true;
}

void up_diff(pps_graph* g, size_t o, const char* src, size_t n, bool force, size_t same_prefix) {
  if (n == 0) return;
  char* mir = g->stage + o;
  g->up_bytes_total += n;
  if (g->up_unknown || force) { memcpy(mir, src, n); g->up_patches.push_back(pps_graph::UpPatch{o, n, false}); return; }
  same_prefix = std::min(same_prefix, n) & ~size_t(63);
  if (same_prefix && g->verify_hints && memcmp(mir, src, same_prefix) != 0) g->hint_violation = true;
  size_t lo = same_prefix, hi = n;
  while (lo + 4096 <= hi && memcmp(mir + lo, src + lo, 4096) == 0) lo += 4096;
  while (lo + 64 <= hi && memcmp(mir + lo, src + lo, 64) == 0) lo += 64;
  if (lo + 64 > hi && memcmp(mir + lo, src + lo, hi - lo) == 0) return;
  while (hi >= lo + 4096 && memcmp(mir + hi - 4096, src + hi - 4096, 4096) == 0) hi -= 4096;
  while (hi >= lo + 64 && memcmp(mir + hi - 64, src + hi - 64, 64) == 0) hi -= 64;
  lo &= ~size_t(15);
  memcpy(mir + lo, src + lo, hi - lo);
  g->up_patches.push_back(pps_graph::UpPatch{o + lo, hi - lo, false});
}


int flush_uploads(pps_graph* g) {
  size_t sent = 0;
  for (const auto& pt : g->up_patches) sent += pt.len;
  g->up_bytes_sent = sent;
  if (g->up_patches.empty()) { g->up_bytes_total = 0; return PPS_OK; }
  if (g->up_unknown) {
    size_t lo = 0, hi = 0;
    for (const auto& pt : g->up_patches) hi = std::max(hi, pt.off + pt.len);
    hi = std::max(hi, g->up_high); hi = std::min(hi, g->stage_cap);
    HIP_TRY(g, hipMemcpyAsync(g->up.base + lo, g->stage + lo, hi - lo, hipMemcpyHostToDevice, g->stream));
    g->up_bytes_sent = hi - lo;
  } else {
    const size_t np = g->up_patches.size();
    const size_t need = np * 32;
    if (need > g->patch_cap) {
      if (g->patch_host) (void)hipHostFree(g->patch_host);
      g->patch_host = nullptr; g->patch_cap = 0;
      const size_t cap = std::max<size_t>(1 << 12, 2 * need);
      HIP_TRY(g, hipHostMalloc(reinterpret_cast<void**>(&g->patch_host), cap, hipHostMallocDefault));
      g->patch_cap = cap;
    }
    long long* tab = reinterpret_cast<long long*>(g->patch_host);
    for (size_t i = 0; i < np; i++) {
      const auto& pt = g->up_patches[i];
      const size_t len = pt.exact8 ? pt.len : ((pt.len + 15) & ~size_t(15));
      tab[4 * i + 0] = (long long)pt.off; tab[4 * i + 1] = (long long)pt.off; tab[4 * i + 2] = (long long)len; tab[4 * i + 3] = pt.exact8 ? 1 : 0;
    }
    HIP_TRY(g, launch_scatter_patches(g->patch_host, g->stage, (int)np, g->up.base, g->stream));
  }
  g->up_unknown = false;
  g->up_patches.clear();
  g->stage_lo = g->stage_hi = 0;
  return PPS_OK;
}

int verify_uploads(pps_graph* g, const char* where) {
  if (g->hint_violation) { g->hint_violation = false; return fail(g, PPS_ESTATE, std::string("upload verification (") + where + "): an array differs from the mirror inside the part the analysis reported as kept"); }
  if (!g->sw.verify_upload || g->up_high == 0 || g->up.spill) return PPS_OK;
  HIP_TRY(g, hipStreamSynchronize(g->stream));
  std::vector<char> dev(g->up_high);
  HIP_TRY(g, hipMemcpy(dev.data(), g->up.base, g->up_high, hipMemcpyDeviceToHost));
  for (size_t k = 0; k < g->up_slots.size() && k < g->up_cursor; k++) {
    if (k == g->slot_obs_meas || k == g->slot_lp_meas) continue;
    const size_t o = g->up_slots[k].off, n = std::min(g->up_slots[k].cap, g->up_high - std::min(g->up_high, o));
    if (o >= g->up_high) continue;
    if (memcmp(dev.data() + o, g->stage + o, n) != 0) {
      size_t b = 0; while (b < n && dev[o + b] == g->stage[o + b]) b++;
      return fail(g, PPS_ESTATE, std::string("upload verification (") + where + "): slot " + std::to_string(k) + " (offset " + std::to_string(o) + ", capacity " +
                                     std::to_string(g->up_slots[k].cap) + ") differs from the mirror at byte " + std::to_string(b));
    }
  }
  return PPS_OK;
}

int ensure_device(pps_graph* g) {
  if (g->dev_ready) return PPS_OK;
  HIP_TRY(g, hipSetDevice(g->props.device));
  HIP_TRY(g, hipStreamCreateWithFlags(&g->stream, hipStreamNonBlocking));
  HIP_TRY(g, hipHostMalloc(reinterpret_cast<void**>(&g->host_result), 12 * sizeof(double), hipHostMallocDefault));
  HIP_TRY(g, hipEventCreate(&g->ev[0]));
  HIP_TRY(g, hipEventCreate(&g->ev[1]));
  g->dev_ready = true;
  return PPS_OK;
}

int64_t j_capacity(int64_t n) { int64_t c = 16; while (c < n) c <<= 1; return c; }
void j_bases(const pps_graph* g, int64_t base[4], int64_t* total) {
  const int64_t n_pp = g->fslot_ids[F_POSE_PRIOR].size(), n_odo = g->fslot_ids[F_ODOMETRY].size(),
                n_obs = g->fslot_ids[F_PLANE_OBS].size(), n_lp = g->fslot_ids[F_PLANE_PRIOR].size();
  const int64_t joff_obs = 0, joff_odo = j_capacity(n_obs) * 30, joff_pp = joff_odo + j_capacity(n_odo) * 78,
                joff_lp = joff_pp + j_capacity(n_pp) * 42;
  base[F_POSE_PRIOR] = joff_pp; base[F_ODOMETRY] = joff_odo; base[F_PLANE_OBS] = joff_obs; base[F_PLANE_PRIOR] = joff_lp;
  if (total) *total = joff_lp + j_capacity(n_lp) * 12;
}
void p_bases(const pps_graph* g, int64_t base[4], int64_t* total) {
  const int64_t n_pp = g->fslot_ids[F_POSE_PRIOR].size(), n_odo = g->fslot_ids[F_ODOMETRY].size(),
                n_obs = g->fslot_ids[F_PLANE_OBS].size(), n_lp = g->fslot_ids[F_PLANE_PRIOR].size();
  const int64_t p_obs = 0, p_odo = j_capacity(n_obs) * kPSize[F_PLANE_OBS], p_pp = p_odo + j_capacity(n_odo) * kPSize[F_ODOMETRY],
                p_lp = p_pp + j_capacity(n_pp) * kPSize[F_POSE_PRIOR];
  base[F_POSE_PRIOR] = p_pp; base[F_ODOMETRY] = p_odo; base[F_PLANE_OBS] = p_obs; base[F_PLANE_PRIOR] = p_lp;
  if (total) *total = p_lp + j_capacity(n_lp) * kPSize[F_PLANE_PRIOR];
}

static int run_analysis_impl(pps_graph* g);
int run_analysis(pps_graph* g) {
  const int rc = run_analysis_impl(g);
  if (rc != PPS_OK) { g->analyzed = false; g->analysis_stale = true; g->topo_dirty = true; g->cmp_valid = false; g->an_seq++; g->an_base_seq = -1; }
  return rc;
}
static int run_analysis_impl(pps_graph* g) {
  const double t0 = now_s();
  std::vector<SymNode>& sn = g->sym_nodes;
  std::vector<SymFactor>& sf = g->sym_factors;
  bool append = g->cmp_valid && g->grown_only && g->n_analyses > 0 && !g->cmp_has_repop && g->cmp_nodes <= g->nodes.size() &&
                g->cmp_factors <= g->factors.size() && !g->sw.no_incr_compact;
  for (size_t i = g->cmp_factors; append && i < g->factors.size(); i++)
    append = !g->factors[i].deleted && !(g->factors[i].type == F_PLANE_OBS && g->factors[i].repop);
  for (size_t i = g->cmp_nodes; append && i < g->nodes.size(); i++) append = !g->nodes[i].deleted;
  if (append) {
    for (size_t i = g->cmp_nodes; i < g->nodes.size(); i++) {
      HostNode& n = g->nodes[i];
      n.compact = (int)sn.size();
      if (n.type == NODE_POSE) { n.slot = (int)g->pose_ids.size(); g->pose_ids.push_back((int)i); sn.push_back({NODE_POSE, 6, n.slot}); }
      else { n.slot = (int)g->plane_ids.size(); g->plane_ids.push_back((int)i); sn.push_back({NODE_PLANE, 3, -1}); }
    }
    for (size_t i = g->cmp_factors; i < g->factors.size(); i++) {
      HostFactor& f = g->factors[i];
      f.slot = (int)g->fslot_ids[f.type].size();
      g->fslot_ids[f.type].push_back((int)i);
    }
    g->n_obs_fixed = (int)g->fslot_ids[F_PLANE_OBS].size();
    int64_t base[4], j_total = 0, pbase[4], p_total = 0;
    j_bases(g, base, &j_total);
    p_bases(g, pbase, &p_total);
    if (j_total > 0x7fffffffLL || p_total > 0x7fffffffLL) return fail(g, PPS_ENOMEM, "graph too large for int32 J offsets");
    if (memcmp(base, g->cmp_base, sizeof(base)) != 0) {
      int cnt[4] = {0, 0, 0, 0};
      for (SymFactor& q : sf) { const int k = cnt[q.type]++; q.joff = (int)(base[q.type] + (int64_t)k * kJSize[q.type]); q.poff = (int)(pbase[q.type] + (int64_t)k * kPSize[q.type]); }
      memcpy(g->cmp_base, base, sizeof(base));
    }
    for (size_t i = g->cmp_factors; i < g->factors.size(); i++) {
      const HostFactor& f = g->factors[i];
      SymFactor q;
      q.type = f.type;
      q.a = g->nodes[f.a].compact;
      q.b = f.b >= 0 ? g->nodes[f.b].compact : -1;
      q.joff = (int)(base[f.type] + (int64_t)f.slot * kJSize[f.type]);
      q.poff = (int)(pbase[f.type] + (int64_t)f.slot * kPSize[f.type]);
      q.direct_ok = f.type == F_PLANE_OBS ? 1 : 0;
      sf.push_back(q);
    }
  } else {
  g->pose_ids.clear(); g->plane_ids.clear();
  for (int t = 0; t < 4; t++) g->fslot_ids[t].clear();
  sn.clear(); sf.clear();
  for (size_t i = 0; i < g->nodes.size(); i++) {
    HostNode& n = g->nodes[i];
    if (n.deleted) { n.compact = n.slot = -1; continue; }
    n.compact = (int)sn.size();
    if (n.type == NODE_POSE) { n.slot = (int)g->pose_ids.size(); g->pose_ids.push_back((int)i); sn.push_back({NODE_POSE, 6, n.slot}); }
    else { n.slot = (int)g->plane_ids.size(); g->plane_ids.push_back((int)i); sn.push_back({NODE_PLANE, 3, -1}); }
  }
  g->cmp_has_repop = false;
  for (int pass = 0; pass < 2; pass++)
    for (size_t i = 0; i < g->factors.size(); i++) {
      HostFactor& f = g->factors[i];
      if (f.deleted) { f.slot = -1; continue; }
      if ((f.type == F_PLANE_OBS && f.repop) != (pass == 1)) continue;
      if (pass == 1) g->cmp_has_repop = true;
      f.slot = (int)g->fslot_ids[f.type].size();
      g->fslot_ids[f.type].push_back((int)i);
    }
  g->n_obs_fixed = 0;
  for (int id : g->fslot_ids[F_PLANE_OBS]) g->n_obs_fixed += g->factors[id].repop ? 0 : 1;
  int64_t base[4], j_total = 0, pbase[4], p_total = 0;
  j_bases(g, base, &j_total);
  p_bases(g, pbase, &p_total);
  if (j_total > 0x7fffffffLL || p_total > 0x7fffffffLL) return fail(g, PPS_ENOMEM, "graph too large for int32 J offsets");
  memcpy(g->cmp_base, base, sizeof(base));
  sf.reserve(g->factors.size());
  bool any_deleted = false;
  for (size_t i = 0; i < g->factors.size(); i++) {
    const HostFactor& f = g->factors[i];
    if (f.deleted) { any_deleted = true; continue; }
    SymFactor s;
    s.type = f.type;
    s.a = g->nodes[f.a].compact;
    s.b = f.b >= 0 ? g->nodes[f.b].compact : -1;
    s.joff = (int)(base[f.type] + (int64_t)f.slot * kJSize[f.type]);
    s.poff = (int)(pbase[f.type] + (int64_t)f.slot * kPSize[f.type]);
    s.direct_ok = (f.type == F_PLANE_OBS && !f.repop) ? 1 : 0;
    sf.push_back(s);
  }
  g->cmp_valid = !any_deleted && sn.size() == g->nodes.size();
  }
  g->cmp_nodes = g->nodes.size(); g->cmp_factors = g->factors.size();
  g->aprm.band_levels = 0;
  g->aprm.seg_len = 64;
  g->aprm.aligned_cuts = (g->n_analyses > 0 && g->grown_only) ? 1 : 0;
  if (g->aprm.aligned_cuts && g->pose_ids.size() < 4000) g->aprm.band_levels = 3;
  g->aprm.band_rows = band_front_limit();
  const char* msg = "";
  try {
  if (g->sw.analysis_timing) fprintf(stderr, "[analysis] %-22s %8.3f ms\n", "compaction (api)", 1e3 * (now_s() - t0));
  if (!g->acache) g->acache = analysis_cache_new();
  if (!analyze(sn, sf, g->aprm, g->an, &msg, g->sw.no_incremental ? nullptr : g->acache))
    return fail(g, PPS_EINVAL, std::string("analysis failed: ") + msg);
  if (g->an.max_front > band_front_limit() && g->aprm.max_pivots < dense_front_max_pivots()) {
    AnalysisParams wide = g->aprm;
    wide.max_pivots = dense_front_max_pivots();
    if (!analyze(sn, sf, wide, g->an, &msg, g->sw.no_incremental ? nullptr : g->acache))
      return fail(g, PPS_EINVAL, std::string("analysis failed: ") + msg);
  }
  } catch (const std::bad_alloc&) {
    g->an = Analysis();
    return fail(g, PPS_ENOMEM, "symbolic analysis ran out of host memory (fronts too wide for this ordering)");
  }
  g->plan = plan_k3(k3_tree_view(g->an), K3Switches{g->sw.no_preassemble, g->sw.no_solve_flow, g->sw.no_root_fuse, g->sw.no_strip, g->sw.trace});
  if (!g->use_band() && !g->use_dense() && g->an.max_front > 4096)
    return fail(g, PPS_ENOMEM, "fronts too wide for this ordering (max front " + std::to_string(g->an.max_front) +
                               " scalars): the pose chain is not a good dissection backbone for this graph");
  if (g->sw.analysis_timing) fprintf(stderr, "[analysis] %-22s %8.3f ms\n", "total incl. api", 1e3 * (now_s() - t0));
  g->analyzed = true; g->analysis_stale = false;
  g->n_analyses++; g->grown_only = true;
  g->an_base_seq = g->an_seq; g->an_seq++;
  g->stats.n_fronts = g->an.n_fronts; g->stats.n_levels = g->an.n_levels; g->stats.max_front = g->an.max_front;
  g->stats.nnz_L = g->an.L_size;
  g->stats.t_analysis = now_s() - t0;
  return PPS_OK;
}

int state_pin_reserve(pps_graph* g, size_t doubles) {
// ... 380 lines not shown
```

Before: 19290 LM iters/s.

## Sum trial chi2 partials on host from pinned slots instead of waiting for device record

Each trial's chi2 and step-norm block partials, plus the not-PD status, are also written with their sequence tag into pinned host memory. The host sums them as soon as all slots arrive, so it can judge the LM step before the last-block ticket reduction publishes the device record. The device record is still checked later and any mismatch raises an error. This aims to cut host-visible latency on each LM iteration's critical path, at the cost of extra host-mapped writes and host-side polling and summation.

```diff
diff --git a/include/pps.h b/include/pps.h
--- a/include/pps.h
+++ b/include/pps.h
@@ -162,6 +162,8 @@
 int pps_debug_front_factor_w(int tiles, int strip, int p, int b, const double* A, double* L, double* U, double* not_pd, int width);
 
 int pps_debug_exmap(int kind, int n, const double* x, const double* delta, double* out);
+
+int pps_debug_host_sum(const pps_graph* g, int counts[2]);
 
 int pps_debug_solve(pps_graph* g, double lambda, double lambda2, double* delta, double* delta2, int* form, double* not_pd);
 
diff --git a/pop_up_slam_amd/__init__.py b/pop_up_slam_amd/__init__.py
--- a/pop_up_slam_amd/__init__.py
+++ b/pop_up_slam_amd/__init__.py
@@ -111,7 +111,7 @@
     "pps_frames_set_calibration", "pps_frames_add", "pps_refresh_measurements", "pps_get_measurement",
     "pps_popup_download_segments3d", "pps_assoc_default_params", "pps_landmark_update", "pps_landmark_set_merged",
     "pps_find_closest_planes", "pps_graph_save", "pps_graph_load", "pps_add_plane_obs2", "pps_edge_ray",
-    "pps_time_linearize", "pps_debug_front_factor", "pps_debug_front_factor_w", "pps_debug_exmap", "pps_debug_solve", "pps_reproject_points", "pps_popup_set_outputs",
+    "pps_time_linearize", "pps_debug_front_factor", "pps_debug_front_factor_w", "pps_debug_exmap", "pps_debug_solve", "pps_debug_host_sum", "pps_reproject_points", "pps_popup_set_outputs",
     "pps_edge_default_params", "pps_edges_create", "pps_edges_destroy", "pps_edges_last_error", "pps_edges_select",
     "pps_edges_download_label", "pps_edges_contour", "pps_edges_last_kernel_time", "pps_edges_host_contour",
     "pps_edges_host_select", "pps_popup_fill_depth", "pps_popup_plane_info", "pps_popup_mask_host",
@@ -234,6 +234,8 @@
             L.pps_debug_front_factor_w.argtypes = L.pps_debug_front_factor.argtypes + [C.c_int]
         L.pps_debug_exmap.argtypes = [C.c_int, C.c_int, _dp, _dp, _dp]
         L.pps_debug_solve.argtypes = [C.c_void_p, C.c_double, C.c_double, _dp, _dp, C.POINTER(C.c_int), C.POINTER(C.c_double)]
+        if hasattr(L, "pps_debug_host_sum"):
+            L.pps_debug_host_sum.argtypes = [C.c_void_p, _ip]
         L.pps_reproject_points.argtypes = [C.c_void_p, C.c_int, _ip, _fp, _fp]
         L.pps_graph_save.argtypes = [C.c_void_p, C.c_char_p, C.c_int]
         L.pps_graph_load.argtypes = [C.c_char_p, C.POINTER(PpsProps), C.POINTER(C.c_void_p)]
@@ -423,6 +425,11 @@
     def debug_cov_select_form(self, form):
         self._ck(self.L.pps_debug_cov_select_form(self.h, int(form)))
 
+    def debug_host_sum(self):
+        c = (C.c_int * 2)()
+        self._ck(self.L.pps_debug_host_sum(self.h, c))
+        return int(c[0]), int(c[1])
+
     def debug_cov_path_form(self, form):
         self._ck(self.L.pps_debug_cov_path_form(self.h, int(form)))
 
diff --git a/pop_up_slam_amd/csrc/pps_api.cpp b/pop_up_slam_amd/csrc/pps_api.cpp
--- a/pop_up_slam_amd/csrc/pps_api.cpp
+++ b/pop_up_slam_amd/csrc/pps_api.cpp
@@ -18,6 +18,7 @@
   s.no_dual = on("PPS_NO_DUAL");
   s.lm_plain_host = on("PPS_LM_PLAIN_HOST");
   s.no_early_record = on("PPS_NO_EARLY_RECORD");
+  s.no_host_sum = on("PPS_NO_HOST_SUM");
   s.no_strip = on("PPS_NO_STRIP");
   s.no_incremental = on("PPS_NO_INCREMENTAL");
   s.no_incr_compact = on("PPS_NO_INCR_COMPACT");
@@ -32,7 +33,7 @@
     long long tm = num("PPS_TIMING", 0);
     if (on("PPS_TIMING") && tm <= 0) tm = 7;
     s.analysis_timing = (tm & 1) != 0; s.upload_timing = (tm & 2) != 0; s.multi_timing = (tm & 8) ? 2 : ((tm & 4) ? 1 : 0);
-    s.lm_timing = (tm & 16) != 0;
+    s.lm_timing = (tm & 16) != 0; s.lm_lead_timing = (tm & 32) != 0;
   }
   s.multi_split = (int)num("PPS_MULTI_SPLIT", 0);
   s.multi_thread_factors = num("PPS_MULTI_THREAD_FACTORS", 120000);
@@ -150,6 +151,7 @@
     free_device(g);
     release_arenas(g);
     if (g->host_result) (void)hipHostFree(g->host_result);
+    if (g->host_slots) (void)hipHostFree(g->host_slots);
     if (g->ev[0]) (void)hipEventDestroy(g->ev[0]);
     if (g->ev[1]) (void)hipEventDestroy(g->ev[1]);
     for (hipEvent_t e : g->k1_events) (void)hipEventDestroy(e);
diff --git a/pop_up_slam_amd/csrc/pps_device.h b/pop_up_slam_amd/csrc/pps_device.h
--- a/pop_up_slam_amd/csrc/pps_device.h
+++ b/pop_up_slam_amd/csrc/pps_device.h
@@ -86,6 +86,7 @@
   bool split_expand = false;
   bool no_spec_lin = false;
   bool no_dual = false;
+  bool no_host_sum = false;
   bool no_early_record = false;
   bool lm_plain_host = false;
   bool no_strip = false;
@@ -95,7 +96,7 @@
   bool multi_levels = false, multi_thread_form = false;
   int debug_drop_flag = 0;
   int trace = 0;
-  bool analysis_timing = false, upload_timing = false, lm_timing = false;
+  bool analysis_timing = false, upload_timing = false, lm_timing = false, lm_lead_timing = false;
   int multi_timing = 0;
   int multi_split = 0;
   long long multi_thread_factors = 120000;
@@ -145,6 +146,9 @@
   unsigned int* ticket;
   double lambda;
 };
+struct HostSlots { double* s[2] = {nullptr, nullptr}; };
+constexpr int kHostSlotsMax = 64;
+int trial_host_slots(const DevGraph& d, int* nb_chi, int* nb_ret);
 hipError_t ensure_k3_attrs();
 hipError_t launch_band_factor(const DevGraph& d, const DualAlt* alt, const K3StagePlan& sp, double lambda, hipStream_t st, hipEvent_t ev0 = nullptr,
                               hipEvent_t ev1 = nullptr, bool pre_ok = true);
@@ -156,10 +160,10 @@
 hipError_t launch_band_all_solve(const DevGraph& d, const DualAlt* alt, const K3Plan& p, int epoch, hipStream_t st);
 hipError_t launch_trial_dual(const DevGraph& d, const DualAlt& alt, const double* base_pose, const double* base_plane, double* out_pose0,
                              double* out_plane0, double* out_pose1, double* out_plane1, double* host_result0, double seq0, double* host_result1,
-                             double seq1, hipStream_t st, int n_trials = 2);
+                             double seq1, hipStream_t st, int n_trials = 2, const HostSlots& hs = HostSlots{});
 hipError_t launch_trial_lin(const DevGraph& d, const DualAlt& alt, const SpecLin& sl, const double* base_pose, const double* base_plane, double* out_pose0,
                             double* out_plane0, double* out_pose1, double* out_plane1, double* host_result0, double seq0, double* host_result1,
-                            double seq1, hipStream_t st, hipEvent_t ev0 = nullptr, hipEvent_t ev1 = nullptr);
+                            double seq1, hipStream_t st, hipEvent_t ev0 = nullptr, hipEvent_t ev1 = nullptr, const HostSlots& hs = HostSlots{});
 int trial_lin_waves(const DevGraph& d);
 bool trial_lin_ok(const DevGraph& d, int mode);
 hipError_t launch_hblocks_spec(const DevGraph& d, const SpecLin& sl, hipStream_t st, const LinGuard* guard = nullptr);
diff --git a/pop_up_slam_amd/csrc/pps_graph.h b/pop_up_slam_amd/csrc/pps_graph.h
--- a/pop_up_slam_amd/csrc/pps_graph.h
+++ b/pop_up_slam_amd/csrc/pps_graph.h
@@ -140,6 +140,8 @@
   size_t up_bytes_sent = 0, up_bytes_total = 0;
   double* host_result = nullptr;
   double seq = 0.0;
+  double* host_slots = nullptr;
+  int hs_trials = 0, hs_mismatches = 0;
   double *spec_pose = nullptr, *spec_plane = nullptr, *spec_chi2_partials = nullptr, *spec_dn_partials = nullptr;
   unsigned int* spec_ticket = nullptr;
   double seq2 = 0.0;
diff --git a/pop_up_slam_amd/csrc/pps_k4.hip b/pop_up_slam_amd/csrc/pps_k4.hip
--- a/pop_up_slam_amd/csrc/pps_k4.hip
+++ b/pop_up_slam_amd/csrc/pps_k4.hip
@@ -78,7 +78,8 @@
 }
 
 __device__ __forceinline__ void body_retract_to(const DevGraph& d, const double* __restrict__ base_pose, const double* __restrict__ base_plane,
-                                                double* __restrict__ out_pose, double* __restrict__ out_plane, int bx, double* red, bool light = false) {
+                                                double* __restrict__ out_pose, double* __restrict__ out_plane, int bx, double* red, bool light = false,
+                                                double* __restrict__ hslots = nullptr, int hslot0 = 0, double seq = 0.0) {
   const int i = bx * blockDim.x + threadIdx.x;
   double dn = 0.0;
   if (i < d.n_pose) {
@@ -107,6 +108,7 @@
   __syncthreads();
   if (threadIdx.x == 0) {
     const double t = red[0] + red[1] + red[2] + red[3];
+    if (hslots) host_slot_store(hslots, hslot0 + bx, t, seq);
     if (light) publish_partial(&d.dn_partials[bx], t); else d.dn_partials[bx] = t;
   }
 }
@@ -114,18 +116,19 @@
 __global__ __launch_bounds__(kChiBlock) void k_trial_dual(DevGraph d, DualAlt alt, const double* __restrict__ base_pose, const double* __restrict__ base_plane,
                                                           double* __restrict__ out_pose, double* __restrict__ out_plane, double* __restrict__ out_pose1,
                                                           double* __restrict__ out_plane1, int nb_ret, int nb_obs, int nb_odo, int nb_pp, int nb_chi,
-                                                          double* __restrict__ out, double seq, double* __restrict__ out1, double seq1) {
+                                                          double* __restrict__ out, double seq, double* __restrict__ out1, double seq1, HostSlots hs) {
   if (blockIdx.y) {
     d.delta = alt.delta; d.chi2_partials = alt.chi2_partials; d.dn_partials = alt.dn_partials; d.ticket = alt.ticket; d.result_dev = alt.result_dev;
     out_pose = out_pose1; out_plane = out_plane1; out = out1; seq = seq1;
   }
+  double* const hslots = hs.s[blockIdx.y ? 1 : 0];
   const int total = nb_ret + nb_chi;
   if ((int)blockIdx.x >= nb_ret) {
-    body_chi2<true, true>(d, base_pose, base_plane, nb_obs, nb_odo, nb_pp, nb_ret, out, seq, (int)blockIdx.x - nb_ret, nb_chi, total);
+    body_chi2<true, true>(d, base_pose, base_plane, nb_obs, nb_odo, nb_pp, nb_ret, out, seq, (int)blockIdx.x - nb_ret, nb_chi, total, CostFn{}, false, hslots);
     return;
   }
   __shared__ double red[4];
-  body_retract_to(d, base_pose, base_plane, out_pose, out_plane, blockIdx.x, red);
+  body_retract_to(d, base_pose, base_plane, out_pose, out_plane, blockIdx.x, red, false, hslots, nb_chi, seq);
   __shared__ bool last;
   if (threadIdx.x == 0) {
     __builtin_amdgcn_fence(__ATOMIC_RELEASE, "agent");
@@ -142,21 +145,27 @@
 
 hipError_t launch_trial_dual(const DevGraph& d, const DualAlt& alt, const double* base_pose, const double* base_plane, double* out_pose0,
                              double* out_plane0, double* out_pose1, double* out_plane1, double* host_result0, double seq0, double* host_result1,
-                             double seq1, hipStream_t st, int n_trials) {
+                             double seq1, hipStream_t st, int n_trials, const HostSlots& hs) {
   const int n = d.n_pose + d.n_plane;
   const int nb_obs = cdiv(d.n_obs, kChiBlock), nb_odo = cdiv(d.n_odo, kChiBlock), nb_pp = cdiv(d.n_pp, kChiBlock), nb_lp = cdiv(d.n_lp, kChiBlock);
   const int nb = nb_obs + nb_odo + nb_pp + nb_lp;
   if (nb == 0 || n == 0) return hipErrorInvalidValue;
   const int nb_ret = cdiv(n, 256);
   PPS_LAUNCH(k_trial_dual, dim3(nb_ret + nb, n_trials), dim3(kChiBlock), 0, st, d, alt, base_pose, base_plane, out_pose0, out_plane0, out_pose1, out_plane1, nb_ret,
-             nb_obs, nb_odo, nb_pp, nb, host_result0, seq0, host_result1, seq1);
-  return hipGetLastError();
+             nb_obs, nb_odo, nb_pp, nb, host_result0, seq0, host_result1, seq1, hs);
+  return hipGetLastError();
+}
+
+int trial_host_slots(const DevGraph& d, int* nb_chi, int* nb_ret) {
+  *nb_chi = cdiv(d.n_obs, kChiBlock) + cdiv(d.n_odo, kChiBlock) + cdiv(d.n_pp, kChiBlock) + cdiv(d.n_lp, kChiBlock);
+  *nb_ret = cdiv(d.n_pose + d.n_plane, 256);
+  return *nb_chi + *nb_ret + 1;
 }
 
 __global__ __launch_bounds__(kChiBlock) void k_trial_lin(DevGraph d, DualAlt alt, SpecLin sl, const double* __restrict__ base_pose, const double* __restrict__ base_plane,
                                                          double* __restrict__ out_pose, double* __restrict__ out_plane, double* __restrict__ out_pose1,
                                                          double* __restrict__ out_plane1, int nb_ret, int nb_obs, int nb_odo, int nb_pp, int nb_chi,
-                                                         double* __restrict__ out, double seq, double* __restrict__ out1, double seq1, int lb_obs, int lb_odo, int lb_pp, int apply) {
+                                                         double* __restrict__ out, double seq, double* __restrict__ out1, double seq1, int lb_obs, int lb_odo, int lb_pp, int apply, HostSlots hs) {
   static_assert(kChiBlock == kLanesPerBlock, "one block size for the trial blocks and the lane-form sweep");
   const int total = nb_ret + nb_chi;
   const bool sweep = (int)blockIdx.x >= 2 * total;
@@ -173,12 +182,13 @@
   }
   const bool light = (d.sw & SW_NO_EARLY_RECORD) == 0;
   if (light) __builtin_amdgcn_s_setprio(3);
+  double* const hslots = hs.s[y];
   if (bx0 >= nb_ret) {
-    body_chi2<true, true>(d, base_pose, base_plane, nb_obs, nb_odo, nb_pp, nb_ret, out, seq, bx0 - nb_ret, nb_chi, total, CostFn{}, light);
+    body_chi2<true, true>(d, base_pose, base_plane, nb_obs, nb_odo, nb_pp, nb_ret, out, seq, bx0 - nb_ret, nb_chi, total, CostFn{}, light, hslots);
     return;
   }
   __shared__ double red[4];
-  body_retract_to(d, base_pose, base_plane, out_pose, out_plane, bx0, red, light);
+  body_retract_to(d, base_pose, base_plane, out_pose, out_plane, bx0, red, light, hslots, nb_chi, seq);
   __shared__ bool last;
   if (threadIdx.x == 0) {
     if (!light) __builtin_amdgcn_fence(__ATOMIC_RELEASE, "agent");
@@ -202,7 +212,7 @@
 
 hipError_t launch_trial_lin(const DevGraph& d, const DualAlt& alt, const SpecLin& sl, const double* base_pose, const double* base_plane, double* out_pose0,
                             double* out_plane0, double* out_pose1, double* out_plane1, double* host_result0, double seq0, double* host_result1,
-                            double seq1, hipStream_t st, hipEvent_t ev0, hipEvent_t ev1) {
+                            double seq1, hipStream_t st, hipEvent_t ev0, hipEvent_t ev1, const HostSlots& hs) {
   const int n = d.n_pose + d.n_plane;
   const int nb_obs = cdiv(d.n_obs, kChiBlock), nb_odo = cdiv(d.n_odo, kChiBlock), nb_pp = cdiv(d.n_pp, kChiBlock), nb_lp = cdiv(d.n_lp, kChiBlock);
   const int nb = nb_obs + nb_odo + nb_pp + nb_lp;
@@ -212,7 +222,7 @@
             lb_lp = cdiv(d.n_lp, kFactorsPerBlock);
   const int lb_all = lb_obs + lb_odo + lb_pp + lb_lp;
   PPS_LAUNCH_EV(ev0, ev1, k_trial_lin, dim3(2 * (nb_ret + nb) + lb_all), dim3(kChiBlock), 0, st, d, alt, sl, base_pose, base_plane, out_pose0,
-                out_plane0, out_pose1, out_plane1, nb_ret, nb_obs, nb_odo, nb_pp, nb, host_result0, seq0, host_result1, seq1, lb_obs, lb_odo, lb_pp, 1);
+                out_plane0, out_pose1, out_plane1, nb_ret, nb_obs, nb_odo, nb_pp, nb, host_result0, seq0, host_result1, seq1, lb_obs, lb_odo, lb_pp, 1, hs);
   return hipGetLastError();
 }
 
diff --git a/pop_up_slam_amd/csrc/pps_k4_body.h b/pop_up_slam_amd/csrc/pps_k4_body.h
--- a/pop_up_slam_amd/csrc/pps_k4_body.h
+++ b/pop_up_slam_amd/csrc/pps_k4_body.h
@@ -11,6 +11,12 @@
   const unsigned long long old = __hip_atomic_exchange(reinterpret_cast<unsigned long long*>(p), (unsigned long long)__double_as_longlong(v),
                                                        __ATOMIC_RELAXED, __HIP_MEMORY_SCOPE_AGENT);
   asm volatile("" ::"v"(old));
+}
+
+typedef double host_slot_t __attribute__((ext_vector_type(2)));
+__device__ __forceinline__ void host_slot_store(double* hslots, int slot, double v, double seq) {
+  host_slot_t x; x.x = v; x.y = seq;
+  *reinterpret_cast<volatile host_slot_t*>(hslots + 2 * (size_t)slot) = x;
 }
 
 __device__ __forceinline__ void chi2_finish(const DevGraph& d, int nb, int n_dn, double* __restrict__ out, double seq, bool light = false) {
@@ -43,8 +49,11 @@
 template <bool TICKET = true, bool APPLY = false, bool ROBUST = false>
 __device__ __forceinline__ void body_chi2(const DevGraph& d, const double* __restrict__ pose,
                                           const double* __restrict__ plane, int nb_obs, int nb_odo, int nb_pp,
-                                          int n_dn, double* __restrict__ out, double seq, int bx, int nb, int total_blocks = 0, const CostFn& cost = CostFn{}, bool light = false) {
+                                          int n_dn, double* __restrict__ out, double seq, int bx, int nb, int total_blocks = 0, const CostFn& cost = CostFn{}, bool light = false,
+                                          double* __restrict__ hslots = nullptr) {
   __shared__ double red[kChiBlock / 64];
+  const bool send_status = TICKET && hslots && bx == 0 && threadIdx.x == 0;
+  const double npd0 = send_status ? __hip_atomic_load(&d.result_dev[2], __ATOMIC_RELAXED, __HIP_MEMORY_SCOPE_AGENT) : 0.0;
   int b = bx;
   double s = 0.0;
   if (b < nb_obs) {
@@ -118,6 +127,8 @@
   if (threadIdx.x == 0) {
     double t = 0.0;
     for (int k = 0; k < kChiBlock / 64; k++) t += red[k];
+    if (hslots) host_slot_store(hslots, bx, t, seq);
+    if (send_status) host_slot_store(hslots, nb + n_dn, npd0, seq);
     if (light) publish_partial(&d.chi2_partials[bx], t);
     else { d.chi2_partials[bx] = t; __builtin_amdgcn_fence(__ATOMIC_RELEASE, "agent"); }
     asm volatile("s_waitcnt vmcnt(0)" ::: "memory");
diff --git a/pop_up_slam_amd/csrc/pps_lm.h b/pop_up_slam_amd/csrc/pps_lm.h
--- a/pop_up_slam_amd/csrc/pps_lm.h
+++ b/pop_up_slam_amd/csrc/pps_lm.h
@@ -73,6 +73,24 @@
   }
 };
 
+inline double chi2_tree_sum(const double* partials, int n) {
+  double a = 0.0;
+  for (int w = 0; w < 4; w++) {
+    double lane[64];
+    const int live = n - 64 * w < 64 ? (n - 64 * w > 0 ? n - 64 * w : 0) : 64;
+    for (int l = 0; l < live; l++) {
+      double s = 0.0;
+      for (int i = 64 * w + l; i < n; i += 256) s += partials[i];
+      lane[l] = s;
+    }
+    for (int l = live; l < 64; l++) lane[l] = 0.0;
+    for (int o = 32; o > 0; o >>= 1)
+      for (int l = 0; l < o; l++) lane[l] += lane[l + o];
+    a += lane[0];
+  }
+  return a;
+}
+
 enum class LmNext {
   Done,
   Second,
diff --git a/pop_up_slam_amd/csrc/pps_solve.cpp b/pop_up_slam_amd/csrc/pps_solve.cpp
--- a/pop_up_slam_amd/csrc/pps_solve.cpp
+++ b/pop_up_slam_amd/csrc/pps_solve.cpp
@@ -140,6 +140,37 @@
   return check_handover(g, const_cast<const double*>(slot));
 }
 
+static int wait_host_sum(pps_graph* g, const double* slots, int nb_chi, int nb_ret, double seq, double* rec, volatile double* dev_rec, bool* summed) {
+  typedef double slot_t __attribute__((vector_size(16)));
+  const int n = nb_chi + nb_ret + 1;
+  double val[kHostSlotsMax];
+  unsigned long long pending = n >= 64 ? ~0ull : (1ull << n) - 1;
+  const double t0 = now_s();
+  unsigned spins = 0;
+  *summed = true;
+  while (pending) {
+    for (unsigned long long m = pending; m; m &= m - 1) {
+      const int i = __builtin_ctzll(m);
+      const slot_t x = *reinterpret_cast<const volatile slot_t*>(slots + 2 * i);
+      if (x[1] == seq) { val[i] = x[0]; pending &= ~(1ull << i); }
+    }
+    if (pending && (++spins & 0x3ff) == 0 && now_s() - t0 > 0.5) {
+      HIP_TRY(g, hipStreamSynchronize(g->stream));
+      if (dev_rec[3] != seq) return fail(g, PPS_EHIP, "result record did not arrive");
+      __atomic_thread_fence(__ATOMIC_ACQUIRE);
+      for (int k = 0; k < 3; k++) rec[k] = dev_rec[k];
+      *summed = false;
+      return check_handover(g, rec);
+    }
+  }
+  rec[0] = chi2_tree_sum(val, nb_chi);
+  rec[1] = chi2_tree_sum(val + nb_chi, nb_ret);
+  rec[2] = val[n - 1];
+  return check_handover(g, rec);
+}
+constexpr const char* kHostSumMessage = "internal error: the host's sum of a trial's partial sums differs from the device's result record";
+static bool same_word(double a, double b) { return memcmp(&a, &b, 8) == 0 || (a != a && b != b); }
+
 void swap_state(pps_graph* g) {
   std::swap(g->dev.pose_est, g->dev.pose_lin);
   std::swap(g->dev.plane_est, g->dev.plane_lin);
@@ -200,6 +231,7 @@
 void begin_solve(pps_graph* g) {
   reset_solve_stats(g);
   g->tr_lambda.clear(); g->tr_chi2.clear(); g->tr_acc.clear();
+  g->hs_trials = g->hs_mismatches = 0;
 }
 
 int clear_stale_status(pps_graph* g) {
@@ -314,6 +346,40 @@
   auto t_plane = [&](int k) { return c_plane[walk.trial(k)]; };
   double seqs[2] = {0, 0};
   const bool adaptive = A.n_fronts >= 2048;
+  int nb_chi = 0, nb_ret = 0;
+  const bool host_sum = !g->sw.no_host_sum && g->host_slots != nullptr && !adaptive &&trial_host_slots(g->dev, &nb_chi, &nb_ret) <= kHostSlotsMax;
+  HostSlots hs;
+  if (host_sum) { hs.s[0] = g->host_slots; hs.s[1] = g->host_slots + 2 * kHostSlotsMax; }
+  double hrec[2][4] = {{0, 0, 0, 0}, {0, 0, 0, 0}};
+  const double* rec[2] = {host_sum ? hrec[0] : g->host_result + 4, host_sum ? hrec[1] : g->host_result + 8};
+  bool owed_verify[2] = {false, false}; double owed_seq[2] = {0, 0};
+  int verify_rc = PPS_OK;
+  const bool lead_timing = g->sw.lm_lead_timing;
+  double rt_lead = 0.0; int rt_n_lead = 0;
+  auto verify_sums = [&]() {
+    for (int k = 0; k < 2; k++) {
+      if (!owed_verify[k]) continue;
+      owed_verify[k] = false;
+      volatile double* dr = g->host_result + 4 + 4 * k;
+      const int rc2 = wait_result(g, dr, owed_seq[k]);
+      if (rc2 != PPS_OK) { if (verify_rc == PPS_OK) verify_rc = rc2; continue; }
+      if (same_word(dr[0], hrec[k][0]) && same_word(dr[1], hrec[k][1]) && same_word(dr[2], hrec[k][2])) continue;
+      g->hs_mismatches++;
+      if (verify_rc == PPS_OK) verify_rc = fail(g, PPS_EHIP, kHostSumMessage);
+    }
+  };
+  auto wait_trial = [&](int k) -> int {
+    if (!host_sum) return wait_result(g, g->host_result + 4 + 4 * k, seqs[k]);
+    bool summed = false;
+    const int rc2 = wait_host_sum(g, hs.s[k], nb_chi, nb_ret, seqs[k], hrec[k], g->host_result + 4 + 4 * k, &summed);
+    if (rc2 == PPS_OK && summed) { g->hs_trials++; owed_verify[k] = true; owed_seq[k] = seqs[k]; }
+    if (rc2 == PPS_OK && summed && lead_timing) {
+      const double t_sum = now_s();
+      const int rc3 = wait_result(g, g->host_result + 4 + 4 * k, seqs[k]); if (rc3 != PPS_OK) return rc3;
+      rt_lead += now_s() - t_sum; rt_n_lead++;
+    }
+    return rc2;
+  };
   bool use_alt = !adaptive;
   const bool fuse_lin = !g->sw.no_spec_lin && g->spec_J != nullptr && trial_lin_ok(d, prop.jacobian_mode) && trial_lin_waves(d) <= 3072;
   int fused_pair = -1;
@@ -324,7 +390,7 @@
     const SpecLin sl{g->spec_J, g->spec_P, g->spec_H, g->spec_Hf, pred_launched};
     hipEvent_t e0, e1;
     { const int rc2 = take_k1_events(g, 1, &e0, &e1, &fused_pair); if (rc2 != PPS_OK) return rc2; }
-    HIP_TRY(g, launch_trial_lin(d, alt, sl, d.pose_lin, d.plane_lin, t_pose(0), t_plane(0), t_pose(1), t_plane(1), slot[0], s0, slot[1], s1, g->stream, e0, e1));
+    HIP_TRY(g, launch_trial_lin(d, alt, sl, d.pose_lin, d.plane_lin, t_pose(0), t_plane(0), t_pose(1), t_plane(1), slot[0], s0, slot[1], s1, g->stream, e0, e1, hs));
     const LinGuard gd{{d.result_dev, g->spec_result}, {nullptr, nullptr}, {nullptr, nullptr}, lm.error, error_known ? 1 : 0, use_alt ? 0 : 1, pred_launched};
     HIP_TRY(g, launch_hblocks_spec(d, sl, g->stream, &gd));
     return PPS_OK;
@@ -337,6 +403,7 @@
   } pending{sink};
   const bool lm_timing = g->sw.lm_timing;
   double t_rec = 0.0, rt_pre = 0.0, rt_call = 0.0, rt_relin = 0.0; int rt_n = 0, rt_n_relin = 0; bool relin = false;
+  double t_queued = 0.0, rt_verdict = 0.0; int rt_n_verdict = 0;
   auto rt_note = [&](double t_pre) {
     if (!lm_timing || t_rec <= 0.0) return;
     const double t = now_s();
@@ -349,17 +416,20 @@
     const int n_trials = use_alt ? 2 : 1;
     const double t_pre = lm_timing ? now_s() : 0.0;
     {
-      const int rc2 = enqueue_factor_solve(g, d, use_alt ? &alt : nullptr, lam, g->stream, g->profiling == 1, [&] { rt_note(t_pre); pending.flush(); });
+      const int rc2 = enqueue_factor_solve(g, d, use_alt ? &alt : nullptr, lam, g->stream, g->profiling == 1, [&] { rt_note(t_pre); pending.flush(); verify_sums(); });
       if (rc2 != PPS_OK) return rc2;
+      if (verify_rc != PPS_OK) return verify_rc;
     }
     g->stats.n_factorize += n_trials;
     g->seq += 1.0; seqs[0] = g->seq;
     g->seq2 += 1.0; seqs[1] = g->seq2;
-    if (fuse_lin) return enqueue_trial_lin(alt, seqs[0], seqs[1]);
+    if (fuse_lin) { const int rc2 = enqueue_trial_lin(alt, seqs[0], seqs[1]); if (lm_timing) t_queued = now_s(); return rc2; }
     HIP_TRY(g, launch_trial_dual(d, alt, d.pose_lin, d.plane_lin, t_pose(0), t_plane(0), t_pose(1), t_plane(1), slot[0], seqs[0], slot[1], seqs[1],
-                                 g->stream, n_trials));
+                                 g->stream, n_trials, hs));
+    if (lm_timing) t_queued = now_s();
     return PPS_OK;
   };
+  auto verdict_note = [&]() { if (lm_timing && t_queued > 0.0) { rt_verdict += now_s() - t_queued; rt_n_verdict++; t_queued = 0.0; } };
   rc = do_linearize(g); if (rc != PPS_OK) return rc;
   g->seq += 1.0;
   const double seq0 = g->seq;
@@ -378,11 +448,12 @@
   lm.error = slot0[0]; error_known = true;
   g->stats.chi2_initial = lm.error;
   rc = enqueue_spec_lin(lm.error); if (rc != PPS_OK) return rc;
-  rc = wait_result(g, slot[0], seqs[0]); if (rc != PPS_OK) return rc;
-  lm.take_step(slot[0]);
+  rc = wait_trial(0); if (rc != PPS_OK) return rc;
+  t_queued = 0.0;
+  lm.take_step(rec[0]);
   while (lm.running(prop)) {
     if (lm_timing) t_rec = now_s();
-    const LmNext next = walk.judge(prop, slot[walk.cur][0], &pending.t);
+    const LmNext next = walk.judge(prop, rec[walk.cur][0], &pending.t);
     if (plain_host) LmControl::note(sink, pending.t); else pending.owed = true;
     if (next == LmNext::Done) break;
     if (next == LmNext::Second) {
@@ -409,14 +480,21 @@
       rc = enqueue_dual(lm.lambda); if (rc != PPS_OK) return rc;
       rc = enqueue_spec_lin(lm.error); if (rc != PPS_OK) return rc;
     }
-    rc = wait_result(g, slot[walk.cur], seqs[walk.cur]); if (rc != PPS_OK) return rc;
-    lm.take_step(slot[walk.cur]);
+    rc = wait_trial(walk.cur); if (rc != PPS_OK) return rc;
+    if (walk.cur == 0) verdict_note();
+    lm.take_step(rec[walk.cur]);
   }
   drop_spec_lin();
   pending.flush();
+  verify_sums();
+  if (verify_rc != PPS_OK) return verify_rc;
+  if (lead_timing && rt_n_lead > 0)
+    fprintf(stderr, "[lm] host sum -> device record: %d trials, the record arrived a mean %.2f us after the host had the sum\n", rt_n_lead, 1e6 * rt_lead / rt_n_lead);
   if (lm_timing && rt_n > 0)
-    fprintf(stderr, "[lm] record -> factor launch: %d launch sets, mean %.2f us before the launch call + %.2f us inside it; %d sets that relinearised first, mean %.2f us\n",
-            rt_n, 1e6 * rt_pre / rt_n, 1e6 * rt_call / rt_n, rt_n_relin, rt_n_relin ? 1e6 * rt_relin / rt_n_relin : 0.0);
+    fprintf(stderr, "[lm] record -> factor launch: %d launch sets, mean %.2f us before the launch call + %.2f us inside it; %d sets that relinearised first, mean %.2f us; "
+                    "launch set queued -> its first verdict: %d sets, mean %.2f us (%s)\n",
+            rt_n, 1e6 * rt_pre / rt_n, 1e6 * rt_call / rt_n, rt_n_relin, rt_n_relin ? 1e6 * rt_relin / rt_n_relin : 0.0,
+            rt_n_verdict, rt_n_verdict ? 1e6 * rt_verdict / rt_n_verdict : 0.0, host_sum ? "summed on the host" : "the device's record");
   place_state_copies(g, c_pose, c_plane, walk.final_copy());
   return end_lm_solve(g, lm, sink, iterations, t0);
 }
@@ -467,6 +545,12 @@
   return end_lm_solve(g, lm, sink, iterations, t0);
 }
 
+int pps_debug_host_sum(const pps_graph* g, int counts[2]) {
+  if (!g || !counts) return PPS_EINVAL;
+  counts[0] = g->hs_trials; counts[1] = g->hs_mismatches;
+  return PPS_OK;
+}
+
 int pps_chi2(pps_graph* g, double* chi2) {
   if (!g || !chi2) return PPS_EINVAL;
   int rc = prepare_solve(g);
diff --git a/pop_up_slam_amd/csrc/pps_upload.cpp b/pop_up_slam_amd/csrc/pps_upload.cpp
--- a/pop_up_slam_amd/csrc/pps_upload.cpp
+++ b/pop_up_slam_amd/csrc/pps_upload.cpp
@@ -118,6 +118,8 @@
   HIP_TRY(g, hipSetDevice(g->props.device));
   HIP_TRY(g, hipStreamCreateWithFlags(&g->stream, hipStreamNonBlocking));
   HIP_TRY(g, hipHostMalloc(reinterpret_cast<void**>(&g->host_result), 12 * sizeof(double), hipHostMallocDefault));
+  HIP_TRY(g, hipHostMalloc(reinterpret_cast<void**>(&g->host_slots), 2 * kHostSlotsMax * 2 * sizeof(double), hipHostMallocDefault));
+  memset(g->host_slots, 0, 2 * kHostSlotsMax * 2 * sizeof(double));
   HIP_TRY(g, hipEventCreate(&g->ev[0]));
   HIP_TRY(g, hipEventCreate(&g->ev[1]));
   g->dev_ready = true;
```

Measured after the change: 19310 LM iters/s, median of 3. Within noise of the previous version (+0.1%).
